# angela000/DQNFlappyBird

Hardware: AMD Instinct MI355X
Metric: env steps/sec (whole node) + DQN grad-steps/sec, 80x80x4 batch=32 (higher is better)
Workload: dtype f32

## Files before the change

dqnflappybird_amd/csrc/fb_common.h:

```cpp
#pragma once
#include <hip/hip_runtime.h>
#include <stdarg.h>
#include <stdint.h>
#include <stdio.h>
#include <string.h>
#include "../../include/fbdqn.h"

extern thread_local char fb_err_buf[512];
int fb_set_error(int code, const char *fmt, ...);

#define FB_CHECK_HIP(expr)                                                                     \
    do {                                                                                       \
        hipError_t e_ = (expr);                                                                \
        if (e_ != hipSuccess)                                                                  \
            return fb_set_error(FB_ERR_HIP, "%s failed: %s (%s:%d)", #expr, hipGetErrorString(e_), \
                                __FILE__, __LINE__);                                           \
    } while (0)

#define FB_REQUIRE(cond, ...)                                          \
    do {                                                               \
        if (!(cond)) return fb_set_error(FB_ERR_INVALID, __VA_ARGS__); \
    } while (0)

#define FB_LAUNCH_CHECK() FB_CHECK_HIP(hipGetLastError())
// ... 4 lines not shown
    return algo == FB_ALGO_C51 || algo == FB_ALGO_C51_DOUBLE || algo == FB_ALGO_C51_PER || algo == FB_ALGO_C51_DOUBLE_PER;
}
static inline bool is_double_c51(int algo) { return algo == FB_ALGO_C51_DOUBLE || algo == FB_ALGO_C51_DOUBLE_PER; }
static inline bool is_qr_algo(int algo) {
    return algo == FB_ALGO_QR || algo == FB_ALGO_QR_DOUBLE || algo == FB_ALGO_QR_PER || algo == FB_ALGO_QR_DOUBLE_PER;
}
static inline bool is_double_qr(int algo) { return algo == FB_ALGO_QR_DOUBLE || algo == FB_ALGO_QR_DOUBLE_PER; }
static inline bool is_per_algo(int algo) {
    return algo == FB_ALGO_PER || algo == FB_ALGO_C51_PER || algo == FB_ALGO_C51_DOUBLE_PER || algo == FB_ALGO_QR_PER ||
           algo == FB_ALGO_QR_DOUBLE_PER;
}

__device__ __forceinline__ unsigned long long fb_flag_load(const unsigned long long *flag) { return __hip_atomic_load(flag, __ATOMIC_RELAXED, __HIP_MEMORY_SCOPE_AGENT); }
__device__ __forceinline__ void fb_flag_store(unsigned long long *flag, unsigned long long v) { __hip_atomic_store(flag, v, __ATOMIC_RELAXED, __HIP_MEMORY_SCOPE_AGENT); }
__device__ __forceinline__ void fb_flag_acquire() { __atomic_thread_fence(__ATOMIC_ACQUIRE); }
struct FbGate { const unsigned long long *flag; unsigned long long val; unsigned *timeouts; };
__device__ __forceinline__ void fb_flag_wait(const unsigned long long *flag, unsigned long long v, unsigned *timeouts);
__device__ __forceinline__ bool fb_gate_workgroup(const FbGate &g) {
    if (!g.flag || blockIdx.x != gridDim.x - 1) return false;
    if (threadIdx.x == 0) fb_flag_wait(g.flag, g.val, g.timeouts);
    return true;
}
__device__ __forceinline__ void fb_flag_wait(const unsigned long long *flag, unsigned long long v, unsigned *timeouts) {
    if (fb_flag_load(flag) >= v) return;
    const long long t0 = wall_clock64();
    while (fb_flag_load(flag) < v) {
        __builtin_amdgcn_s_sleep(8);
        if (wall_clock64() - t0 > 100000000LL) { atomicAdd(timeouts, 1u); break; }
    }
}

#define FB_STREAM_GAP 0u
#define FB_STREAM_EPS 1u
#define FB_STREAM_SAMPLE 2u
#define FB_STREAM_PER 3u
#define FB_STREAM_INIT 4u
#define FB_STREAM_EVAL 5u
#define FB_STREAM_NOISE 6u
#define FB_STREAM_ENV_NOISE 7u

struct fb_u4 { uint32_t x, y, z, w; };

__host__ __device__ static inline fb_u4 fb_philox(uint32_t k0, uint32_t k1, uint32_t c0, uint32_t c1,
                                                  uint32_t c2, uint32_t c3) {
#pragma unroll
    for (int r = 0; r < 10; r++) {
        uint64_t p0 = (uint64_t)0xD2511F53u * c0, p1 = (uint64_t)0xCD9E8D57u * c2;
        uint32_t n0 = (uint32_t)(p1 >> 32) ^ c1 ^ k0, n1 = (uint32_t)p1;
        uint32_t n2 = (uint32_t)(p0 >> 32) ^ c3 ^ k1, n3 = (uint32_t)p0;
        c0 = n0; c1 = n1; c2 = n2; c3 = n3;
        k0 += 0x9E3779B9u; k1 += 0xBB67AE85u;
    }
    return fb_u4{c0, c1, c2, c3};
}

struct FbMT { uint32_t mt[624]; uint32_t idx; };

struct FbSplitFlags;
struct FbSampleCtx { FbMT *mt; int *error; long long n; FbSplitFlags *gate; unsigned long long gate_val; long long newest_from; int wait_last_round; };
struct FbSampleRider { FbSampleCtx ctx; int k; long long setsize; long long *out; };
struct NetOff { int bf1, wv, bv, wq, bq, n; };
struct HeadCore {
    const float *hf; int stot, nks; float *q; int FC, A, dueling; NetOff off;
    uint8_t *actions; float epsilon; uint32_t seed_lo, seed_hi, step_lo, step_hi;
};
struct FbHeadRider { HeadCore c; const float *params; int on; unsigned long long *on_arrival; unsigned long long arrival_val; };
struct FbEvalRider {
    const int32_t *env_of;
    int32_t *ep_k, *ep_len;
    int32_t *score, *length; uint8_t *trunc;
    int episodes;
    unsigned *live;
    unsigned long long *done_step;
    unsigned long long step;
};
struct FbGatherCtx {
    long long cap; int n_envs, t_f, kind;
    const unsigned long long *bits; const uint8_t *act; const float *rew; const uint8_t *term; int *error;
    int nstep; double gamma;
};
struct FbRingSrc { FbGatherCtx c; long long steps; const long long *idx; uint8_t *a; float *r; uint8_t *t; };
int fb_replay_ring_src(fb_replay_t h, int batch, const int64_t *idx, uint8_t *a, float *r, uint8_t *t, FbRingSrc *out);
int fb_qnet_train_step_ring(fb_qnet_t h, int algo, int batch, const FbRingSrc *ring, const float *isw, double gamma, float *loss,
                            float *abs_err, float *flat_grad, void *stream, const FbSampleRider *rider = nullptr, const struct FbSplitCtx *split = nullptr);
struct FbSplitFlags {
    unsigned long long c_entry, p0[7];
    unsigned long long trunk_done, p2[7];
    unsigned long long fc1_done, p3[7];
    unsigned long long env_done, p4[7];
    unsigned long long last_round, p8[7];
    unsigned clean_count;
    unsigned timeouts[7];
};
struct FbSplitCtx {
    hipStream_t tstream;
    FbSplitFlags *f;
    unsigned long long seq;
    const void *probed_stream; int probed_ok;
};
int fb_split_probe(FbSplitCtx *ctx, void *stream);
int fb_streams_concurrent(hipStream_t side, hipStream_t caller);
hipStream_t fb_side_stream_beside(hipStream_t caller, int priority, hipStream_t current, int *ok);
FbSplitCtx *fb_qnet_split_ctx(fb_qnet_t h);
int fb_replay_sample_gated(fb_replay_t h, int batch, int64_t *idx, const FbSplitCtx *ctx, void *stream, int wait_last_round = 0);
int fb_split_wait(const FbSplitCtx *ctx, const unsigned long long *flag, unsigned long long v, void *stream);
int fb_split_set(const FbSplitCtx *ctx, unsigned long long *flag, unsigned long long v, void *stream);
int fb_qnet_refresh_planes(fb_qnet_t h, void *stream);
int fb_qnet_profile_ring(fb_qnet_t h, int kernel, int reps, int algo, int batch, const FbRingSrc *ring, float *loss, void *stream);
struct FbPushRider { unsigned long long *bits; uint8_t *act; float *rew; uint8_t *term; long long *steps_dev; long long steps_new; };
int fb_env_step_rider(fb_env_t h, const uint8_t *actions, uint8_t *frames, uint64_t *frame_bits, float *reward, uint8_t *terminal,
                      int32_t *score, const FbSampleRider *rider, const FbPushRider *push, const FbHeadRider *head, void *stream);
int fb_qnet_num_actions(fb_qnet_t h);
int fb_qnet_is_c51(fb_qnet_t h);
int fb_qnet_is_qr(fb_qnet_t h);
int fb_qnet_is_dist(fb_qnet_t h);
int fb_qnet_c51_eval_head(fb_qnet_t h, const FbHeadRider *hd, int n, const int32_t *key_of, void *stream);
int fb_qnet_eval_trunk(fb_qnet_t h, const uint8_t *nib_states, int n, FbHeadRider *head, void *stream);
int fb_qnet_max_rows(fb_qnet_t h);
hipStream_t fb_qnet_side_stream(fb_qnet_t h);
void *fb_qnet_get_grad_event(fb_qnet_t h);
void *fb_qnet_take_grad_event_recorded(fb_qnet_t h);
int fb_qnet_check_step(fb_qnet_t h, int n_envs, int train_batch);
int fb_qnet_acting_noise(fb_qnet_t h);
int fb_qnet_check_env_noise(fb_qnet_t h, int n, const char *who);
int fb_qnet_act_nib_env_noise_keep(fb_qnet_t h, const uint8_t *nib_states, int n, float epsilon, uint64_t seed, uint64_t step,
                                   uint8_t *actions, float *q, void *stream);
int fb_env_num_envs(fb_env_t h);
int fb_replay_num_envs(fb_replay_t h);
int fb_replay_is_prioritized(fb_replay_t h);
int fb_replay_check_gamma(fb_replay_t h, double gamma, const char *who);
int fb_replay_check_complete(fb_replay_t h, int pushes_ahead, const char *who);
double fb_replay_bootstrap_gamma(fb_replay_t h, double gamma);
int fb_replay_update_priorities_keep(fb_replay_t h, int batch, const int64_t *idx, const float *abs_err, void *stream);
int fb_replay_update_priorities_ahead(fb_replay_t h, int batch, const int64_t *idx, const float *abs_err, void *stream);
int fb_replay_per_store_ahead(fb_replay_t h, void *stream);
int fb_replay_sample_ahead(fb_replay_t h, int batch, int64_t *idx, double *isw, float *isw32, void *stream);
int fb_env_can_carry_head(fb_env_t h);
int fb_qnet_act_nib_rider(fb_qnet_t h, const uint8_t *nib_states, int n, float epsilon, uint64_t seed, uint64_t step,
                          uint8_t *actions, FbHeadRider *head, void *stream, const FbSplitCtx *split = nullptr);
int fb_replay_begin_push_rider(fb_replay_t h, FbPushRider *push);
int fb_replay_finish_push(fb_replay_t h, void *stream);
int fb_replay_sample_f32(fb_replay_t h, int batch, const double *uniforms, int64_t *idx, double *isw, float *isw32, void *stream);
int fb_replay_sample_rider(fb_replay_t h, int batch, int64_t *idx, FbSampleRider *rider, int pushes_ahead = 1);
void fb_mt_init_genrand_host(FbMT *s, uint32_t seed);
void fb_mt_init_by_array_host(FbMT *s, const uint32_t *key, int n);
```

dqnflappybird_amd/csrc/fb_common.hip:

```cpp
#include <execinfo.h>
#include <fcntl.h>
#include <signal.h>
#include <stdlib.h>
#include <unistd.h>
#include "fb_common.h"

thread_local char fb_err_buf[512] = "";

int fb_set_error(int code, const char *fmt, ...) {
    va_list ap;
    va_start(ap, fmt);
    vsnprintf(fb_err_buf, sizeof(fb_err_buf), fmt, ap);
    va_end(ap);
    return code;
}

extern "C" const char *fb_last_error(void) { return fb_err_buf; }

static struct sigaction fb_prev_abrt;
static bool fb_abrt_installed = false;
static int fb_abrt_log_fd = -1;
static void fb_abort_backtrace(int sig, siginfo_t *info, void *ctx) {
    static const char msg[] = "\n[libfbdqn] SIGABRT: native stack of the aborting thread\n";
    void *frames[64];
// ... 180 lines not shown
}

hipStream_t fb_side_stream_beside(hipStream_t C, int priority, hipStream_t current, int *ok) {
    bool good = current && fb_streams_concurrent(current, C);
    for (int attempt = 0; !good && attempt < 6; attempt++) {
        hipStream_t ts = nullptr;
        if (hipStreamCreateWithPriority(&ts, hipStreamNonBlocking, priority) != hipSuccess) break;
        if (current) { (void)hipStreamSynchronize(current); (void)hipStreamDestroy(current); }
        current = ts;
        good = fb_streams_concurrent(current, C);
    }
    (void)hipGetLastError();
    if (ok) *ok = good ? 1 : 0;
    return current;
}

static int fb_vec_split_flag = 1;
extern "C" int fb_vec_step_set_schedule(int split) { fb_vec_split_flag = split ? 1 : 0; return FB_OK; }

extern "C" int fb_vec_step(fb_env_t env, fb_replay_t replay, fb_qnet_t net, const fb_step_buffers *b, int n_envs, int algo,
                           int batch, float epsilon, uint64_t seed, uint64_t step, int train, double gamma, void *stream) {
    FB_REQUIRE(env && replay && net && b, "fb_vec_step: NULL handle");
    FB_REQUIRE(b->nib && b->actions && b->frame_bits && b->reward && b->terminal && b->score, "fb_vec_step: NULL env buffer");
    const bool per = is_per_algo(algo);
    if (per && train) FB_REQUIRE(b->isw && b->isw32 && b->abs_err, "fb_vec_step: the prioritized step needs the isw / isw32 / abs_err buffers");
    FB_REQUIRE((algo >= 0 && algo <= 3) || is_c51_algo(algo) || is_qr_algo(algo), "fb_vec_step: unknown algo %d (0..3, FB_ALGO_C51 .. FB_ALGO_QR_DOUBLE_PER)", algo);
    if (is_c51_algo(algo) || fb_qnet_is_c51(net)) {
        FB_REQUIRE(is_c51_algo(algo) == (fb_qnet_is_c51(net) != 0),
                   "%s: a C51 net takes a C51 algo (FB_ALGO_C51, _DOUBLE, _PER, _DOUBLE_PER), and those algos take a C51 net only (algo %d)", "fb_vec_step", algo);
        if (!is_per_algo(algo))
            FB_REQUIRE(!fb_replay_is_prioritized(replay), "%s: C51 trains from a uniform memory only (prioritized replay with C51 is not supported)", "fb_vec_step");
    }
    {
        const int rq = qr_check(replay, net, algo, "fb_vec_step");
        if (rq != FB_OK) return rq;
    }
    FB_REQUIRE(per == (fb_replay_is_prioritized(replay) != 0), "fb_vec_step: algo %d and the memory's kind (uniform / prioritized) do not match", algo);
    FB_REQUIRE(n_envs == fb_env_num_envs(env) && n_envs == fb_replay_num_envs(replay), "fb_vec_step: n_envs %d does not match the env (%d) / replay (%d) handles",
               n_envs, fb_env_num_envs(env), fb_replay_num_envs(replay));
    if (train) FB_REQUIRE(b->idx && b->s && b->s2 && b->a && b->r && b->t && b->loss, "fb_vec_step: NULL training buffer");
    {
        const int rc0 = fb_qnet_check_step(net, n_envs, train ? batch : -1);
        if (rc0 != FB_OK) return rc0;
        const int rc1 = fb_replay_check_gamma(replay, gamma, "fb_vec_step");
        if (rc1 != FB_OK) return rc1;
        const int rc2 = train ? fb_replay_check_complete(replay, 1, "fb_vec_step") : FB_OK;
        if (rc2 != FB_OK) return rc2;
    }
    gamma = fb_replay_bootstrap_gamma(replay, gamma);
    const bool noisy = fb_qnet_is_noisy(net) != 0;
    const bool env_noise = noisy && fb_qnet_acting_noise(net) == FB_ACT_NOISE_PER_ENV;
    if (env_noise) {
        const int rc0 = fb_qnet_check_env_noise(net, n_envs, "fb_vec_step");
        if (rc0 != FB_OK) return rc0;
    }
    if (noisy && !env_noise) {
        const int rc0 = fb_qnet_reset_noise(net, 0, seed, step, FB_NOISE_SAMPLE, stream);
        if (rc0 != FB_OK) return rc0;
    }
    auto target_noise = [&]() { return noisy ? fb_qnet_reset_noise(net, 1, seed, step, FB_NOISE_SAMPLE, stream) : FB_OK; };
    if (fb_vec_split_flag && train && !per && n_envs >= 256 && batch < 256 && fb_env_can_carry_head(env) && fb_qnet_num_actions(net) == 2 &&
        !fb_qnet_is_dist(net)) {
        hipStream_t A = fb_stream(stream);
        hipStreamCaptureStatus cap = hipStreamCaptureStatusNone;
        (void)hipStreamIsCapturing(A, &cap);
        FbSampleRider probe;
        FbSplitCtx *sc = cap == hipStreamCaptureStatusNone && fb_replay_sample_rider(replay, batch, b->idx, &probe) ? fb_qnet_split_ctx(net) : nullptr;
        if (sc && !fb_split_probe(sc, stream)) sc = nullptr;
        if (sc) {
            hipStream_t C = A, S = sc->tstream;
            FbSplitFlags *F = sc->f;
            sc->seq += 1;
            const int trunk_wgs = (n_envs + 4) / 5, wait_last_round = n_envs >= 4096 && trunk_wgs % 256 != 0;
            if (!fb_replay_sample_gated(replay, batch, b->idx, sc, C, wait_last_round)) { sc->seq -= 1; return fb_set_error(FB_ERR_HIP, "fb_vec_step: the gated draw could not be launched"); }
            int rc = fb_split_wait(sc, &F->c_entry, sc->seq, S);
            FbHeadRider hrider;
            if (rc == FB_OK) rc = fb_qnet_act_nib_rider(net, b->nib, n_envs, epsilon, seed, step, b->actions, &hrider, S, sc);
            if (rc != FB_OK) { (void)hipStreamSynchronize(S); return rc; }
            hrider.on_arrival = &F->fc1_done; hrider.arrival_val = sc->seq;
            FbPushRider prider;
            fb_replay_begin_push_rider(replay, &prider);
            FbRingSrc ring;
            rc = fb_replay_ring_src(replay, batch, b->idx, b->a, b->r, b->t, &ring);
            if (rc == FB_OK) rc = fb_qnet_train_step_ring(net, algo, batch, &ring, nullptr, gamma, b->loss, nullptr, b->flat_grad, C, nullptr, sc);
            const int rc2 = fb_env_step_rider(env, b->actions, nullptr, b->frame_bits, b->reward, b->terminal, b->score, nullptr, &prider, &hrider, S);
            const int rc3 = fb_split_set(sc, &F->env_done, sc->seq, S);
            return rc != FB_OK ? rc : rc2 != FB_OK ? rc2 : rc3;
        }
    }
    int sampled = 0;
    if (per && fb_replay_per_store_ahead(replay, stream) && train)
        sampled = fb_replay_sample_ahead(replay, batch, b->idx, b->isw, b->isw32, stream);
    FbHeadRider hrider;
    const int have_h = fb_env_can_carry_head(env) && fb_qnet_num_actions(net) == 2 && !fb_qnet_is_dist(net);
    int rc = have_h ? fb_qnet_act_nib_rider(net, b->nib, n_envs, epsilon, seed, step, b->actions, &hrider, stream)
             : env_noise ? fb_qnet_act_nib_env_noise_keep(net, b->nib, n_envs, epsilon, seed, step, b->actions, nullptr, stream)
                         : fb_qnet_act_nib(net, b->nib, n_envs, epsilon, seed, step, b->actions, nullptr, stream);
    if (rc != FB_OK) return rc;
    FbSampleRider srider;
    FbPushRider prider;
    const int have_s = train ? fb_replay_sample_rider(replay, batch, b->idx, &srider) : 0;
    const int have_p = fb_replay_begin_push_rider(replay, &prider);
    rc = fb_env_step_rider(env, b->actions, nullptr, b->frame_bits, b->reward, b->terminal, b->score, have_s ? &srider : nullptr,
                           have_p ? &prider : nullptr, have_h ? &hrider : nullptr, stream);
    if (rc != FB_OK) return rc;
    if (!have_p) {
        if (train && !have_s && !per) rc = fb_replay_push_sample(replay, nullptr, b->frame_bits, b->actions, b->reward, b->terminal, batch, b->idx, stream);
        else rc = fb_replay_push(replay, nullptr, b->frame_bits, b->actions, b->reward, b->terminal, stream);
    } else {
        rc = fb_replay_finish_push(replay, stream);
        if (rc == FB_OK && train && !have_s && !per) rc = fb_replay_sample(replay, batch, nullptr, b->idx, nullptr, stream);
    }
    if (rc == FB_OK && env_noise) rc = fb_qnet_reset_noise(net, 0, seed, step, FB_NOISE_SAMPLE, stream);
    if (rc != FB_OK || !train) return rc;
    if (per) {
        if (!sampled) rc = fb_replay_sample_f32(replay, batch, nullptr, b->idx, b->isw, b->isw32, stream);
        if (rc != FB_OK) return rc;
        rc = target_noise();
        if (rc != FB_OK) return rc;
        if (n_envs >= 256) {
            FbRingSrc ring;
            rc = fb_replay_ring_src(replay, batch, b->idx, b->a, b->r, b->t, &ring);
            if (rc == FB_OK) rc = fb_qnet_train_step_ring(net, algo, batch, &ring, b->isw32, gamma, b->loss, b->abs_err, b->flat_grad, stream);
        } else {
            rc = fb_replay_gather(replay, batch, b->idx, b->s, b->s2, b->a, b->r, b->t, stream);
            if (rc == FB_OK) rc = fb_qnet_train_step(net, algo, batch, b->s, b->a, b->r, b->s2, b->t, b->isw32, gamma, b->loss, b->abs_err, nullptr, b->flat_grad, stream);
        }
        if (rc != FB_OK) return rc;
        if (fb_replay_update_priorities_ahead(replay, batch, b->idx, b->abs_err, stream)) return FB_OK;
        return fb_replay_update_priorities_keep(replay, batch, b->idx, b->abs_err, stream);
    }
    rc = target_noise();
    if (rc != FB_OK) return rc;
    if (n_envs >= 256) {
        FbRingSrc ring;
        rc = fb_replay_ring_src(replay, batch, b->idx, b->a, b->r, b->t, &ring);
        if (rc != FB_OK) return rc;
        return fb_qnet_train_step_ring(net, algo, batch, &ring, nullptr, gamma, b->loss, nullptr, b->flat_grad, stream);
    }
    rc = fb_replay_gather(replay, batch, b->idx, b->s, b->s2, b->a, b->r, b->t, stream);
    if (rc != FB_OK) return rc;
    return fb_qnet_train_step(net, algo, batch, b->s, b->a, b->r, b->s2, b->t, nullptr, gamma, b->loss, nullptr, nullptr, b->flat_grad,
                              stream);
}

extern "C" int fb_train_from_replay(fb_replay_t replay, fb_qnet_t net, int algo, int batch, const int64_t *idx, const float *isw, uint8_t *a,
                                    float *r, uint8_t *t, double gamma, float *loss, float *abs_err, float *flat_grad, void *stream) {
    FB_REQUIRE(replay && net && idx && a && r && t && loss, "fb_train_from_replay: NULL argument");
    FB_REQUIRE((algo >= 0 && algo <= 3) || is_c51_algo(algo) || is_qr_algo(algo), "fb_train_from_replay: unknown algo %d (0..3, FB_ALGO_C51 .. FB_ALGO_QR_DOUBLE_PER)", algo);
    if (is_c51_algo(algo) || fb_qnet_is_c51(net)) {
        FB_REQUIRE(is_c51_algo(algo) == (fb_qnet_is_c51(net) != 0),
                   "%s: a C51 net takes a C51 algo (FB_ALGO_C51, _DOUBLE, _PER, _DOUBLE_PER), and those algos take a C51 net only (algo %d)", "fb_train_from_replay", algo);
        if (!is_per_algo(algo))
            FB_REQUIRE(!fb_replay_is_prioritized(replay), "%s: C51 trains from a uniform memory only (prioritized replay with C51 is not supported)", "fb_train_from_replay");
    }
    {
        const int rq = qr_check(replay, net, algo, "fb_train_from_replay");
        if (rq != FB_OK) return rq;
    }
    FB_REQUIRE(!is_per_algo(algo) || isw, "fb_train_from_replay: the prioritized step needs the importance weights");
    if (is_c51_algo(algo) && is_per_algo(algo))
        FB_REQUIRE(fb_replay_is_prioritized(replay), "fb_train_from_replay: algo %d (C51 with prioritized replay) trains from a prioritized memory only", algo);
    FB_REQUIRE(batch >= 1 && batch <= 256, "fb_train_from_replay: batch must be in 1..256");
    int rc = fb_replay_check_gamma(replay, gamma, "fb_train_from_replay");
    if (rc != FB_OK) return rc;
    rc = fb_replay_check_complete(replay, 0, "fb_train_from_replay");
    if (rc != FB_OK) return rc;
    gamma = fb_replay_bootstrap_gamma(replay, gamma);
    FbRingSrc ring;
    rc = fb_replay_ring_src(replay, batch, idx, a, r, t, &ring);
    if (rc != FB_OK) return rc;
    if (batch >= 256) {
        rc = fb_qnet_refresh_planes(net, stream);
        if (rc != FB_OK) return rc;
    }
    return fb_qnet_train_step_ring(net, algo, batch, &ring, isw, gamma, loss, abs_err, flat_grad, stream);
}

extern "C" int fb_profile_ring_kernel(fb_replay_t replay, fb_qnet_t net, int kernel, int reps, int algo, int batch, const int64_t *idx,
                                      uint8_t *a, float *r, uint8_t *t, float *loss, void *stream) {
    FB_REQUIRE(replay && net && idx && a && r && t && loss && reps >= 1, "fb_profile_ring_kernel: bad argument");
    FbRingSrc ring;
    int rc = fb_replay_ring_src(replay, batch, idx, a, r, t, &ring);
    if (rc != FB_OK) return rc;
    return fb_qnet_profile_ring(net, kernel, reps, algo, batch, &ring, loss, stream);
}
```

dqnflappybird_amd/csrc/fb_qnet.hip:

```cpp
#include <math.h>
#include <stdlib.h>
#include "fb_common.h"

#ifndef FK_ABL
#define FK_ABL 0
#endif
#ifndef BW_ABL
#define BW_ABL 0
#endif

namespace {

typedef float f32x16 __attribute__((ext_vector_type(16)));

constexpr int OFF_W1 = 0, OFF_B1 = 8192, OFF_W2 = 8224, OFF_B2 = 40992, OFF_W3 = 41056, OFF_B3 = 77920,
              OFF_WF1 = 77984;
constexpr int CONV_PARAMS = OFF_WF1;
#include "fb_head.h"
#include "fb_sampler.h"
#include "fb_gather.h"
constexpr int MAXTB = 256;


struct Slice { const float *params; const uint8_t *states; int s_off, count; const uint16_t *w1s; int fshift; };
// ... 814 lines not shown
                    if constexpr (NS == 3) {
                        const _Float16 hh = (_Float16)bv, ll = (_Float16)((bv - (float)hh) * F16_LO_SCALE);
                        d[0] = __builtin_bit_cast(uint16_t, hh); d[IN_P * 8] = __builtin_bit_cast(uint16_t, ll);
                        bad |= bv >= FB_F16_RANGE;
                    } else d[0] = (uint16_t)f32_to_bf16_rn(bv);
                }
            }
        }
    }
    __syncthreads();
    if (W16 && wave >= 8) { if constexpr (NS == 3) note_overflow(bad, a.ovf); return; }
    if (RING && C23T_EXIT == 2) { if (smem[tid].x == 0x12345u) a.h2[0] = 1.f; return; }
    const int oy = j / 5, ox = j - oy * 5;
    const bool rowok = j < 25;
    f32x16 acc = {0}, acl = {0};
    auto finish = [&](const float *__restrict__ bias, float *__restrict__ out, bool planes) {
#pragma unroll
        for (int r = 0; r < 16; r++) red[((kq * 2 + ct) * 16 + r) * 64 + lane] = NS == 3 ? fmaf(acl[r], F16_LO_UNSCALE, acc[r]) : acc[r];
        __syncthreads();
        const int ctp = wave & 1, q = wave >> 1;
        float v[4];
#pragma unroll
        for (int e = 0; e < 4; e++) {
            v[e] = red[((0 * 2 + ctp) * 16 + 4 * q + e) * 64 + lane];
#pragma unroll
            for (int k = 1; k < 4; k++) v[e] += red[((k * 2 + ctp) * 16 + 4 * q + e) * 64 + lane];
        }
        const int ch = ctp * 32 + 8 * q + 4 * hl;
        const float4 bv = *reinterpret_cast<const float4 *>(bias + ch);
        v[0] = fmaxf(v[0] + bv.x, 0.f); v[1] = fmaxf(v[1] + bv.y, 0.f); v[2] = fmaxf(v[2] + bv.z, 0.f); v[3] = fmaxf(v[3] + bv.w, 0.f);
        if (rowok) *reinterpret_cast<float4 *>(out + (row * 25 + j) * 64 + ch) = make_float4(v[0], v[1], v[2], v[3]);
        if ((planes || a.a3s) && rowok) {
            uint32_t h0, l0, h1, l1, m_;
            if constexpr (NS == 3) { split2x2(v[0], v[1], h0, l0); split2x2(v[2], v[3], h1, l1); bad |= out_of_f16_range(v[0], v[1], v[2], v[3]); }
            else { split3x2(v[0], v[1], h0, m_, l0); split3x2(v[2], v[3], h1, m_, l1); }
            if (planes) {
                uint2 *d = reinterpret_cast<uint2 *>(smem + C2O + j * 8 + ((ctp * 4 + q) ^ ((j >> 1) & 7))) + hl;
                d[0] = make_uint2(h0, h1);
                if (NS == 3) d[2 * C2_P] = make_uint2(l0, l1);
            } else {
                uint16_t *d = a.a3s + (row * 25 + j) * 64 + ch;
                *reinterpret_cast<uint2 *>(d) = make_uint2(h0, h1);
                if (NS == 3) *reinterpret_cast<uint2 *>(d + a.pl3) = make_uint2(l0, l1);
            }
        }
#pragma unroll
        for (int r = 0; r < 16; r++) { acc[r] = 0.f; acl[r] = 0.f; }
    };
#pragma unroll
    for (int c = 0; c < 17; c++) {
        int aidx[2];
        if (c < 8) {
            const int tap = 2 * c + (kq >> 1), iy = 2 * oy + (tap >> 2) - 1, ix = 2 * ox + (tap & 3) - 1, pix = iy * 10 + ix;
            const bool ok = rowok && iy >= 0 && iy < 10 && ix >= 0 && ix < 10;
#pragma unroll
            for (int p = 0; p < NPL; p++) aidx[p] = ok ? p * IN_P + pix * 4 + ((((kq & 1) * 2 + hl) + (pix >> 2)) & 3) : ZOFF;
        } else {
            const int tap = c - 8, ky = tap / 3, iy = oy + ky - 1, ix = ox + (tap - 3 * ky) - 1, pix = iy * 5 + ix;
            const bool ok = rowok && iy >= 0 && iy < 5 && ix >= 0 && ix < 5;
#pragma unroll
            for (int p = 0; p < NPL; p++) aidx[p] = ok ? C2O + p * C2_P + pix * 8 + ((2 * kq + hl) ^ ((pix >> 1) & 7)) : ZOFF;
        }
        uint4 A[NPL];
#pragma unroll
        for (int p = 0; p < NPL; p++) A[p] = smem[aidx[p]];
        const WF W = w0;
        w0 = w1; w1 = w2;
        if (c + 3 < 17) w2 = loadW(c + 3);
        if constexpr (NS == 3) {
            acl = mfma_h(W.v[0], A[1], acl);
            acl = mfma_h(W.v[1], A[0], acl);
            acc = mfma_h(W.v[0], A[0], acc);
        } else acc = mfma_b(W.v[0], A[0], acc);
        if (c == 7) { finish(s.params + OFF_B2, a.h2, true); __syncthreads(); }
    }
    finish(s.params + OFF_B3, a.h3, false);
    if constexpr (NS == 3) note_overflow(bad, a.ovf);
}

constexpr int FC1_SP_KS = 4;
struct Fc1Args { const uint16_t *ain; size_t aplane; const uint16_t *zeros; const uint4 *w; float *hfp; int stot, M, N;
                 const unsigned *pver; unsigned *wver;
                 const uint4 *w2; int m_split;
                 const float *hp_src; float *hp_dst; int hp_n;
                 unsigned long long *set_flag; unsigned long long set_val; };

#ifndef FC1_ABL
#define FC1_ABL 0
#endif
template <int NS>
__global__ __launch_bounds__(256) void fc1_sp_kernel(Fc1Args a) {
    constexpr int NPL = NS == 3 ? 2 : 1, P0 = NS == 3 ? 0 : 2;
    constexpr int ASZ = NPL * 512, BSZ = 4 * NPL * 64, SLOT = ASZ + BSZ;
    __shared__ uint4 smem[3 * SLOT];
    const int lane = threadIdx.x & 63, wave = threadIdx.x >> 6, hl = lane >> 5, j = lane & 31;
    if (a.wver && blockIdx.x == 0 && threadIdx.x == 0) *a.wver = *a.pver;
    if (a.hp_dst) { const int i = blockIdx.x * 256 + threadIdx.x; if (i < a.hp_n) a.hp_dst[i] = a.hp_src[i]; }
    if (a.set_flag && blockIdx.x == 0 && threadIdx.x == 0) fb_flag_store(a.set_flag, a.set_val);
    const int xcd = blockIdx.x & 7, w = blockIdx.x >> 3, nth = a.N >> 7;
    const int ks = xcd & 3, m0 = (w / nth) * 128, n0 = ((xcd >> 2) * nth + w % nth) * 64;
    const int cbase = ks * 12 + (ks < 2 ? ks : 2), count = ks < 2 ? 13 : 12;
    struct St { uint4 a0, a1, a2, a3, b0, b1; };
    const int r0 = min(m0 + (int)(threadIdx.x >> 2), a.M - 1), r1 = min(m0 + 64 + (int)(threadIdx.x >> 2), a.M - 1);
    const uint16_t *pa0 = a.ain + (size_t)r0 * 1600 + (size_t)cbase * 32 + (threadIdx.x & 3) * 8;
    const uint16_t *pa1 = a.ain + (size_t)r1 * 1600 + (size_t)cbase * 32 + (threadIdx.x & 3) * 8;
    auto ldA = [&](int c, int p, int i) { return *reinterpret_cast<const uint4 *>((i ? pa1 : pa0) + p * a.aplane + c * 32); };
    const uint4 *wsel = a.w2 && m0 >= a.m_split ? a.w2 : a.w;
    auto pbq = [&](int q) {
        const int e = wave + 4 * q, k8 = e / NPL, pl = e - k8 * NPL;
        return wsel + ((size_t)(cbase * 4 + k8) * 3 + P0 + pl) * a.N + n0 + lane;
    };
    const uint4 *pb0 = pbq(0), *pb1 = pbq(NPL == 2 ? 1 : 0);
    const size_t bstep = (size_t)12 * a.N;
    auto ldB = [&](int c, int q) {
        (void)c;
        const uint4 *&pb = q == 0 ? pb0 : pb1;
        const uint4 v = *pb;
        pb += bstep;
        return v;
    };
    auto load = [&](int c) {
        St r;
        r.a0 = ldA(c, 0, 0); r.a1 = ldA(c, 0, 1); r.b0 = ldB(c, 0);
        if (NPL == 2) { r.a2 = ldA(c, 1, 0); r.a3 = ldA(c, 1, 1); r.b1 = ldB(c, 1); }
        else { r.a2 = r.a0; r.a3 = r.a0; r.b1 = r.b0; }
        return r;
    };
    auto stA_ = [&](int slot, int p, int i, const uint4 v) {
        const int q = threadIdx.x + 256 * i, row = q >> 2;
        smem[slot * SLOT + p * 512 + row * 4 + ((q + (row >> 2)) & 3)] = v;
    };
    auto store = [&](int slot, const St r) {
        stA_(slot, 0, 0, r.a0); stA_(slot, 0, 1, r.a1);
        uint4 *d = smem + slot * SLOT + ASZ + wave * 64 + lane;
        d[0] = r.b0;
        if (NPL == 2) { stA_(slot, 1, 0, r.a2); stA_(slot, 1, 1, r.a3); d[256] = r.b1; }
    };
    struct Fr { uint4 A[NPL]; uint4 W[2][NPL]; };
    const int row = wave * 32 + j;
    auto readF = [&](int slot, int s) {
        Fr f;
#pragma unroll
        for (int p = 0; p < NPL; p++) {
            f.A[p] = smem[slot * SLOT + p * 512 + row * 4 + ((2 * s + hl + (row >> 2)) & 3)];
#pragma unroll
            for (int ct = 0; ct < 2; ct++) f.W[ct][p] = smem[slot * SLOT + ASZ + ((2 * s + hl) * NPL + p) * 64 + ct * 32 + j];
        }
        return f;
    };
    f32x16 acc[2] = {{0}, {0}}, acl[2] = {{0}, {0}};
    auto compute = [&](const Fr f) {
        if (FC1_ABL == 2) { acc[0][0] += __uint_as_float(f.A[0].x ^ f.W[0][0].y ^ f.W[1][NPL - 1].z ^ f.A[NPL - 1].w); return; }
#pragma unroll
        for (int ct = 0; ct < 2; ct++) {
            if constexpr (NS == 3) {
                acl[ct] = mfma_h(f.A[1], f.W[ct][0], acl[ct]);
                acl[ct] = mfma_h(f.A[0], f.W[ct][1], acl[ct]);
                acc[ct] = mfma_h(f.A[0], f.W[ct][0], acc[ct]);
            } else acc[ct] = mfma_b(f.A[0], f.W[ct][0], acc[ct]);
        }
    };
    St stA = load(0), stB = load(1);
    store(0, stA); stA = load(2);
    __syncthreads();
    store(1, stB); stB = load(3);
    Fr cur = readF(0, 0);
    __syncthreads();
#define FB_STEP(cc, ST)                                                                                    \
    {                                                                                                          \
        const Fr f1 = FC1_ABL == 3 ? cur : readF((cc) % 3, 1);                                                 \
        __builtin_amdgcn_sched_barrier(0);                                                                     \
        compute(cur);                                                                                          \
        __builtin_amdgcn_sched_barrier(0);                                                                     \
        const Fr nx = FC1_ABL == 3 ? cur : readF(((cc) + 1) % 3, 0);                                           \
        if ((cc) + 2 < 13) { if (FC1_ABL != 3) store(((cc) + 2) % 3, ST); if ((cc) + 4 < 13 && FC1_ABL != 1) ST = load((cc) + 4); }              \
        __builtin_amdgcn_sched_barrier(0);                                                                     \
        compute(f1);                                                                                           \
        __builtin_amdgcn_sched_barrier(0);                                                                     \
        __syncthreads();                                                                                       \
        cur = nx;                                                                                              \
    }
// ... 126 lines not shown
#pragma unroll
                for (int a = 0; a < AT; a++) dadv[tid][a] = a == a_b ? g : 0.f;
            }
        }
    }
    __syncthreads();
    if (lead && tid == 0) {
        float s = 0.f;
        for (int b = 0; b < B; b++) s += lterm[b];
        *L.loss = L.algo == FB_ALGO_DQN ? s : s / (float)B;
        if (L.tick && L.adam->ticks == L.adam->applies) {
            AdamDev &ad = *L.adam;
            ad.alpha = ad.lr * sqrtf(1.f - ad.b2pow) / (1.f - ad.b1pow);
            ad.b1pow *= ad.b1; ad.b2pow *= ad.b2;
            ad.ticks += 1;
        }
    }
    if (lead && tid >= 64 && tid < 64 + A) { const int a = tid - 64; float s = 0.f; for (int b = 0; b < B; b++) s += dadv[b][a]; L.grad[L.off.bq + a] = s; }
    if (lead && tid == 128 && L.dueling) { float s = 0.f; for (int b = 0; b < B; b++) s += dv[b]; L.grad[L.off.bv] = s; }
    for (int b0 = bg; b0 < B; b0 += 128) {
        if (b0 != bg) {
#pragma unroll
            for (int u = 0; u < 8; u++) {
                const int b = b0 + 16 * u;
                hv[u] = fc1_out(L.hf, L.stot, L.FC, b < B ? b : bg, jj, bias, L.nks);
            }
#pragma unroll
            for (int u = 0; u < 8; u++) keep(hv[u]);
        }
#pragma unroll
        for (int u = 0; u < 8; u++) {
            const int b = b0 + 16 * u;
            if (b < B) {
                const float h = hv[u];
                float d = dv[b] * wvj;
#pragma unroll
                for (int a = 0; a < AT; a++) if (a < A) { d = fmaf(dadv[b][a], wrow[a], d); gw[a] = fmaf(h, dadv[b][a], gw[a]); }
                gv = fmaf(h, dv[b], gv);
                const float dh = h > 0.f ? d : 0.f;
                L.dhf[(size_t)b * L.FC + jj] = dh;
                dmax = fmaxf(dmax, fabsf(dh));
                gb += dh;
            }
        }
    }
#pragma unroll
    for (int a = 0; a < AT; a++) part[bg][jl][a] = gw[a];
    part[bg][jl][MAXA] = gv; part[bg][jl][MAXA + 1] = gb;
    wg_max_write(dmax, wmax, tid >> 6, tid & 63);
    __syncthreads();
    if (tid == 0) L.gmax[blockIdx.x] = wg_max_read<4>(wmax);
    if (bg == 0) {
        auto total = [&](int c) {
            float v = part[0][jl][c];
#pragma unroll
            for (int g = 1; g < 16; g++) v += part[g][jl][c];
            return v;
        };
#pragma unroll
        for (int a = 0; a < AT; a++)
            if (a < A) L.grad[L.off.wq + jj * A + a] = total(a);
        if (L.dueling) L.grad[L.off.wv + jj] = total(MAXA);
        L.grad[L.off.bf1 + jj] = total(MAXA + 1);
    }
}

__global__ __launch_bounds__(256) void loss_head_kernel(LossArgs L) {
    __shared__ float dadv[MAXTB][MAXA];
    __shared__ float dv[MAXTB];
    __shared__ float lterm[MAXTB];
    __shared__ float part[16][16][MAXA + 2];
    __shared__ float wmax[4];
    if (L.A == 2) loss_head_body<2>(L, dadv, dv, lterm, part, wmax);
    else loss_head_body<MAXA>(L, dadv, dv, lterm, part, wmax);
}

__global__ void adam_tick_kernel(AdamDev *ad) {
    if (ad->ticks != ad->applies) return;
    ad->alpha = ad->lr * sqrtf(1.f - ad->b2pow) / (1.f - ad->b1pow);
    ad->b1pow *= ad->b1; ad->b2pow *= ad->b2;
    ad->ticks += 1;
}
__global__ void bump_pver_kernel(AdamDev *ad, int which) { ad->pver[which] += 1; }
__global__ void mark_split_kernel(AdamDev *ad, int which) { ad->wver[which] = ad->pver[which]; ad->wverc[which] = ad->pver[which]; }

struct C51Sup { int N; float vmin, vmax, dz; };
__device__ __forceinline__ float rdlane(float v, int l) { return __int_as_float(__builtin_amdgcn_readlane(__float_as_int(v), l)); }
__device__ __forceinline__ float wave_sum(float v) {
#pragma unroll
    for (int o = 32; o > 0; o >>= 1) v += __shfl_xor(v, o);
    return v;
}
template <int AT>
__device__ __forceinline__ void c51_logits(const float *__restrict__ hf, int stot, int nks, int FC, const float *__restrict__ P, const NetOff &off,
                                           int A, int N, int row, int lane, float (&lg)[AT]) {
    const int AN = A * N, il = lane < N ? lane : N - 1;
#pragma unroll
    for (int a = 0; a < AT; a++) lg[a] = 0.f;
    for (int j0 = 0; j0 < FC; j0 += 64) {
        const float x = fc1_out(hf, stot, FC, row, j0 + lane, P[off.bf1 + j0 + lane], nks);
        const float *__restrict__ w = P + off.wq + (size_t)j0 * AN + il;
#pragma unroll 8
        for (int k = 0; k < 64; k++) {
            const float xs = rdlane(x, k);
#pragma unroll
            for (int a = 0; a < AT; a++) lg[a] = fmaf(xs, w[(size_t)k * AN + (a < A ? a : 0) * N], lg[a]);
        }
    }
#pragma unroll
    for (int a = 0; a < AT; a++) lg[a] += P[off.bq + (a < A ? a : 0) * N + il];
}
__device__ __forceinline__ float c51_softmax(float lg, bool on, float &lse) {
    const float m = wave_max(on ? lg : -INFINITY);
    const float e = on ? expf(lg - m) : 0.f;
    const float s = wave_sum(e);
    lse = m + logf(s);
    return e / s;
}
template <int AT>
__device__ __forceinline__ void c51_q(const float (&lg)[AT], bool on, float z, float (&qv)[AT]) {
#pragma unroll
    for (int a = 0; a < AT; a++) {
        float lse;
        qv[a] = wave_sum(c51_softmax(lg[a], on, lse) * z);
    }
}

struct C51Core {
    const float *hf; int stot, nks; float *q, *probs; int FC, A; NetOff off; C51Sup sup;
    uint8_t *actions; float epsilon; uint32_t seed_lo, seed_hi, step_lo, step_hi;
    const int32_t *key_of; uint32_t stream;
};
template <int AT, bool QR = false>
__device__ __forceinline__ void c51_head_one(const C51Core &C, const float *__restrict__ P, int smp, int lane) {
    const int A = AT == MAXA ? C.A : AT, N = C.sup.N;
    const bool on = lane < N;
    const int key = C.key_of ? C.key_of[smp] : smp;
    float lg[AT], qv[AT];
    c51_logits<AT>(C.hf, C.stot, C.nks, C.FC, P, C.off, A, N, smp, lane, lg);
    const float z = C.sup.vmin + (float)(on ? lane : 0) * C.sup.dz;
    if constexpr (QR) {
        float *row = C.probs ? C.probs + (size_t)smp * A * N + lane : nullptr;
#pragma unroll
        for (int a = 0; a < AT; a++) {
            if (row && on && a < A) row[a * N] = lg[a];
            qv[a] = wave_sum(on ? lg[a] : 0.f) * (1.f / (float)N);
        }
    } else if (C.probs) {
        float *row = C.probs + (size_t)smp * A * N + lane;
#pragma unroll
        for (int a = 0; a < AT; a++) {
            float lse;
            const float p = c51_softmax(lg[a], on, lse);
            if (on && a < A) row[a * N] = p;
            qv[a] = wave_sum(p * z);
        }
    } else c51_q<AT>(lg, on, z, qv);
    if (lane == 0) {
#pragma unroll
        for (int a = 0; a < AT; a++) if (a < A) C.q[(size_t)smp * A + a] = qv[a];
        if (C.actions) {
            int best = 0;
#pragma unroll
            for (int a = 1; a < AT; a++) if (a < A && qv[a] > qv[best]) best = a;
            const fb_u4 o = fb_philox(C.seed_lo, C.seed_hi, (uint32_t)key, C.step_lo, C.stream, C.step_hi);
            const float u = (float)(o.x >> 8) * (1.0f / 16777216.0f);
// ... 1114 lines not shown
        float g4[4];
#pragma unroll
        for (int q = 0; q < 4; q++) g4[q] = gmax[lane + 64 * q < nm ? lane + 64 * q : 0];
#pragma unroll
        for (int q = 0; q < 4; q++) gm = fmaxf(gm, g4[q]);
    }
    if (tile < n_dx) {
        const int mt = tile / 50, it = tile - mt * 50, m = mt * 32 + r;
        const int per = KX ? KX : FC / 128, k0 = wave * per;
        const float4 *pa = reinterpret_cast<const float4 *>(dhf + (size_t)(m < B ? m : 0) * FC + 8 * hl) + k0 * 4;
        const float4 *pb = reinterpret_cast<const float4 *>(params + OFF_WF1 + (size_t)(it * 32 + r) * FC + 8 * hl) + k0 * 4;
        auto ld = [&](int ks) { return FragF{pa[ks * 4], pa[ks * 4 + 1], pb[ks * 4], pb[ks * 4 + 1]}; };
        if constexpr (KX > 0) {
            FragF f[KX];
#pragma unroll
            for (int q = 0; q < KX; q++) f[q] = ld(q);
            const Pow2 G = pow2_scale(wave_max(gm));
#pragma unroll
            for (int q = 0; q < KX; q++) mma_frag<NS, true>(f[q], acc, acl, G.s, bad);
            if constexpr (NS == 3) {
#pragma unroll
                for (int q = 0; q < 16; q++) acc[q] = fmaf(acl[q], F16_LO_UNSCALE, acc[q]) * G.inv;
            }
        } else {
            const Pow2 G = pow2_scale(wave_max(gm));
            for (int q = 0; q < per; q++) mma_frag<NS, true>(ld(q), acc, acl, G.s, bad);
            if constexpr (NS == 3) {
#pragma unroll
                for (int q = 0; q < 16; q++) acc[q] = fmaf(acl[q], F16_LO_UNSCALE, acc[q]) * G.inv;
            }
        }
        reduce_rows<8>(acc, red, wave, lane, mt * 32, B, [&](float v, int, int mr) {
            const size_t o = (size_t)mr * 1600 + it * 32 + r;
            dh3[o] = h3[o] > 0.f ? v : 0.f;
        });
        return;
    }
    const int t = tile - n_dx, nt_n = FC / 32;
    const int it = t / nt_n, nt = t - it * nt_n;
    const float *pa = h3 + it * 32 + r, *pb = dhf + nt * 32 + r;
    const int per = KW ? KW : ((B + 15) / 16 + 7) / 8, k0 = wave * per;
    auto ld = [&](int ks) {
        const int b0 = 16 * (k0 + ks) + 8 * hl;
        float a[8], bb[8];
#pragma unroll
        for (int j = 0; j < 8; j++) {
            const bool ok = b0 + j < B;
            const size_t bc = ok ? b0 + j : 0;
            const float x = pa[bc * 1600], y = pb[bc * FC];
            a[j] = ok ? x : 0.f; bb[j] = ok ? y : 0.f;
        }
        return FragF{make_float4(a[0], a[1], a[2], a[3]), make_float4(a[4], a[5], a[6], a[7]), make_float4(bb[0], bb[1], bb[2], bb[3]),
                     make_float4(bb[4], bb[5], bb[6], bb[7])};
    };
    const Pow2 G = pow2_scale(wave_max(gm));
    if constexpr (KW > 0) {
        FragF f[KW];
#pragma unroll
        for (int q = 0; q < KW; q++) f[q] = ld(q);
#pragma unroll
        for (int q = 0; q < KW; q++) mma_frag<NS, false>(f[q], acc, acl, G.s, bad);
    } else {
        for (int q = 0; q < per; q++) mma_frag<NS, false>(ld(q), acc, acl, G.s, bad);
    }
    if constexpr (NS == 3) {
#pragma unroll
        for (int q = 0; q < 16; q++) acc[q] = fmaf(acl[q], F16_LO_UNSCALE, acc[q]) * G.inv;
        note_overflow(bad, ovf);
    }
    reduce_rows<8>(acc, red, wave, lane, 0, 32, [&](float v, int, int row32) {
        grad[OFF_WF1 + (size_t)(it * 32 + row32) * FC + nt * 32 + r] = v;
    });
}

__device__ __forceinline__ void adam4(float4 &P, float4 &Mv, float4 &V, const float4 Gv, float alpha, float omb1, float omb2, float eps) {
#define FB_ADAM1(c)                                  \
    Mv.c += (Gv.c - Mv.c) * omb1;                    \
    V.c += (Gv.c * Gv.c - V.c) * omb2;               \
    P.c -= (Mv.c * alpha) / (sqrtf(V.c) + eps);
    FB_ADAM1(x) FB_ADAM1(y) FB_ADAM1(z) FB_ADAM1(w)
#undef FB_ADAM1
}

struct AdamSpan { float *p, *m, *v; const float *g; const AdamDev *ad; int q0, q1; };
__device__ __forceinline__ void adam_span_body(int blk, int nblk, const AdamSpan a) {
    const float alpha = a.ad->alpha, omb1 = 1.f - a.ad->b1, omb2 = 1.f - a.ad->b2, eps = a.ad->eps;
    for (int q = a.q0 + blk * (int)blockDim.x + (int)threadIdx.x; q < a.q1; q += nblk * (int)blockDim.x) {
        float4 P = reinterpret_cast<float4 *>(a.p)[q], Mv = reinterpret_cast<float4 *>(a.m)[q], V = reinterpret_cast<float4 *>(a.v)[q];
        adam4(P, Mv, V, reinterpret_cast<const float4 *>(a.g)[q], alpha, omb1, omb2, eps);
        reinterpret_cast<float4 *>(a.p)[q] = P; reinterpret_cast<float4 *>(a.m)[q] = Mv; reinterpret_cast<float4 *>(a.v)[q] = V;
    }
}

constexpr int DW1_IMG_W = 104, DW1_IMG_H = 84, DW1_IMG = DW1_IMG_H * DW1_IMG_W * 4;
constexpr int DW1_STEPS = 30;

template <int NSP> struct Dw1Lds { static constexpr int U4 = DW1_IMG / 16 + (DW1_STEPS / NSP) * 2 * 64 + 64 + 4; };

struct Dw1Ring { const unsigned long long *bits, *fo; };
template <int NSP, bool RING = false>
__device__ __forceinline__ void conv1_dw2_body(int blk, const uint8_t *__restrict__ states, const float *__restrict__ dp1,
                                               const uint8_t *__restrict__ amax, float *__restrict__ slabs, size_t slab_stride, uint4 *pool,
                                               Dw1Ring ring = Dw1Ring{nullptr, nullptr}) {
    constexpr int SW = DW1_STEPS / NSP, PU = (SW + 7) / 8;
    uint4 *img4 = pool, *bfr = pool + DW1_IMG / 16;
    float (*bsum)[32] = reinterpret_cast<float (*)[32]>(bfr + SW * 2 * 64);
    float *sx = reinterpret_cast<float *>(bfr + SW * 2 * 64 + 64);
    const int b = blk / NSP, part = blk - b * NSP, s0 = part * SW;
    const int tid = threadIdx.x, lane = tid & 63, wave = tid >> 6, hl = lane >> 5, c = lane & 31;
    uint8_t *img = reinterpret_cast<uint8_t *>(img4);
    float dv[PU][4];
    int am[PU][4];
#pragma unroll
    for (int u = 0; u < PU; u++) {
        const int ls = wave + 8 * u, g = 2 * (s0 + ls) + hl, oy = g / 3, ox0 = (g - 3 * oy) * 8;
#pragma unroll
        for (int q = 0; q < 4; q++) {
            const int px = (ox0 >> 1) + q;
            const bool ok = ls < SW && px < 10;
            const uint32_t po = ((uint32_t)b * 100u + (uint32_t)(ok ? (oy >> 1) * 10 + px : 0)) * 32u + (uint32_t)c;
            dv[u][q] = dp1[po]; am[u][q] = amax[po];
        }
    }
    {
        float m = 0.f;
#pragma unroll
        for (int u = 0; u < PU; u++)
#pragma unroll
            for (int q = 0; q < 4; q++) m = fmaxf(m, wave + 8 * u < SW ? fabsf(dv[u][q]) : 0.f);
        wg_max_write(m, sx, wave, lane);
    }
    uint4 pxa, pxb, pxc, pxd;
    if constexpr (!RING) {
        const uint4 *sp = reinterpret_cast<const uint4 *>(states + (size_t)b * 25600);
        pxa = sp[tid]; pxb = sp[tid + 512]; pxc = sp[tid + 1024]; pxd = sp[tid + 1536 < 1600 ? tid + 1536 : 0];
    } else {
        const unsigned long long f0 = ring.fo[b * 4], f1 = ring.fo[b * 4 + 1], f2 = ring.fo[b * 4 + 2], f3 = ring.fo[b * 4 + 3];
        auto chunk = [&](int i) {
            const int pp = (i < 1600 ? i : 0) * 4, w = pp >> 6, sh = pp & 63;
            const uint32_t n0 = (uint32_t)(ring.bits[f0 + w] >> sh) & 0xFu, n1 = (uint32_t)(ring.bits[f1 + w] >> sh) & 0xFu,
                           n2 = (uint32_t)(ring.bits[f2 + w] >> sh) & 0xFu, n3 = (uint32_t)(ring.bits[f3 + w] >> sh) & 0xFu;
            return make_uint4(expand4(n0, n1, n2, n3, 0), expand4(n0, n1, n2, n3, 1), expand4(n0, n1, n2, n3, 2), expand4(n0, n1, n2, n3, 3));
        };
        pxa = chunk(tid); pxb = chunk(tid + 512); pxc = chunk(tid + 1024); pxd = chunk(tid + 1536);
    }
    for (int i = tid; i < DW1_IMG / 16; i += 512) img4[i] = make_uint4(0u, 0u, 0u, 0u);
    __syncthreads();
    {
        auto put = [&](int i, const uint4 v) {
            const int row = i / 20, col4 = i - row * 20;
            if (i < 1600) *reinterpret_cast<uint4 *>(img + ((row + 2) * DW1_IMG_W + 4 + 4 * col4) * 4) = v;
        };
        put(tid, pxa); put(tid + 512, pxb); put(tid + 1024, pxc); put(tid + 1536, pxd);
    }
    const Pow2 S1 = pow2_scale(wg_max_read<8>(sx));
    float bs = 0.f;
#pragma unroll
    for (int u = 0; u < PU; u++) {
        const int ls = wave + 8 * u, g = 2 * (s0 + ls) + hl, oy = g / 3, ox0 = (g - 3 * oy) * 8;
        float v[8];
#pragma unroll
        for (int q = 0; q < 4; q++) {
            const bool ok = ls < SW && (ox0 >> 1) + q < 10;
            const int pos = (oy & 1) * 2;
            v[2 * q] = ok && am[u][q] == pos ? dv[u][q] : 0.f;
            v[2 * q + 1] = ok && am[u][q] == pos + 1 ? dv[u][q] : 0.f;
        }
        uint4 fh, fl;
        split2x2(v[0] * S1.s, v[1] * S1.s, fh.x, fl.x); split2x2(v[2] * S1.s, v[3] * S1.s, fh.y, fl.y);
        split2x2(v[4] * S1.s, v[5] * S1.s, fh.z, fl.z); split2x2(v[6] * S1.s, v[7] * S1.s, fh.w, fl.w);
        if (ls < SW) { bfr[(ls * 2 + 0) * 64 + lane] = fh; bfr[(ls * 2 + 1) * 64 + lane] = fl; }
#pragma unroll
        for (int q = 0; q < 8; q++) bs += v[q];
    }
    bs += __shfl_xor(bs, 32);
    if (hl == 0) bsum[wave][c] = bs;
    __syncthreads();
    const int ky = wave, kx = c >> 2, ci = c & 3;
    const uint8_t *tapk = img + (ky * DW1_IMG_W + kx + 2) * 4 + ci;
    struct Ops { uint32_t x[8]; uint4 bh, bl; };
    auto fetch = [&](int ls) {
        const int g = 2 * (s0 + ls) + hl, oy = g / 3, ox0 = (g - 3 * oy) * 8;
        const uint8_t *tap = tapk + ((4 * oy) * DW1_IMG_W + 4 * ox0) * 4;
        Ops o;
#pragma unroll
        for (int jq = 0; jq < 8; jq++) o.x[jq] = tap[16 * jq];
        o.bh = bfr[(ls * 2 + 0) * 64 + lane]; o.bl = bfr[(ls * 2 + 1) * 64 + lane];
        return o;
    };
    f32x16 acc = {0}, acl = {0};
    Ops cur = fetch(0);
#pragma unroll
    for (int ls = 0; ls < SW; ls++) {
        Ops nxt = cur;
        if (ls + 1 < SW) nxt = fetch(ls + 1);
        uint4 A;
        {
            const f32x2 p0 = {(float)cur.x[0], (float)cur.x[1]}, p1 = {(float)cur.x[2], (float)cur.x[3]};
            const f32x2 p2 = {(float)cur.x[4], (float)cur.x[5]}, p3 = {(float)cur.x[6], (float)cur.x[7]};
            A.x = __builtin_bit_cast(uint32_t, __builtin_convertvector(p0, f16x2)); A.y = __builtin_bit_cast(uint32_t, __builtin_convertvector(p1, f16x2));
            A.z = __builtin_bit_cast(uint32_t, __builtin_convertvector(p2, f16x2)); A.w = __builtin_bit_cast(uint32_t, __builtin_convertvector(p3, f16x2));
        }
        acc = mfma_h(A, cur.bh, acc);
        acl = mfma_h(A, cur.bl, acl);
        cur = nxt;
    }
    float *o = slabs + (size_t)blk * slab_stride;
#pragma unroll
    for (int r = 0; r < 16; r++) o[OFF_W1 + (ky * 32 + drow(r, lane)) * 32 + c] = fmaf(acl[r], F16_LO_UNSCALE, acc[r]) * S1.inv;
    if (wave == 0 && hl == 0) {
        float sum = bsum[0][c];
#pragma unroll
        for (int w = 1; w < 8; w++) sum += bsum[w][c];
        o[OFF_B1 + c] = sum;
    }
}

template <int NS>
__global__ __launch_bounds__(512) void conv_bx_kernel(BxArgs bx, int B, int nz, float *__restrict__ slabs, size_t slab_stride, int n_adam,
                                                      AdamSpan span, FbSampleRider rider, int rb) {
    __shared__ uint4 pool[BxLds<NS>::U4];
    static_assert(BxLds<NS>::U4 * 16 >= FB_SAMPLE_LDS_WORDS * 4 && BxLds<NS>::U4 >= 2048, "the riders borrow the pool");
    const int rid = rider.k ? 1 : 0, bid = (int)blockIdx.x - rid;
    if (bid < 0) {
        uint32_t *sw = reinterpret_cast<uint32_t *>(pool);
        if (threadIdx.x < 64) sample_cpython_body(rider.ctx, rider.k, rider.setsize, rider.out, sw, reinterpret_cast<int *>(sw + 624));
        return;
    }
    if (bid < B) { conv32_bx_body<NS>(bx, bid, pool); return; }
    const int t = bid - B;
    if (t < 38 * nz) {
        float *red = reinterpret_cast<float *>(pool);
        conv_dw_body<3>(t % 38, t / 38, nz, red, B, bx.h2, bx.dh3, slabs, slab_stride, rb);
        return;
    }
    adam_span_body(t - 38 * nz, n_adam, span);
}

template <int NSP, bool RING>
__global__ __launch_bounds__(512) void conv_dw21_kernel(int nz, int B, const float *__restrict__ p1, const float *__restrict__ dh2,
                                                        const uint8_t *__restrict__ states, const float *__restrict__ dp1,
                                                        const uint8_t *__restrict__ amax, float *__restrict__ slabs, size_t slab_stride,
                                                        float *__restrict__ slabs1, size_t stride1, int rb, Dw1Ring ring, FbGate gate) {
    if (fb_gate_workgroup(gate)) return;
    const int n2 = 34 * nz;
    __shared__ uint4 pool[Dw1Lds<NSP>::U4];
    static_assert(Dw1Lds<NSP>::U4 >= 2048, "the conv2 tiles borrow the pool");
    if ((int)blockIdx.x < n2) {
        float *red = reinterpret_cast<float *>(pool);
        conv_dw_body<2>(blockIdx.x % 34, blockIdx.x / 34, nz, red, B, p1, dh2, slabs, slab_stride, rb);
        return;
    }
    if ((int)blockIdx.x < n2 + NSP * B) conv1_dw2_body<NSP, RING>((int)blockIdx.x - n2, states, dp1, amax, slabs1, stride1, pool, ring);
}

constexpr int BW1_ROWS = 44, BW1_IMG_U4 = BW1_ROWS * DW1_IMG_W * 4 / 16;
constexpr int BW_NW2 = 2, BW_NW3 = 2, BW_WGS = 2 + BW_NW2 + BW_NW3;
constexpr int BW_AUX_U4 = 1200, BW_DP1_U4 = 800;
template <int NS> struct BwLds { static constexpr int CH = BxLds<NS>::U4, U4 = CH + BW_AUX_U4 + BW_DP1_U4; };
static_assert(BW1_IMG_U4 <= BW_AUX_U4, "C1's image lives in the aux area");

#ifndef DWT_ABL
#define DWT_ABL 0
#endif
template <int LAYER>
__device__ __forceinline__ void dw_sample_tiles(const float *xs, const float *dys, float *__restrict__ o, bool rb, int sub, int nsub) {
    using G = DwGeom<LAYER>;
    constexpr int NT = DWT_ABL == 3 ? 8 : G::CELLS * G::CIT * 2;
    const int lane = threadIdx.x & 63, wave = threadIdx.x >> 6, hl = lane >> 5, i = lane & 31;
    for (int tile = wave + 8 * sub; tile < NT; tile += 8 * nsub) {
        const int cot = tile & 1, cit = G::CIT == 2 ? (tile >> 1) & 1 : 0, cell = tile / (2 * G::CIT), ky = cell / G::K, kx = cell - ky * G::K;
        float a[13], bb[13];
#pragma unroll
        for (int t = 0; t < 13; t++) {
            const int m = 2 * t + hl;
            const int oy = hl ? (2 * t + 1) / 5 : (2 * t) / 5, ox = hl ? (2 * t + 1) % 5 : (2 * t) % 5;
            const bool ok = t < 12 || hl == 0;
            const int iy = oy * G::S + ky - G::P, ix = ox * G::S + kx - G::P;
            const bool in = ok && iy >= 0 && iy < G::IH && ix >= 0 && ix < G::IW;
            const float xv = xs[(in ? iy * G::IW + ix : 0) * G::CI + cit * 32 + i], dv = dys[(ok ? m : 0) * 64 + cot * 32 + i];
            a[t] = in ? xv : 0.f; bb[t] = ok ? dv : 0.f;
        }
        f32x16 acc = {0};
        if (DWT_ABL == 1) { float sm = 0.f;
#pragma unroll
            for (int t = 0; t < 13; t++) sm += a[t] * bb[t];
#pragma unroll
            for (int r = 0; r < 16; r++) acc[r] = sm; }
        else {
#pragma unroll
        for (int t = 0; t < 13; t++) acc = mfma(rbf(a[t], rb), rbf(bb[t], rb), acc);
        }
        if (DWT_ABL == 2) { if (acc[0] == 12345.f) o[0] = acc[3]; continue; }
#pragma unroll
        for (int r = 0; r < 16; r++) o[G::WOFF + (size_t)(cell * G::CI + cit * 32 + drow(r, lane)) * G::CO + cot * 32 + i] = acc[r];
    }
}
__device__ __forceinline__ void dw_sample_bias(const float *dys, float *__restrict__ ob) {
    if (threadIdx.x < 64) {
        float sum = dys[threadIdx.x];
#pragma unroll
        for (int m = 1; m < 25; m++) sum += dys[m * 64 + threadIdx.x];
        ob[threadIdx.x] = sum;
    }
}

struct Bw1Pre { int am[2][4]; uint4 pxa, pxb; };
template <bool RING>
__device__ __forceinline__ Bw1Pre bw1_request(int b, int part, const uint8_t *__restrict__ states, const uint8_t *__restrict__ amax, Dw1Ring ring) {
    const int tid = threadIdx.x, lane = tid & 63, wave = tid >> 6, hl = lane >> 5, c = lane & 31, s0 = part * 15;
    Bw1Pre r;
#pragma unroll
    for (int u = 0; u < 2; u++) {
        const int ls = wave + 8 * u, g = 2 * (s0 + ls) + hl, oy = g / 3, ox0 = (g - 3 * oy) * 8;
#pragma unroll
        for (int q = 0; q < 4; q++) {
            const int px = (ox0 >> 1) + q;
            const bool ok = ls < 15 && px < 10;
            r.am[u][q] = amax[((uint32_t)b * 100u + (uint32_t)(ok ? (oy >> 1) * 10 + px : 0)) * 32u + (uint32_t)c];
        }
    }
    const int i0 = part ? 760 : 0, ia = i0 + tid, ib = i0 + (tid < 328 ? 512 + tid : 0);
    if constexpr (!RING) {
        const uint4 *sp = reinterpret_cast<const uint4 *>(states + (size_t)b * 25600);
        r.pxa = sp[ia]; r.pxb = sp[ib];
    } else {
        const unsigned long long f0 = ring.fo[b * 4], f1 = ring.fo[b * 4 + 1], f2 = ring.fo[b * 4 + 2], f3 = ring.fo[b * 4 + 3];
// ... 27 lines not shown
    float m = 0.f;
#pragma unroll
    for (int u = 0; u < PU; u++) {
        const int ls = wave + 8 * u, g = 2 * (s0 + ls) + hl, oy = g / 3, ox0 = (g - 3 * oy) * 8;
#pragma unroll
        for (int q = 0; q < 4; q++) {
            const int px = (ox0 >> 1) + q;
            const bool ok = ls < SW && px < 10;
            dv[u][q] = dp1s[(ok ? (oy >> 1) * 10 + px : 0) * 32 + c];
            m = fmaxf(m, ls < SW ? fabsf(dv[u][q]) : 0.f);
        }
    }
    wg_max_write(m, sx, wave, lane);
    __syncthreads();
    const Pow2 S1 = pow2_scale(wg_max_read<8>(sx));
    float bs = 0.f;
#pragma unroll
    for (int u = 0; u < PU; u++) {
        const int ls = wave + 8 * u, g = 2 * (s0 + ls) + hl, oy = g / 3, ox0 = (g - 3 * oy) * 8;
        float v[8];
#pragma unroll
        for (int q = 0; q < 4; q++) {
            const bool ok = ls < SW && (ox0 >> 1) + q < 10;
            const int pos = (oy & 1) * 2;
            v[2 * q] = ok && pre.am[u][q] == pos ? dv[u][q] : 0.f;
            v[2 * q + 1] = ok && pre.am[u][q] == pos + 1 ? dv[u][q] : 0.f;
        }
        uint4 fh, fl;
        split2x2(v[0] * S1.s, v[1] * S1.s, fh.x, fl.x); split2x2(v[2] * S1.s, v[3] * S1.s, fh.y, fl.y);
        split2x2(v[4] * S1.s, v[5] * S1.s, fh.z, fl.z); split2x2(v[6] * S1.s, v[7] * S1.s, fh.w, fl.w);
        if (ls < SW) { bfr[(ls * 2 + 0) * 64 + lane] = fh; bfr[(ls * 2 + 1) * 64 + lane] = fl; }
#pragma unroll
        for (int q = 0; q < 8; q++) bs += v[q];
    }
    bs += __shfl_xor(bs, 32);
    if (hl == 0) bsum[wave][c] = bs;
    __syncthreads();
    const int ky = wave, kx = c >> 2, ci = c & 3;
    const uint8_t *tapk = img + ((ky - 40 * part) * DW1_IMG_W + kx + 2) * 4 + ci;
    struct Ops { uint32_t x[8]; uint4 bh, bl; };
    auto fetch = [&](int ls) {
        const int g = 2 * (s0 + ls) + hl, oy = g / 3, ox0 = (g - 3 * oy) * 8;
        const uint8_t *tap = tapk + ((4 * oy) * DW1_IMG_W + 4 * ox0) * 4;
        Ops o;
#pragma unroll
        for (int jq = 0; jq < 8; jq++) o.x[jq] = tap[16 * jq];
        o.bh = bfr[(ls * 2 + 0) * 64 + lane]; o.bl = bfr[(ls * 2 + 1) * 64 + lane];
        return o;
    };
    f32x16 acc = {0}, acl = {0};
    Ops cur = fetch(0);
#pragma unroll
    for (int ls = 0; ls < SW; ls++) {
        Ops nxt = cur;
        if (ls + 1 < SW) nxt = fetch(ls + 1);
        uint4 A;
        {
            const f32x2 p0 = {(float)cur.x[0], (float)cur.x[1]}, p1 = {(float)cur.x[2], (float)cur.x[3]};
            const f32x2 p2 = {(float)cur.x[4], (float)cur.x[5]}, p3 = {(float)cur.x[6], (float)cur.x[7]};
            A.x = __builtin_bit_cast(uint32_t, __builtin_convertvector(p0, f16x2)); A.y = __builtin_bit_cast(uint32_t, __builtin_convertvector(p1, f16x2));
            A.z = __builtin_bit_cast(uint32_t, __builtin_convertvector(p2, f16x2)); A.w = __builtin_bit_cast(uint32_t, __builtin_convertvector(p3, f16x2));
        }
        acc = mfma_h(A, cur.bh, acc);
        acl = mfma_h(A, cur.bl, acl);
        cur = nxt;
    }
    float *o = slabs + (size_t)blk * slab_stride;
#pragma unroll
    for (int r = 0; r < 16; r++) o[OFF_W1 + (ky * 32 + drow(r, lane)) * 32 + c] = fmaf(acl[r], F16_LO_UNSCALE, acc[r]) * S1.inv;
    if (wave == 0 && hl == 0) {
        float sum = bsum[0][c];
#pragma unroll
        for (int w = 1; w < 8; w++) sum += bsum[w][c];
        o[OFF_B1 + c] = sum;
    }
}

#ifndef CBW_ABL
#define CBW_ABL 0
#endif
template <int NS, bool RING>
__global__ __launch_bounds__(512) void conv_bw_kernel(BxArgs bx, int B, float *__restrict__ slabs, size_t slab_stride, float *__restrict__ slabs1,
                                                      size_t stride1, const uint8_t *__restrict__ states, const uint8_t *__restrict__ amax, Dw1Ring ring,
                                                      int n_adam, AdamSpan span, FbSampleRider rider, int rb, FbGate gate) {
    __shared__ uint4 pool[BwLds<NS>::U4];
    if (fb_gate_workgroup(gate)) return;
    static_assert(BwLds<NS>::U4 * 16 >= FB_SAMPLE_LDS_WORDS * 4, "the sampler rider borrows the pool");
    uint4 *aux = pool + BwLds<NS>::CH;
    float *dp1s = reinterpret_cast<float *>(aux + BW_AUX_U4);
    const int rid = rider.k ? 1 : 0, bid = (int)blockIdx.x - rid, tid = threadIdx.x;
    if (bid < 0) {
        uint32_t *sw = reinterpret_cast<uint32_t *>(pool);
        if (tid < 64) sample_cpython_body(rider.ctx, rider.k, rider.setsize, rider.out, sw, reinterpret_cast<int *>(sw + 624));
        return;
    }
    if (bid < 2 * B) {
        if (CBW_ABL == 5 || CBW_ABL == 6 || CBW_ABL == 7 || CBW_ABL == 8 || CBW_ABL == 11) return;
        const int b = bid >> 1, part = bid & 1;
        const Bw1Pre pre = bw1_request<RING>(b, part, states, amax, ring);
        for (int i = tid; i < BW1_IMG_U4; i += 512) aux[i] = make_uint4(0u, 0u, 0u, 0u);
        conv32_bx_body<NS, 1>(bx, b, pool, dp1s);
        bw1_put(pre, part, aux);
        __syncthreads();
        if (CBW_ABL == 1 || CBW_ABL == 10) { if (dp1s[tid] == 12345.f) slabs1[0] = 1.f; return; }
        bw1_main(bid, part, pre, dp1s, aux, pool + (BwLds<NS>::CH - 2048 - 4), slabs1, stride1);
        return;
    }
    if (bid < (2 + BW_NW2) * B) {
        if (CBW_ABL == 6 || CBW_ABL == 7 || CBW_ABL == 9 || CBW_ABL == 10) return;
        const int b = (bid - 2 * B) / BW_NW2, sub = (bid - 2 * B) - b * BW_NW2;
        float *p1s = reinterpret_cast<float *>(aux), *dys = p1s + 3200;
        const float4 *src = reinterpret_cast<const float4 *>(bx.p1 + (size_t)b * 3200);
        const float4 xa = src[tid], xb = src[tid < 288 ? 512 + tid : 0];
        reinterpret_cast<float4 *>(p1s)[tid] = xa;
        if (tid < 288) reinterpret_cast<float4 *>(p1s)[512 + tid] = xb;
        conv32_bx_body<NS, 2>(bx, b, pool, dys);
        __syncthreads();
        float *o = slabs + (size_t)b * slab_stride;
        if (CBW_ABL == 2 || CBW_ABL == 11) { if (dys[tid] == 12345.f) o[0] = 1.f; return; }
        dw_sample_tiles<2>(p1s, dys, o, rb, sub, BW_NW2);
        if (sub == BW_NW2 - 1) dw_sample_bias(dys, o + OFF_B2);
        return;
    }
    if (bid < BW_WGS * B) {
        if (CBW_ABL == 3 || CBW_ABL == 6 || CBW_ABL == 8 || CBW_ABL == 9 || CBW_ABL == 10 || CBW_ABL == 11) return;
        const int b = (bid - (2 + BW_NW2) * B) / BW_NW3, sub = (bid - (2 + BW_NW2) * B) - b * BW_NW3;
        float *dys = reinterpret_cast<float *>(aux), *xs = dys + 1600;
        const int q = tid < 400 ? tid : 0;
        const float4 d = reinterpret_cast<const float4 *>(bx.dh3 + (size_t)b * 1600)[q], x = reinterpret_cast<const float4 *>(bx.h2 + (size_t)b * 1600)[q];
        if (tid < 400) { reinterpret_cast<float4 *>(dys)[tid] = d; reinterpret_cast<float4 *>(xs)[tid] = x; }
        __syncthreads();
        float *o = slabs + (size_t)b * slab_stride;
        dw_sample_tiles<3>(xs, dys, o, rb, sub, BW_NW3);
        if (sub == BW_NW3 - 1) dw_sample_bias(dys, o + OFF_B3);
        return;
    }
    if (CBW_ABL == 4) return;
    adam_span_body(bid - BW_WGS * B, n_adam, span);
}

template <int NS> struct DwgLds {
    static constexpr int NPL = NS == 3 ? 2 : 1, PLH = 25 * 32 * 16;
    static constexpr int U4 = 2 * NPL * PLH / 8 + 64 + 128 + 2048 + 4;
};

template <int NS, int LAYER>
__device__ __forceinline__ void conv_dwg_body(int blk, const float *__restrict__ x, const float *__restrict__ dy, float *__restrict__ slabs,
                                              size_t slab_stride, uint4 *pool, unsigned *ovf) {
    constexpr int NPL = DwgLds<NS>::NPL, PLH = DwgLds<NS>::PLH, ZERO = 2 * NPL * PLH;
    uint16_t *X = reinterpret_cast<uint16_t *>(pool), *DY = X + NPL * PLH;
    float *part = reinterpret_cast<float *>(pool + 2 * NPL * PLH / 8 + 64);
    float *red = part + 512;
    float *sx = red + 8192;
    const int tid = threadIdx.x, lane = tid & 63, wave = tid >> 6, hl = lane >> 5, r = lane & 31;
    const int cot = blk & 1, mid = LAYER == 3 ? (blk >> 1) & 1 : (blk >> 1) & 3, g = LAYER == 3 ? blk >> 2 : blk >> 3;
    const int py = mid >> 1, px = mid & 1;
    float xa[13], xb[13], ya[13], yb[13];
#pragma unroll
    for (int q = 0; q < 13; q++) {
        const int w = wave + 8 * q, wc = w < 100 ? w : 0, pos = wc % 25, bp = wc / 25 + 4 * hl;
        const size_t s0 = (size_t)g * 16 + 2 * bp;
        size_t xo;
        if (LAYER == 3) xo = (s0 * 25 + pos) * 64 + mid * 32 + r;
        else { const int qy = pos / 5, qx = pos - qy * 5; xo = (s0 * 100 + (py + 2 * qy) * 10 + px + 2 * qx) * 32 + r; }
        const size_t yo = (s0 * 25 + pos) * 64 + cot * 32 + r;
        xa[q] = x[xo]; xb[q] = x[xo + (LAYER == 3 ? 1600 : 3200)];
        ya[q] = dy[yo]; yb[q] = dy[yo + 1600];
    }
    if (tid < 64) pool[2 * NPL * PLH / 8 + tid] = make_uint4(0u, 0u, 0u, 0u);
// ... 82 lines not shown
        fold();
        if (half) {
#pragma unroll
            for (int q = 0; q < 16; q++) red[(t4 * 16 + q) * 64 + lane] = acc[q];
        }
        __syncthreads();
        if (!half) {
#pragma unroll
            for (int q = 0; q < 16; q++)
                o[OFF_W2 + (size_t)(((ky * 4 + kx) * 32 + drow(q, lane)) * 64) + cot * 32 + r] = acc[q] + red[(t4 * 16 + q) * 64 + lane];
        }
    }
}

template <int NS>
__global__ __launch_bounds__(512) void conv_dwg_kernel(int n3, const float *__restrict__ h2, const float *__restrict__ dh3, const float *__restrict__ p1,
                                                       const float *__restrict__ dh2, float *__restrict__ slabs, size_t slab_stride, unsigned *__restrict__ ovf) {
    __shared__ uint4 pool[DwgLds<NS>::U4];
    if ((int)blockIdx.x < n3) conv_dwg_body<NS, 3>(blockIdx.x, h2, dh3, slabs, slab_stride, pool, ovf);
    else conv_dwg_body<NS, 2>(blockIdx.x - n3, p1, dh2, slabs, slab_stride, pool, ovf);
}

constexpr int CONV1_PARAMS = OFF_W2;
__global__ void slab_fold_kernel(const float *__restrict__ sub, int nsub, int fold, float *__restrict__ slabs, size_t slab_stride) {
    const int idx = blockIdx.x * blockDim.x + threadIdx.x, s = blockIdx.y;
    if (idx >= CONV1_PARAMS) return;
    float v = 0.f;
    for (int q0 = 0; q0 < fold; q0 += 4) {
        float x[4];
#pragma unroll
        for (int q = 0; q < 4; q++) {
            const int z = s * fold + q0 + q;
            const bool ok = q0 + q < fold && z < nsub;
            x[q] = sub[(size_t)(ok ? z : 0) * CONV1_PARAMS + idx];
            x[q] = ok ? x[q] : 0.f;
        }
#pragma unroll
        for (int q = 0; q < 4; q++) v += x[q];
    }
    slabs[s * slab_stride + idx] = v;
}

constexpr int SLAB_CHUNK = 16;
__device__ __forceinline__ float4 slab_chunk4(const float *__restrict__ slabs, size_t slab_stride, long long q4, int z, int c) {
    float4 g = make_float4(0.f, 0.f, 0.f, 0.f), t[SLAB_CHUNK];
    const int s0 = c * SLAB_CHUNK;
#pragma unroll
    for (int q = 0; q < SLAB_CHUNK; q++) t[q] = *reinterpret_cast<const float4 *>(slabs + (size_t)(s0 + q < z ? s0 + q : 0) * slab_stride + q4 * 4);
#pragma unroll
    for (int q = 0; q < SLAB_CHUNK; q++) {
        const bool ok = s0 + q < z;
        g.x += ok ? t[q].x : 0.f; g.y += ok ? t[q].y : 0.f; g.z += ok ? t[q].z : 0.f; g.w += ok ? t[q].w : 0.f;
    }
    return g;
}
__device__ __forceinline__ float4 add4(float4 a, float4 b) { return make_float4(a.x + b.x, a.y + b.y, a.z + b.z, a.w + b.w); }
__device__ __forceinline__ float4 slab_combine4(float4 c0, float4 c1, float4 c2, float4 c3) { return add4(add4(add4(c0, c1), c2), c3); }
__device__ __forceinline__ float4 slab_sum4(const float *__restrict__ slabs, size_t slab_stride, long long q4, int z) {
    const float4 zero = make_float4(0.f, 0.f, 0.f, 0.f);
    const float4 c0 = slab_chunk4(slabs, slab_stride, q4, z, 0);
    const float4 c1 = z > SLAB_CHUNK ? slab_chunk4(slabs, slab_stride, q4, z, 1) : zero;
    const float4 c2 = z > 2 * SLAB_CHUNK ? slab_chunk4(slabs, slab_stride, q4, z, 2) : zero;
    const float4 c3 = z > 3 * SLAB_CHUNK ? slab_chunk4(slabs, slab_stride, q4, z, 3) : zero;
    return slab_combine4(c0, c1, c2, c3);
}

__global__ __launch_bounds__(256) void slab_reduce_kernel(const float *__restrict__ slabs, size_t slab_stride, int z1, int z2, int z3,
                                   float *__restrict__ grad) {
    const int q4 = blockIdx.x * blockDim.x + threadIdx.x, idx = q4 * 4;
    if (idx >= CONV_PARAMS) return;
    const int z = idx < OFF_W2 ? z1 : (idx < OFF_W3 ? z2 : z3);
    reinterpret_cast<float4 *>(grad)[q4] = slab_sum4(slabs, slab_stride, q4, z);
}
static_assert(OFF_W2 % 4 == 0 && OFF_W3 % 4 == 0 && CONV_PARAMS % 4 == 0, "slab regions are float4 aligned");

constexpr int ADAMF_T2 = 64, ADAMF_T3 = 72;
struct AdamFused {
    float *p, *m, *v; const float *g; long long n; AdamDev *ad;
    const float *slabs; size_t slab_stride; int z1, z2, z3;
    uint16_t *w1s; uint4 *wsp; int FC;
    int tail0;
    int n_rest;
    int lanes;
    FbSplitFlags *split; unsigned long long split_val;
};
__device__ __forceinline__ float4 shfl4(float4 v, int src) { return make_float4(__shfl(v.x, src), __shfl(v.y, src), __shfl(v.z, src), __shfl(v.w, src)); }
__global__ __launch_bounds__(256) void adam_fused_kernel(AdamFused a) {
    __shared__ float tile[8][68];
    const int bid = blockIdx.x, tid = threadIdx.x, lane = tid & 63;
    const float alpha = a.ad->alpha, omb1 = 1.f - a.ad->b1, omb2 = 1.f - a.ad->b2, eps = a.ad->eps;
    const float4 zero = make_float4(0.f, 0.f, 0.f, 0.f);
    if (bid < ADAMF_T2 + ADAMF_T3) {
        const bool l3 = bid >= ADAMF_T2;
        const int k0 = 8 * (l3 ? bid - ADAMF_T2 : bid), woff = l3 ? OFF_W3 : OFF_W2, CI = l3 ? 64 : 32, z = l3 ? a.z3 : a.z2;
        const int f = tid >> 1, c = tid & 1, kr = f >> 4, c4 = f & 15;
        const long long q = (woff + (k0 + kr) * 64 + 4 * c4) >> 2;
        float4 P = reinterpret_cast<float4 *>(a.p)[q], Mv = reinterpret_cast<float4 *>(a.m)[q], V = reinterpret_cast<float4 *>(a.v)[q];
        float4 Gv;
        if (z > 0) {
            const float4 ca = slab_chunk4(a.slabs, a.slab_stride, q, z, c);
            const float4 cb = z > 2 * SLAB_CHUNK ? slab_chunk4(a.slabs, a.slab_stride, q, z, c + 2) : zero;
            const float4 oa = shfl4(ca, lane ^ 1), ob = shfl4(cb, lane ^ 1);
            Gv = c == 0 ? slab_combine4(ca, oa, cb, ob) : slab_combine4(oa, ca, ob, cb);
        } else Gv = reinterpret_cast<const float4 *>(a.g)[q];
        adam4(P, Mv, V, Gv, alpha, omb1, omb2, eps);
        if (c == 0) {
            reinterpret_cast<float4 *>(a.p)[q] = P; reinterpret_cast<float4 *>(a.m)[q] = Mv; reinterpret_cast<float4 *>(a.v)[q] = V;
            *reinterpret_cast<float4 *>(&tile[kr][4 * c4]) = P;
        }
        __syncthreads();
        if (tid < 64) {
            const int col = tid;
            uint4 *o = a.wsp + (l3 ? WSP_W3 : WSP_W2) + (size_t)(k0 / 8) * 3 * 64 + col;
            wsplit_store(o, 64, tile[0][col], tile[1][col], tile[2][col], tile[3][col], tile[4][col], tile[5][col], tile[6][col], tile[7][col]);
        } else if (tid < 128) {
            const int r = (tid - 64) >> 3, co8 = tid & 7, tap = k0 / CI, ci = k0 - tap * CI + r;
            uint4 *o = a.wsp + (l3 ? wsp_w3t(a.FC) : wsp_w2t(a.FC)) + (size_t)(tap * 8 + co8) * 3 * CI + ci;
            const float *t = &tile[r][8 * co8];
            wsplit_store(o, CI, t[0], t[1], t[2], t[3], t[4], t[5], t[6], t[7]);
        }
        return;
    }
    const int n0 = OFF_W2 / 4, n1 = (OFF_W3 - OFF_B2) / 4, n2 = (OFF_WF1 - OFF_B3) / 4;
    const long long n4 = a.n >> 2, nq = n0 + n1 + n2 + (n4 - a.tail0);
    const int L = a.lanes, per = 256 / L, c = tid & (L - 1);
    for (long long base = (long long)(bid - ADAMF_T2 - ADAMF_T3) * per; base < nq; base += (long long)a.n_rest * per) {
        const long long qq = base + tid / L;
        const bool live = qq < nq;
        const long long qc = live ? qq : 0;
        long long q; int z;
        if (qc < n0) { q = qc; z = a.z1; }
        else if (qc < n0 + n1) { q = OFF_B2 / 4 + (qc - n0); z = a.z2; }
        else if (qc < n0 + n1 + n2) { q = OFF_B3 / 4 + (qc - n0 - n1); z = a.z3; }
        else { q = a.tail0 + (qc - n0 - n1 - n2); z = 0; }
        float4 P = reinterpret_cast<float4 *>(a.p)[q], Mv = reinterpret_cast<float4 *>(a.m)[q], V = reinterpret_cast<float4 *>(a.v)[q];
        float4 Gv;
        if (L == 4) {
            const float4 mine = z > c * SLAB_CHUNK ? slab_chunk4(a.slabs, a.slab_stride, q, z, c) : zero;
            const int l0 = lane & ~3;
            const float4 c0 = shfl4(mine, l0), c1 = shfl4(mine, l0 + 1), c2 = shfl4(mine, l0 + 2), c3 = shfl4(mine, l0 + 3);
            Gv = z > 0 ? slab_combine4(c0, c1, c2, c3) : reinterpret_cast<const float4 *>(a.g)[q];
        } else Gv = z > 0 ? slab_sum4(a.slabs, a.slab_stride, q, z) : reinterpret_cast<const float4 *>(a.g)[q];
        adam4(P, Mv, V, Gv, alpha, omb1, omb2, eps);
        if (live && c == 0) {
            reinterpret_cast<float4 *>(a.p)[q] = P; reinterpret_cast<float4 *>(a.m)[q] = Mv; reinterpret_cast<float4 *>(a.v)[q] = V;
            if (q * 4 < OFF_B1) {
                const int idx = (int)q * 4;
                split_w1(P.x, idx, a.w1s); split_w1(P.y, idx + 1, a.w1s); split_w1(P.z, idx + 2, a.w1s); split_w1(P.w, idx + 3, a.w1s);
            }
        }
    }
    if (bid == ADAMF_T2 + ADAMF_T3 && tid == 0) { a.ad->applies = a.ad->ticks; a.ad->pver[0] += 1; a.ad->wverc[0] = a.ad->pver[0]; }
    if (bid == ADAMF_T2 + ADAMF_T3 && tid < (int)(a.n & 3)) {
        const long long q = (n4 << 2) + tid;
        float mm = a.m[q], vv = a.v[q];
        mm += (a.g[q] - mm) * omb1; vv += (a.g[q] * a.g[q] - vv) * omb2;
        a.p[q] -= (mm * alpha) / (sqrtf(vv) + eps);
        a.m[q] = mm; a.v[q] = vv;
    }
    if (a.split && bid == ADAMF_T2 + ADAMF_T3 && tid == 0) fb_flag_wait(&a.split->env_done, a.split_val, &a.split->timeouts[4]);
}

__global__ void init_params_kernel(float *__restrict__ p, long long n, NetOff off, int FC, int A, int dueling,
                                   uint32_t seed_lo, uint32_t seed_hi) {
    const long long i = (long long)blockIdx.x * blockDim.x + threadIdx.x;
    if (i >= n) return;
    bool bias = (i >= OFF_B1 && i < OFF_W2) || (i >= OFF_B2 && i < OFF_W3) || (i >= OFF_B3 && i < OFF_WF1) ||
                (i >= off.bf1 && i < off.bf1 + FC) || (i >= off.bq && i < off.bq + A) || (dueling && i == off.bv);
    if (bias) { p[i] = 0.01f; return; }
    for (uint32_t ctr = 0;; ctr++) {
        const fb_u4 r = fb_philox(seed_lo, seed_hi, (uint32_t)i, ctr, FB_STREAM_INIT, 0u);
        const float u1 = ((r.x >> 8) + 1) * (1.0f / 16777216.0f), u2 = (r.y >> 8) * (1.0f / 16777216.0f);
        const float z = sqrtf(-2.f * logf(u1)) * cosf(6.28318530717958647692f * u2);
        if (fabsf(z) <= 2.f) { p[i] = 0.01f * z; return; }
    }
}

}

#ifndef FB_ADAM_GRID
#define FB_ADAM_GRID 1024
#endif
constexpr int ADAM_GRID = FB_ADAM_GRID;

struct fb_qnet {
    int arch, FC, A, max_batch;
    long long n;
    NetOff off;
    float *params[2], *adam_m, *adam_v, *grad, *slabs;
    float *slabs1;
    uint16_t *w1s[2];
    uint4 *wsp[2];
    uint16_t *zeros;
    uint16_t *a1s, *a3s;
    int nsplit;
    int nsplit_train;
    bool adam_ticked;
    AdamDev *adam;
    float *p1, *h2, *h3, *hf, *q;
    float *qpart;
    unsigned long long *ring_fo;
    hipEvent_t grad_ev;
    hipEvent_t grad_ev_recorded;
    uint8_t *amax;
    float *dhf, *dh3, *dh2, *dp1;
    float *gmax;
    int zmax;
    float *hf_act, *hp_act;
    FbSplitCtx *split;
    C51Sup sup;
    float kappa;
    float *c51_dl, *c51_xs, *c51_lt;
    NetOff hoff;
    float *heff[2];
    bool noisy;
    long long ntot;
    NoisyNet nnet;
    float *mst[2], *nz[2];
    int act_noise;
    float *nz_zero, *ht;
    uint4 *wsig;
    uint16_t *a3n;
    int *sig_seen;
    bool split_adam_pending;
};

static NetOff make_off(int FC, int A, int dueling) {
    NetOff o;
    o.bf1 = OFF_WF1 + 1600 * FC;
    int p = o.bf1 + FC;
    if (dueling) { o.wv = p; o.bv = p + FC; p = o.bv + 1; } else { o.wv = 0; o.bv = 0; }
    o.wq = p; o.bq = p + FC * A; o.n = o.bq + A;
    return o;
}

static NetOff make_off_c51d(int FC, int A, int N) {
    NetOff o;
    o.bf1 = OFF_WF1 + 1600 * FC;
    o.wv = o.bf1 + FC; o.bv = o.wv + FC * N;
    o.wq = o.bv + N; o.bq = o.wq + FC * A * N; o.n = o.bq + A * N;
    return o;
}
static bool is_c51d(const fb_qnet *h) { return h->arch == FB_ARCH_C51_DUELING || h->arch == FB_ARCH_QR_DUELING; }
static bool is_qr(const fb_qnet *h) { return h->arch == FB_ARCH_QR || h->arch == FB_ARCH_QR_DUELING; }
static const float *head_base(const fb_qnet *h, const float *params) {
    if (!is_c51d(h)) return params;
    return h->heff[params == h->params[1] ? 1 : 0] - h->off.bf1;
}
static void c51d_fold(fb_qnet *h, int which, hipStream_t st) {
    if (!is_c51d(h)) return;
    const C51dFoldArgs F{h->params[which], h->heff[which], h->off, h->FC, h->A, h->sup.N};
    const int tot = h->FC + (h->FC + 1) * h->A * h->sup.N;
    hipLaunchKernelGGL(c51d_fold_kernel, dim3((tot + 255) / 256), dim3(256), 0, st, F);
}

static float *master(const fb_qnet *h, int which) { return h->noisy ? h->mst[which] : h->params[which]; }
static void noisy_materialise(fb_qnet *h, int which, int q0, bool bump, hipStream_t st) {
    if (!h->noisy) return;
    const NoisyMat a{h->mst[which], h->params[which], h->nz[which], h->nnet, q0, which, bump ? h->adam : nullptr};
    hipLaunchKernelGGL(noisy_mat_kernel, dim3((unsigned)((h->n - q0 + 255) / 256)), dim3(256), 0, st, a);
}
static void env_noise_invalidate(fb_qnet *h, int which, hipStream_t st) {
    if (h->noisy && which == 0) (void)hipMemsetD32Async((hipDeviceptr_t)h->sig_seen, -1, 1, st);
}
static void noisy_sgrad(fb_qnet *h, float *g, hipStream_t st) {
    if (!h->noisy) return;
    hipLaunchKernelGGL(noisy_sgrad_kernel, dim3((unsigned)((h->n - OFF_WF1 + 255) / 256)), dim3(256), 0, st, g, (const float *)h->nz[0], h->nnet);
}

static int qnet_create(int arch, int fc_width, int n_actions, const C51Sup &sup, int max_batch, fb_qnet_t *out, float sigma0 = -1.f);

extern "C" int fb_qnet_create(int arch, int fc_width, int n_actions, int max_batch, fb_qnet_t *out) {
    FB_REQUIRE(out, "fb_qnet_create: out is NULL");
    FB_REQUIRE(arch != FB_ARCH_C51, "fb_qnet_create: a C51 net is made by fb_qnet_create_c51 (it needs the support)");
    FB_REQUIRE(arch != FB_ARCH_C51_DUELING, "fb_qnet_create: a dueling C51 net is made by fb_qnet_create_c51_dueling (it needs the support)");
    FB_REQUIRE(arch != FB_ARCH_QR && arch != FB_ARCH_QR_DUELING, "fb_qnet_create: a QR net is made by fb_qnet_create_qr (it needs N and kappa)");
    FB_REQUIRE(arch == FB_ARCH_PLAIN || arch == FB_ARCH_DUELING, "fb_qnet_create: arch must be 0 or 1");
    FB_REQUIRE(fc_width >= 128 && fc_width <= 4096 && fc_width % 128 == 0, "fb_qnet_create: fc_width must be a multiple of 128");
    FB_REQUIRE(n_actions >= 1 && n_actions <= MAXA, "fb_qnet_create: n_actions must be in 1..%d", MAXA);
    FB_REQUIRE(max_batch >= 1 && max_batch <= (1 << 20), "fb_qnet_create: max_batch out of range");
    return qnet_create(arch, fc_width, n_actions, C51Sup{0, 0.f, 0.f, 0.f}, max_batch, out);
}

static int c51_create(const char *fn, int arch, int fc_width, int n_actions, int n_atoms, float v_min, float v_max, int max_batch, fb_qnet_t *out,
                      float sigma0 = -1.f) {
    FB_REQUIRE(out, "%s: out is NULL", fn);
    FB_REQUIRE(fc_width >= 128 && fc_width <= 4096 && fc_width % 128 == 0, "%s: fc_width must be a multiple of 128", fn);
    FB_REQUIRE(n_actions >= 1 && n_actions <= MAXA, "%s: n_actions must be in 1..%d", fn, MAXA);
    FB_REQUIRE(n_atoms >= 2 && n_atoms <= FB_C51_MAX_ATOMS, "%s: n_atoms=%d outside 2..%d", fn, n_atoms, FB_C51_MAX_ATOMS);
    FB_REQUIRE(n_actions * n_atoms <= 128, "%s: n_actions * n_atoms = %d exceeds 128", fn, n_actions * n_atoms);
    FB_REQUIRE(isfinite(v_min) && isfinite(v_max) && v_min < v_max, "%s: the support needs finite v_min < v_max (got %g, %g)",
               fn, (double)v_min, (double)v_max);
    FB_REQUIRE(max_batch >= 1 && max_batch <= (1 << 20), "%s: max_batch out of range", fn);
    const float dz = (v_max - v_min) / (float)(n_atoms - 1);
    FB_REQUIRE(isfinite(dz) && dz > 0.f, "%s: the atom spacing (v_max - v_min) / (n_atoms - 1) is not a positive finite float", fn);
    return qnet_create(arch, fc_width, n_actions, C51Sup{n_atoms, v_min, v_max, dz}, max_batch, out, sigma0);
}

extern "C" int fb_qnet_create_c51(int fc_width, int n_actions, int n_atoms, float v_min, float v_max, int max_batch, fb_qnet_t *out) {
    return c51_create("fb_qnet_create_c51", FB_ARCH_C51, fc_width, n_actions, n_atoms, v_min, v_max, max_batch, out);
}

extern "C" int fb_qnet_create_c51_dueling(int fc_width, int n_actions, int n_atoms, float v_min, float v_max, int max_batch, fb_qnet_t *out) {
    return c51_create("fb_qnet_create_c51_dueling", FB_ARCH_C51_DUELING, fc_width, n_actions, n_atoms, v_min, v_max, max_batch, out);
}

extern "C" int fb_qnet_create_c51_noisy(int arch, int fc_width, int n_actions, int n_atoms, float v_min, float v_max, float sigma0, int max_batch,
// ... 81 lines not shown
    alloc((void **)&h->gmax, (size_t)(fc_width / 16) * 4);
    alloc((void **)&h->hf_act, S * fc_width * 4 * FC1_SP_KS); alloc((void **)&h->hp_act, sizeof(float) * (size_t)(h->n - h->off.bf1));
    if (sup.N) { alloc((void **)&h->c51_dl, Bm * 64 * 4); alloc((void **)&h->c51_xs, Bm * fc_width * 4); alloc((void **)&h->c51_lt, Bm * 4); }
    if (is_c51d(h)) for (int w = 0; w < 2; w++) alloc((void **)&h->heff[w], sizeof(float) * (size_t)(h->hoff.n - h->off.bf1));
    if (e != hipSuccess) {
        fb_set_error(e == hipErrorOutOfMemory ? FB_ERR_NOMEM : FB_ERR_HIP, "fb_qnet_create: %s", hipGetErrorString(e));
        fb_qnet_destroy(h);
        return e == hipErrorOutOfMemory ? FB_ERR_NOMEM : FB_ERR_HIP;
    }
    *out = h;
    {
        AdamDev a; memset(&a, 0, sizeof(a));
        a.pver[0] = a.pver[1] = 1;
        if (hipMemcpy(h->adam, &a, sizeof(a), hipMemcpyHostToDevice) != hipSuccess) { fb_qnet_destroy(h); *out = nullptr; return fb_set_error(FB_ERR_HIP, "fb_qnet_create: hipMemcpy failed"); }
    }
    return fb_qnet_set_hparams(h, 1e-6f, 0.9f, 0.999f, 1e-8f);
}

extern "C" int fb_qnet_destroy(fb_qnet_t h) {
    if (!h) return FB_OK;
    void *ptrs[] = {h->zeros, h->wsp[0], h->wsp[1], h->a1s, h->a3s, h->w1s[0], h->w1s[1], h->params[0], h->params[1], h->adam_m, h->adam_v, h->grad, h->slabs, h->slabs1, h->adam, h->p1, h->amax, h->h2,
                    h->h3, h->hf, h->q, h->qpart, h->dhf, h->dh3, h->dh2, h->dp1, h->ring_fo, h->gmax, h->hf_act, h->hp_act,
                    h->c51_dl, h->c51_xs, h->c51_lt, h->heff[0], h->heff[1], h->mst[0], h->mst[1], h->nz[0], h->nz[1],
                    h->nz_zero, h->wsig, h->a3n, h->ht, h->sig_seen};
    if (h->split) {
        FbSplitCtx *c = h->split;
        if (c->tstream) { (void)hipStreamSynchronize(c->tstream); (void)hipStreamDestroy(c->tstream); }
        if (c->f) (void)hipFree(c->f);
        delete c;
    }
    for (void *p : ptrs) if (p) (void)hipFree(p);
    delete h;
    return FB_OK;
}

__global__ void flag_wait_kernel(const unsigned long long *flag, unsigned long long v, unsigned *timeouts) { if (threadIdx.x == 0) fb_flag_wait(flag, v, timeouts); }
__global__ void flag_set_kernel(unsigned long long *flag, unsigned long long v) { fb_flag_store(flag, v); }

FbSplitCtx *fb_qnet_split_ctx(fb_qnet_t h) {
    if (!h) return nullptr;
    if (h->split) return h->split->tstream ? h->split : nullptr;
    FbSplitCtx *c = new FbSplitCtx();
    memset(c, 0, sizeof(*c));
    h->split = c;
    int lo = 0, hi = 0;
    bool ok = hipMalloc((void **)&c->f, sizeof(FbSplitFlags)) == hipSuccess && hipMemset(c->f, 0, sizeof(FbSplitFlags)) == hipSuccess;
    hipStream_t ts = nullptr;
    ok = ok && hipDeviceGetStreamPriorityRange(&lo, &hi) == hipSuccess && hipStreamCreateWithPriority(&ts, hipStreamNonBlocking, lo) == hipSuccess;
    if (!ok) { (void)hipGetLastError(); return nullptr; }
    c->tstream = ts;
    return c;
}

int fb_split_probe(FbSplitCtx *c, void *stream) {
    if (!c || !c->tstream) return 0;
    if (c->probed_stream == stream && c->seq > 0) return c->probed_ok;
    int lo = 0, hi = 0, ok = 0;
    if (hipDeviceGetStreamPriorityRange(&lo, &hi) != hipSuccess) return 0;
    c->tstream = fb_side_stream_beside(reinterpret_cast<hipStream_t>(stream), lo, c->tstream, &ok);
    c->probed_stream = stream; c->probed_ok = ok;
    return ok;
}

int fb_split_wait(const FbSplitCtx *c, const unsigned long long *flag, unsigned long long v, void *stream) {
    hipLaunchKernelGGL(flag_wait_kernel, dim3(1), dim3(64), 0, fb_stream(stream), flag, v, &c->f->timeouts[1]);
    FB_LAUNCH_CHECK();
    return FB_OK;
}

int fb_split_set(const FbSplitCtx *, unsigned long long *flag, unsigned long long v, void *stream) {
    hipLaunchKernelGGL(flag_set_kernel, dim3(1), dim3(1), 0, fb_stream(stream), flag, v);
    FB_LAUNCH_CHECK();
    return FB_OK;
}

extern "C" int fb_qnet_split_stats(fb_qnet_t h, int64_t *steps_host, int64_t *clean_host) {
    FB_REQUIRE(h && steps_host && clean_host, "fb_qnet_split_stats: NULL argument");
    *steps_host = 0; *clean_host = 0;
    if (!h->split || !h->split->tstream) return FB_OK;
    FB_CHECK_HIP(hipDeviceSynchronize());
    unsigned v[8] = {0};
    FB_CHECK_HIP(hipMemcpy(v, &h->split->f->clean_count, sizeof(v), hipMemcpyDeviceToHost));
    FB_REQUIRE(!(v[1] | v[2] | v[3] | v[4] | v[5] | v[6]), "fb_qnet_split_stats: waits between the two chains of the split schedule gave up after 1 s (the draw %u, the side stream's entry %u, "
               "the fc1 backward launch's gate %u, the conv backward launch's gate %u, the Adam launch's last wait %u): the results of those steps are not to be trusted", v[1], v[2], v[3], v[4], v[5]);
    *steps_host = (int64_t)h->split->seq; *clean_host = (int64_t)v[0];
    return FB_OK;
}

extern "C" int fb_qnet_num_params(fb_qnet_t h, int64_t *n_host) {
    FB_REQUIRE(h && n_host, "fb_qnet_num_params: NULL argument");
    *n_host = h->ntot;
    return FB_OK;
}

extern "C" int fb_qnet_set_hparams(fb_qnet_t h, float lr, float beta1, float beta2, float eps) {
    FB_REQUIRE(h, "fb_qnet_set_hparams: NULL handle");
    FB_CHECK_HIP(hipDeviceSynchronize());
    AdamDev a;
    FB_CHECK_HIP(hipMemcpy(&a, h->adam, sizeof(a), hipMemcpyDeviceToHost));
    const bool fresh = a.b1 == 0.f && a.b2 == 0.f;
    a.lr = lr; a.b1 = beta1; a.b2 = beta2; a.eps = eps;
    if (fresh) { a.b1pow = beta1; a.b2pow = beta2; a.alpha = 0.f; }
    FB_CHECK_HIP(hipMemcpy(h->adam, &a, sizeof(a), hipMemcpyHostToDevice));
    return FB_OK;
}

extern "C" int fb_qnet_overflow_count(fb_qnet_t h, int reset, int64_t *count_host) {
    FB_REQUIRE(h && count_host, "fb_qnet_overflow_count: NULL argument");
    FB_CHECK_HIP(hipDeviceSynchronize());
    unsigned v = 0;
    FB_CHECK_HIP(hipMemcpy(&v, &h->adam->ovf, sizeof(v), hipMemcpyDeviceToHost));
    if (reset && v) { const unsigned z = 0; FB_CHECK_HIP(hipMemcpy(&h->adam->ovf, &z, sizeof(z), hipMemcpyHostToDevice)); }
    *count_host = (int64_t)v;
    return FB_OK;
}

extern "C" int fb_qnet_set_inference_dtype(fb_qnet_t h, int dtype) {
    FB_REQUIRE(h && (dtype == FB_DTYPE_F32 || dtype == FB_DTYPE_BF16), "fb_qnet_set_inference_dtype: dtype must be FB_DTYPE_F32 or FB_DTYPE_BF16");
    h->nsplit = dtype == FB_DTYPE_BF16 ? 1 : 3;
    return FB_OK;
}

extern "C" int fb_qnet_set_train_dtype(fb_qnet_t h, int dtype) {
    FB_REQUIRE(h && (dtype == FB_DTYPE_F32 || dtype == FB_DTYPE_BF16), "fb_qnet_set_train_dtype: dtype must be FB_DTYPE_F32 or FB_DTYPE_BF16");
    h->nsplit_train = dtype == FB_DTYPE_BF16 ? 1 : 3;
    return FB_OK;
}

static void resplit_now(fb_qnet *h, int which, hipStream_t st) {
    const int items = wsplit_items(h->FC);
    hipLaunchKernelGGL(wsplit_kernel, dim3((items + 255) / 256), dim3(256), 0, st, h->params[which], h->wsp[which], h->FC,
                       (const unsigned *)&h->adam->pver[which], (const unsigned *)&h->adam->wver[which]);
    hipLaunchKernelGGL(mark_split_kernel, dim3(1), dim3(1), 0, st, h->adam, which);
}

extern "C" int fb_qnet_init_params(fb_qnet_t h, int which, uint64_t seed, void *stream) {
    FB_REQUIRE(h && (which == 0 || which == 1), "fb_qnet_init_params: bad argument");
    hipLaunchKernelGGL(init_params_kernel, dim3((unsigned)((h->n + 255) / 256)), dim3(256), 0, fb_stream(stream),
                       master(h, which), h->n, h->off, h->FC, h->sup.N ? h->A * h->sup.N : h->A, h->arch == FB_ARCH_DUELING || is_c51d(h), (uint32_t)seed,
                       (uint32_t)(seed >> 32));
    if (is_c51d(h)) {
        const float b = 0.01f;
        uint32_t bits;
        memcpy(&bits, &b, 4);
        FB_CHECK_HIP(hipMemsetD32Async((hipDeviceptr_t)(master(h, which) + h->off.bv), (int)bits, (size_t)h->sup.N, fb_stream(stream)));
    }
    if (h->noisy)
        hipLaunchKernelGGL(noisy_sigma_init_kernel, dim3((unsigned)((h->n - OFF_WF1 + 255) / 256)), dim3(256), 0, fb_stream(stream), h->mst[which], h->nnet);
    noisy_materialise(h, which, 0, false, fb_stream(stream));
    env_noise_invalidate(h, which, fb_stream(stream));
    c51d_fold(h, which, fb_stream(stream));
    hipLaunchKernelGGL(w1_split_kernel, dim3(32), dim3(256), 0, fb_stream(stream), h->params[which], h->w1s[which], &h->adam->pver[which]);
    resplit_now(h, which, fb_stream(stream));
    FB_LAUNCH_CHECK();
    return FB_OK;
}

extern "C" int fb_qnet_load_params(fb_qnet_t h, int which, const float *flat, void *stream) {
    FB_REQUIRE(h && flat && (which == 0 || which == 1), "fb_qnet_load_params: bad argument");
    FB_CHECK_HIP(hipMemcpyAsync(master(h, which), flat, sizeof(float) * (size_t)h->ntot, hipMemcpyDeviceToDevice, fb_stream(stream)));
    noisy_materialise(h, which, 0, false, fb_stream(stream));
    env_noise_invalidate(h, which, fb_stream(stream));
    hipLaunchKernelGGL(w1_split_kernel, dim3(32), dim3(256), 0, fb_stream(stream), h->params[which], h->w1s[which], &h->adam->pver[which]);
    c51d_fold(h, which, fb_stream(stream));
    resplit_now(h, which, fb_stream(stream));
    FB_LAUNCH_CHECK();
    return FB_OK;
}

extern "C" int fb_qnet_store_params(fb_qnet_t h, int which, float *flat, void *stream) {
    FB_REQUIRE(h && flat && (which == 0 || which == 1), "fb_qnet_store_params: bad argument");
    FB_CHECK_HIP(hipMemcpyAsync(flat, master(h, which), sizeof(float) * (size_t)h->ntot, hipMemcpyDeviceToDevice, fb_stream(stream)));
    return FB_OK;
}

extern "C" int fb_qnet_get_adam_state(fb_qnet_t h, float *m, float *v, float *beta_pows_host) {
    FB_REQUIRE(h, "fb_qnet_get_adam_state: NULL handle");
    FB_CHECK_HIP(hipDeviceSynchronize());
    const size_t nb = sizeof(float) * (size_t)h->ntot;
    if (m) FB_CHECK_HIP(hipMemcpy(m, h->adam_m, nb, hipMemcpyDeviceToDevice));
    if (v) FB_CHECK_HIP(hipMemcpy(v, h->adam_v, nb, hipMemcpyDeviceToDevice));
    if (beta_pows_host) {
        AdamDev a;
        FB_CHECK_HIP(hipMemcpy(&a, h->adam, sizeof(a), hipMemcpyDeviceToHost));
        beta_pows_host[0] = a.b1pow; beta_pows_host[1] = a.b2pow;
    }
    return FB_OK;
}

extern "C" int fb_qnet_set_adam_state(fb_qnet_t h, const float *m, const float *v, const float *beta_pows_host) {
    FB_REQUIRE(h, "fb_qnet_set_adam_state: NULL handle");
    FB_CHECK_HIP(hipDeviceSynchronize());
    const size_t nb = sizeof(float) * (size_t)h->ntot;
    if (m) FB_CHECK_HIP(hipMemcpy(h->adam_m, m, nb, hipMemcpyDeviceToDevice));
    if (v) FB_CHECK_HIP(hipMemcpy(h->adam_v, v, nb, hipMemcpyDeviceToDevice));
    if (beta_pows_host) {
        AdamDev a;
        FB_CHECK_HIP(hipMemcpy(&a, h->adam, sizeof(a), hipMemcpyDeviceToHost));
        a.b1pow = beta_pows_host[0]; a.b2pow = beta_pows_host[1];
        FB_CHECK_HIP(hipMemcpy(h->adam, &a, sizeof(a), hipMemcpyHostToDevice));
    }
    return FB_OK;
}

enum KernelId {
    K_CONV1 = 0, K_CONV2, K_CONV3, K_FC1, K_HEAD, K_LOSS, K_FC1_BWD, K_CONV3_BWD, K_CONV2_BWD, K_CONV1_DW, K_SLAB, K_ADAM,
    K_COUNT
};

struct Plan {
    Slices sl; int ns;
    bool nib;
    uint8_t *actions; float epsilon; uint64_t seed, step;
    bool train;
    int algo, B; const uint8_t *s, *a, *t; const float *r, *isw; double gamma;
    float *loss, *abs_err, *y, *G; bool apply_adam, tick;
    FbHeadRider *head_rider;
    const FbSampleRider *sample_rider;
    const FbRingSrc *ring;
    const FbSplitCtx *split;
    bool any_rows;
    float *probs;
    bool no_head;
};

#include <type_traits>
template <int V> using IntTag = std::integral_constant<int, V>;
template <class F> static void with_nsp(int nsp, F f) { if (nsp == 3) f(IntTag<3>{}); else f(IntTag<1>{}); }
template <class F> static void with_bool(bool b, F f) { if (b) f(std::true_type{}); else f(std::false_type{}); }
template <class F> static void with_actions(int A, F f) { if (A == 2) f(IntTag<2>{}); else f(IntTag<MAXA>{}); }

template <class T> static void put_seed_words(T &c, uint64_t seed, uint64_t step) {
    c.seed_lo = (uint32_t)seed; c.seed_hi = (uint32_t)(seed >> 32);
    c.step_lo = (uint32_t)step; c.step_hi = (uint32_t)(step >> 32);
}

struct PlanCtx {
    int only; hipStream_t st;
    int maxc, total;
    bool big, trunk, fused, c51;
    int nsp, stot; size_t pl1, pl2;
};
static bool runs(const PlanCtx &c, int id) { return c.only < 0 || c.only == id; }

static PlanCtx plan_ctx(const fb_qnet *h, const Plan &p, int only, hipStream_t st) {
    PlanCtx c{only, st, 0, 0};
    for (int z = 0; z < p.ns; z++) { if (p.sl.s[z].count > c.maxc) c.maxc = p.sl.s[z].count; c.total += p.sl.s[z].count; }
    c.big = c.maxc >= 256 || p.any_rows;
    c.nsp = p.train ? h->nsplit_train : h->nsplit;
    c.stot = 3 * h->max_batch; c.pl1 = (size_t)c.stot * 3200; c.pl2 = (size_t)c.stot * 1600;
    c.trunk = p.ring != nullptr;
    c.fused = c.big && p.nib && !p.train && !c.trunk && p.ns == 1;
    c.c51 = h->sup.N > 0;
    return c;
}

static C23T trunk_args(fb_qnet *h, const Plan &p, const PlanCtx &c, SplitJob *job) {
    C23T c23t;
    memset(job, 0, sizeof(*job)); memset(&c23t, 0, sizeof(c23t));
    job->FC = h->FC;
    c23t.sl = p.sl; c23t.p1 = h->p1; c23t.h2 = h->h2; c23t.h3 = h->h3; c23t.ovf = &h->adam->ovf;
    for (int z = 0; z < p.ns; z++) {
        const int which = p.sl.s[z].params == h->params[1] ? 1 : 0;
        c23t.w[z] = h->wsp[which] + WSP_W2;
        if (c.only < 0) {
            job->params[which] = h->params[which]; job->wsp[which] = h->wsp[which];
            job->pver[which] = &h->adam->pver[which]; job->wverc[which] = &h->adam->wverc[which];
            c23t.pver[which] = &h->adam->pver[which]; c23t.wverc[which] = &h->adam->wverc[which];
        }
    }
    return c23t;
}

static void ring_trunk(fb_qnet *h, const Plan &p, const PlanCtx &c) {
    SplitJob job;
    C23T c23t = trunk_args(h, p, c, &job);
    if (c.big) { c23t.a3s = h->a3s; c23t.pl3 = c.pl2; }
    c23t.ring = *p.ring; c23t.p1o = h->p1; c23t.amax = h->amax; c23t.ring_fo = h->ring_fo;
    const bool w16 = c.maxc * p.ns <= 256;
    const bool nst = p.ring->c.nstep > 1;
    with_nsp(c.nsp, [&](auto ns) { with_bool(w16, [&](auto w) { with_bool(nst, [&](auto nv) {
        constexpr bool W16 = decltype(w)::value;
        hipLaunchKernelGGL((conv23_t_kernel<decltype(ns)::value, true, W16, decltype(nv)::value>), dim3(c.maxc, p.ns), dim3(W16 ? 1024 : 512), 0, c.st, c23t);
    }); }); });
}

static int large_pass(fb_qnet *h, const Plan &p, const PlanCtx &c, int *z) {
    const int z0 = *z;
    int z1 = z0 + 1;
    while (z1 < p.ns && p.sl.s[z1].params == p.sl.s[z0].params && p.sl.s[z1].count == p.sl.s[z0].count && p.sl.s[z1].s_off == p.sl.s[z1 - 1].s_off + p.sl.s[z1 - 1].count) z1++;
    const Slice s0 = p.sl.s[z0];
    const int which = s0.params == h->params[1] ? 1 : 0, row0 = s0.s_off, rows = s0.count * (z1 - z0);
    const unsigned *pver = c.only < 0 ? &h->adam->pver[which] : nullptr;
    unsigned *wver = c.only < 0 ? &h->adam->wver[which] : nullptr;
    Slice sl = s0;
    sl.count = rows;
    C1Side side;
    memset(&side, 0, sizeof(side));
    if (z1 - z0 > 1) { side.per = s0.count; side.st1 = p.sl.s[z0 + 1].states; side.st2 = z1 - z0 > 2 ? p.sl.s[z0 + 2].states : p.sl.s[z0 + 1].states; }
    if (p.train) { side.p1 = h->p1; side.amax = h->amax; }
    const int t1p = (rows * 100 + 7) / 8, gsp = min(256, (t1p + C1_WAVES - 1) / C1_WAVES);
    if (!c.trunk && !c.fused && runs(c, K_CONV1))
        hipLaunchKernelGGL(conv1_sp_kernel, dim3(gsp), dim3(64 * C1_WAVES), 0, c.st, sl, (const uint8_t *)h->zeros, h->a1s, c.pl1, c.nsp, h->wsp[which], h->FC, pver, (const unsigned *)wver, side, &h->adam->ovf);
    C23Args c23{h->a1s + (size_t)row0 * 3200, c.pl1, h->wsp[which] + WSP_W2, s0.params + OFF_B2, s0.params + OFF_B3, h->a3s + (size_t)row0 * 1600, c.pl2, rows, pver, wver, c.only < 0 ? &h->adam->wverc[which] : nullptr,
                p.train ? h->h2 + (size_t)row0 * 1600 : nullptr, p.train ? h->h3 + (size_t)row0 * 1600 : nullptr,
                s0.states, s0.w1s, s0.params + OFF_B1, s0.params, h->wsp[which], h->FC, &h->adam->ovf};
    Fc1Args af{h->a3s + (size_t)row0 * 1600, c.pl2, h->zeros, h->wsp[which] + WSP_WF1, (c.fused ? h->hf_act : h->hf) + (size_t)row0 * h->FC, c.stot, rows, h->FC,
               c.fused ? pver : nullptr, c.fused ? wver : nullptr, nullptr, 0,
               c.fused ? head_base(h, s0.params) + h->off.bf1 : nullptr, c.fused ? h->hp_act : nullptr, c.fused ? (int)(h->hoff.n - h->off.bf1) : 0,
               c.fused && p.split && c.only < 0 ? &p.split->f->trunk_done : nullptr, p.split ? p.split->seq : 0};
    if (c.trunk && z1 < p.ns && rows % 128 == 0) {
        int z2 = z1 + 1;
        while (z2 < p.ns && p.sl.s[z2].params == p.sl.s[z1].params && p.sl.s[z2].s_off == p.sl.s[z2 - 1].s_off + p.sl.s[z2 - 1].count) z2++;
        const Slice sn = p.sl.s[z1];
        if (z2 == p.ns && sn.s_off == row0 + rows && sn.params != s0.params) {
            int rows2 = 0;
            for (int z = z1; z < z2; z++) rows2 += p.sl.s[z].count;
            af.w2 = h->wsp[sn.params == h->params[1] ? 1 : 0] + WSP_WF1; af.m_split = rows; af.M = rows + rows2;
            z1 = z2;
        }
    }
    *z = z1;
    const dim3 gc((rows + 4) / 5), gf(((af.M + 127) / 128) * (h->FC / 64) * FC1_SP_KS);
    if (c.fused && p.split && c.only < 0 && gc.x > 256 && gc.x % 256 != 0) { c23.round_flag = &p.split->f->last_round; c23.round_val = p.split->seq; c23.round_blk = (int)(gc.x / 256) * 256; }
    with_nsp(c.nsp, [&](auto ns) {
        if (!c.trunk && runs(c, K_CONV2))
            with_bool(c.fused, [&](auto fu) { hipLaunchKernelGGL((conv23_sp_kernel<decltype(ns)::value, 5, decltype(fu)::value>), gc, dim3(512), 0, c.st, c23); });
        if (runs(c, K_FC1)) hipLaunchKernelGGL(fc1_sp_kernel<decltype(ns)::value>, gf, dim3(256), 0, c.st, af);
    });
    if (c.fused && (c.only < 0 || c.only == K_FC1) && (long long)af.hp_n > (long long)gf.x * 256) {
        const size_t done = (size_t)gf.x * 256;
        FB_CHECK_HIP(hipMemcpyAsync(h->hp_act + done, af.hp_src + done, sizeof(float) * ((size_t)af.hp_n - done), hipMemcpyDeviceToDevice, c.st));
    }
    return FB_OK;
}

static void small_forward(fb_qnet *h, const Plan &p, const PlanCtx &c) {
    if (!c.trunk) {
        SplitJob job;
        const C23T c23t = trunk_args(h, p, c, &job);
        const int t1 = (c.maxc * 100 + 7) / 8;
        if (runs(c, K_CONV1))
            with_bool(p.nib, [&](auto nib) { hipLaunchKernelGGL(conv1_pool_kernel<decltype(nib)::value>, dim3((t1 + 3) / 4, 1, p.ns), dim3(256), 0, c.st, p.sl, h->p1, h->amax, job); });
        if (runs(c, K_CONV2))
            with_nsp(c.nsp, [&](auto ns) { hipLaunchKernelGGL((conv23_t_kernel<decltype(ns)::value, false>), dim3(c.maxc, p.ns), dim3(512), 0, c.st, c23t); });
    }
    if (runs(c, K_FC1)) {
        FkArgs fa;
        fa.sl = p.sl; fa.h3 = h->h3; fa.hf = h->hf; fa.qpart = p.train && !c.c51 ? h->qpart : nullptr; fa.FC = h->FC; fa.A = h->A;
        fa.dueling = h->arch == FB_ARCH_DUELING; fa.stot = c.stot; fa.off = h->off;
        hipLaunchKernelGGL(fc1_fk_kernel, dim3((c.maxc + 15) / 16, h->FC / 16, p.ns), dim3(512), 0, c.st, fa);
    }
}

static void launch_dist_head(const fb_qnet *h, const C51HeadArgs &H, int rows, hipStream_t st) {
    with_actions(h->A, [&](auto a) {
        if (is_qr(h)) hipLaunchKernelGGL(qr_head_kernel<decltype(a)::value>, dim3((rows + 3) / 4), dim3(256), 0, st, H);
        else hipLaunchKernelGGL(c51_head_kernel<decltype(a)::value>, dim3((rows + 3) / 4), dim3(256), 0, st, H);
    });
}

static void head_stage(fb_qnet *h, const Plan &p, const PlanCtx &c) {
    if (c.c51 && !p.train && !p.no_head && runs(c, K_HEAD)) {
        C51HeadArgs H;
        H.sl = p.sl; H.nslices = p.ns; H.params = nullptr;
        for (int z = 0; z < p.ns; z++) H.sl.s[z].params = head_base(h, p.sl.s[z].params);
        C51Core &C = H.c;
        C.hf = c.fused ? h->hf_act : h->hf; C.stot = c.stot; C.nks = c.big ? FC1_SP_KS : 1; C.q = h->q; C.probs = p.probs; C.FC = h->FC; C.A = h->A;
        C.off = h->hoff; C.sup = h->sup; C.actions = p.actions; C.epsilon = p.epsilon;
        put_seed_words(C, p.seed, p.step); C.key_of = nullptr; C.stream = FB_STREAM_EPS;
        if (p.head_rider) {
            memset(p.head_rider, 0, sizeof(*p.head_rider));
            p.head_rider->c.hf = C.hf; p.head_rider->c.stot = c.stot; p.head_rider->c.nks = C.nks;
            p.head_rider->params = c.fused ? h->hp_act - h->off.bf1 : H.sl.s[0].params;
        } else launch_dist_head(h, H, c.total, c.st);
    }
    if (!c.c51 && !(!c.big && p.train) && runs(c, K_HEAD)) {
        HeadArgs H;
        H.sl = p.sl; H.nslices = p.ns;
        HeadCore &C = H.c;
        C.hf = c.fused ? h->hf_act : h->hf; C.stot = c.stot; C.nks = c.big ? FC1_SP_KS : 1; C.q = h->q; C.FC = h->FC; C.A = h->A;
        C.dueling = h->arch == FB_ARCH_DUELING; C.off = h->off; C.actions = p.actions; C.epsilon = p.epsilon;
        put_seed_words(C, p.seed, p.step);
        if (p.head_rider) { p.head_rider->c = C; p.head_rider->params = c.fused ? h->hp_act - h->off.bf1 : p.sl.s[0].params; p.head_rider->on = 1; p.head_rider->on_arrival = nullptr; p.head_rider->arrival_val = 0; }
        else hipLaunchKernelGGL(head_kernel, dim3((c.total + 3) / 4), dim3(256), 0, c.st, H);
    }
}

static void loss_stage(fb_qnet *h, const Plan &p, const PlanCtx &c) {
    const int B = p.B, FC = h->FC;
    if (!c.c51) {
        LossArgs L;
        L.algo = p.algo; L.B = B; L.FC = FC; L.A = h->A; L.dueling = h->arch == FB_ARCH_DUELING; L.off = h->off;
        L.params = h->params[0]; L.q = h->q; L.hf = h->hf; L.stot = c.stot; L.nks = FC1_SP_KS; L.act = p.a; L.rew = p.r; L.term = p.t; L.isw = p.isw;
        L.gamma = p.gamma; L.grad = p.G; L.dhf = h->dhf; L.loss = p.loss; L.abs_err = p.abs_err; L.y_out = p.y; L.gmax = h->gmax;
        L.adam = h->adam; L.tick = p.tick;
        hipLaunchKernelGGL(loss_head_kernel, dim3(FC / 16), dim3(256), 0, c.st, L);
        return;
    }
    const bool pw = is_per_algo(p.algo);
    auto shared = [&](auto &L) {
        L.B = B; L.FC = FC; L.A = h->A; L.nks = c.big ? FC1_SP_KS : 1; L.stot = c.stot; L.off = h->hoff;
        L.p_on = head_base(h, h->params[0]); L.p_next = head_base(h, p.sl.s[1].params);
        L.p_tgt = head_base(h, p.ns > 2 ? p.sl.s[2].params : p.sl.s[1].params);
        L.hf = h->hf; L.act = p.a; L.rew = p.r; L.term = p.t; L.gamma = p.gamma;
        L.dl = h->c51_dl; L.xs = h->c51_xs; L.lterm = h->c51_lt; L.dhf = h->dhf;
        L.isw = pw ? p.isw : nullptr; L.abs_err = pw ? p.abs_err : nullptr;
    };
    with_actions(h->A, [&](auto a) { with_bool(pw, [&](auto w) {
        if (is_qr(h)) {
            QRLossArgs L;
            shared(L);
            L.algo = is_double_qr(p.algo) ? FB_ALGO_QR_DOUBLE : FB_ALGO_QR; L.N = h->sup.N; L.kappa = h->kappa;
            hipLaunchKernelGGL((qr_loss_kernel<decltype(a)::value, decltype(w)::value>), dim3((B + 3) / 4), dim3(256), 0, c.st, L);
        } else {
            C51LossArgs L;
            shared(L);
            L.algo = is_double_c51(p.algo) ? FB_ALGO_C51_DOUBLE : FB_ALGO_C51; L.sup = h->sup;
            hipLaunchKernelGGL((c51_loss_kernel<decltype(a)::value, decltype(w)::value>), dim3((B + 3) / 4), dim3(256), 0, c.st, L);
        }
    }); });
    const C51GradArgs gA{B, FC, h->A, h->sup.N, h->off, h->c51_dl, h->c51_xs, h->c51_lt, h->dhf, p.a, p.G, p.loss, h->gmax, h->adam, p.tick};
    if (is_c51d(h)) hipLaunchKernelGGL(c51d_grad_kernel, dim3(FC / 16), dim3(256), 0, c.st, gA);
    else hipLaunchKernelGGL(c51_grad_kernel, dim3(FC / 16), dim3(256), 0, c.st, gA);
}

static void fc1_backward(fb_qnet *h, const Plan &p, const PlanCtx &c) {
    const int B = p.B, FC = h->FC;
    if (!c.big && !c.c51) {
        const int ndx1 = ((B + 31) / 32) * 50;
        Bw1Args L;
        L.algo = p.algo; L.B = B; L.FC = FC; L.A = h->A; L.dueling = h->arch == FB_ARCH_DUELING; L.stot = c.stot; L.n_dx = ndx1; L.off = h->off;
        L.params = h->params[0]; L.pnext = p.sl.s[1].params; L.ptarget = p.ns > 2 ? p.sl.s[2].params : p.sl.s[1].params;
        L.hf = h->hf; L.qpart = h->qpart; L.h3 = h->h3; L.act = p.a; L.rew = p.r; L.term = p.t; L.isw = p.isw; L.gamma = p.gamma;
        L.grad = p.G; L.dh3 = h->dh3; L.loss = p.loss; L.abs_err = p.abs_err; L.y_out = p.y;
        L.adam = h->adam; L.tick = p.tick; L.rb = h->nsplit_train == 1;
        L.gate = p.split && c.only < 0 ? FbGate{&p.split->f->trunk_done, p.split->seq, &p.split->f->timeouts[2]} : FbGate{nullptr, 0, nullptr};
        hipLaunchKernelGGL(fc1_bwd2_kernel, dim3(ndx1 + (FC / 32) * 7 + (L.gate.flag ? 1 : 0)), dim3(512), 0, c.st, L);
        return;
    }
    const int ndx = ((B + 31) / 32) * 50, ntile = ndx + 50 * (FC / 32);
    const bool std_shape = FC == 512 && B == 256;
    with_nsp(h->nsplit_train, [&](auto ns) { with_bool(std_shape, [&](auto s) {
        hipLaunchKernelGGL((fc1_bwd_big_kernel<decltype(ns)::value, decltype(s)::value ? 4 : 0, decltype(s)::value ? 2 : 0>), dim3(ntile), dim3(512), 0, c.st,
                           ndx, h->params[0], h->h3, h->dhf, h->dh3, p.G, B, FC, (const float *)h->gmax, &h->adam->ovf);
    }); });
}

struct SlabCounts { int z1, z3; };
static SlabCounts conv_backward(fb_qnet *h, const Plan &p, const PlanCtx &c, int span0, int span1) {
    const int B = p.B, FC = h->FC, rbt = h->nsplit_train == 1;
    int z3 = min((B * 25 + 255) / 256, h->zmax);
    const size_t ss = CONV_PARAMS;
    const AdamSpan span{master(h, 0), h->adam_m, h->adam_v, p.G, h->adam, span0, span1};
    const FbGate gate_fc1 = p.split && c.only < 0 ? FbGate{&p.split->f->fc1_done, p.split->seq, &p.split->f->timeouts[3]} : FbGate{nullptr, 0, nullptr};
    const FbSampleRider srider = p.sample_rider ? *p.sample_rider : FbSampleRider{};
    const bool fold1 = 2 * B > h->zmax;
    const int fold = (2 * B + h->zmax - 1) / h->zmax;
    const int z1 = fold1 ? (2 * B + fold - 1) / fold : 2 * B;
    const int n_adam5 = (span1 - span0 + 511) / 512;
    const BxArgs bx{h->dh3, h->h2, h->p1, h->dh2, h->dp1, h->wsp[0] + wsp_w3t(FC), h->wsp[0] + wsp_w2t(FC)};
    const Dw1Ring dr{p.ring ? p.ring->c.bits : nullptr, h->ring_fo};
    float *s1 = fold1 ? h->slabs1 : h->slabs;
    const size_t st1 = fold1 ? (size_t)CONV1_PARAMS : ss;
    const bool dwg = c.big && B % 16 == 0;
    const int zt3 = dwg ? 0 : z3, zt2 = zt3;
    const bool bw = !c.big && B <= h->zmax;
    if (bw) {
        z3 = B;
        const dim3 g(BW_WGS * B + n_adam5 + (srider.k ? 1 : 0) + (gate_fc1.flag ? 1 : 0));
        if (runs(c, K_CONV3_BWD)) with_nsp(h->nsplit_train, [&](auto ns) { with_bool(p.ring != nullptr, [&](auto r) {
            hipLaunchKernelGGL((conv_bw_kernel<decltype(ns)::value, decltype(r)::value>), g, dim3(512), 0, c.st,
                               bx, B, h->slabs, ss, s1, st1, p.s, (const uint8_t *)h->amax, dr, n_adam5, span, srider, rbt, gate_fc1);
        }); });
    } else {
        const dim3 g3(B + 38 * zt3 + n_adam5 + (srider.k ? 1 : 0)), g2(34 * zt2 + 2 * B + (gate_fc1.flag ? 1 : 0));
        if (runs(c, K_CONV3_BWD)) with_nsp(h->nsplit_train, [&](auto ns) {
            hipLaunchKernelGGL(conv_bx_kernel<decltype(ns)::value>, g3, dim3(512), 0, c.st, bx, B, zt3, h->slabs, ss, n_adam5, span, srider, rbt);
        });
        if (dwg) {
            z3 = B / 16;
            const int n3 = z3 * 4, n2 = z3 * 8;
            if (runs(c, K_CONV2_BWD)) with_nsp(h->nsplit_train, [&](auto ns) {
                hipLaunchKernelGGL(conv_dwg_kernel<decltype(ns)::value>, dim3(n3 + n2), dim3(512), 0, c.st, n3, h->h2, h->dh3, h->p1, h->dh2, h->slabs, ss, &h->adam->ovf);
            });
        }
        if (runs(c, K_CONV2_BWD)) with_bool(p.ring != nullptr, [&](auto r) {
            hipLaunchKernelGGL((conv_dw21_kernel<2, decltype(r)::value>), g2, dim3(512), 0, c.st,
                               zt2, B, h->p1, h->dh2, p.s, h->dp1, h->amax, h->slabs, ss, s1, st1, rbt, dr, gate_fc1);
        });
    }
    if (fold1 && runs(c, K_CONV2_BWD)) hipLaunchKernelGGL(slab_fold_kernel, dim3((CONV1_PARAMS + 255) / 256, z1), dim3(256), 0, c.st, h->slabs1, 2 * B, fold, h->slabs, ss);
    return SlabCounts{z1, z3};
}

static void reduce_or_adam(fb_qnet *h, const Plan &p, const PlanCtx &c, SlabCounts z, int span1) {
    if (p.split && c.only < 0) h->split_adam_pending = !p.apply_adam;
    if (!p.apply_adam && runs(c, K_SLAB)) hipLaunchKernelGGL(slab_reduce_kernel, dim3((CONV_PARAMS / 4 + 255) / 256), dim3(256), 0, c.st, h->slabs, (size_t)CONV_PARAMS, z.z1, z.z3, z.z3, p.G);
    if (c.only < 0) noisy_sgrad(h, p.G, c.st);
    if (p.apply_adam && runs(c, K_ADAM)) {
        AdamFused af;
        af.p = master(h, 0); af.m = h->adam_m; af.v = h->adam_v; af.g = p.G; af.n = h->ntot; af.ad = h->adam;
        af.slabs = h->slabs; af.slab_stride = CONV_PARAMS; af.z1 = z.z1; af.z2 = af.z3 = z.z3;
        af.w1s = h->w1s[0]; af.wsp = h->wsp[0]; af.FC = h->FC; af.tail0 = span1;
        const long long nrest4 = OFF_W2 / 4 + (OFF_W3 - OFF_B2) / 4 + (OFF_WF1 - OFF_B3) / 4 + (h->ntot / 4 - span1);
        af.lanes = 4;
        af.split = p.split && c.only < 0 ? p.split->f : nullptr; af.split_val = p.split ? p.split->seq : 0;
        af.n_rest = (int)((nrest4 * af.lanes + 255) / 256);
        hipLaunchKernelGGL(adam_fused_kernel, dim3(ADAMF_T2 + ADAMF_T3 + af.n_rest), dim3(256), 0, c.st, af);
        noisy_materialise(h, 0, 0, false, c.st);
        c51d_fold(h, 0, c.st);
    }
}

static int run_plan(fb_qnet *h, const Plan &p, int only, hipStream_t st) {
    const PlanCtx c = plan_ctx(h, p, only, st);
    if (c.trunk && runs(c, K_CONV2)) ring_trunk(h, p, c);
    if (c.big) {
        for (int z = 0; z < p.ns;) {
            const int rc = large_pass(h, p, c, &z);
            if (rc != FB_OK) return rc;
        }
    } else small_forward(h, p, c);
    head_stage(h, p, c);
    if (p.train) {
        if (p.tick) h->adam_ticked = !p.apply_adam;
        if ((c.c51 || c.big) && runs(c, K_LOSS)) loss_stage(h, p, c);
        if (runs(c, K_FC1_BWD)) fc1_backward(h, p, c);
        if (!p.apply_adam && only < 0) {
            h->grad_ev_recorded = nullptr;
            if (h->grad_ev) { FB_CHECK_HIP(hipEventRecord(h->grad_ev, st)); h->grad_ev_recorded = h->grad_ev; }
        }
        const int span0 = OFF_WF1 / 4, span1 = p.apply_adam ? (OFF_WF1 + 1600 * h->FC) / 4 : span0;
        reduce_or_adam(h, p, c, conv_backward(h, p, c, span0, span1), span1);
    }
    FB_LAUNCH_CHECK();
    return FB_OK;
}

static Plan forward_plan(fb_qnet *h, int which, const uint8_t *states, int n) {
    Plan p; memset(&p, 0, sizeof(p));
    p.sl.s[0] = Slice{h->params[which], states, 0, n, h->w1s[which], 0};
    p.ns = 1;
    return p;
}

static bool rows_ok(const fb_qnet *h, int n) { return n >= 1 && n <= 3 * h->max_batch; }
static int copy_q(fb_qnet *h, int n, float *q, hipStream_t st) {
    if (q) FB_CHECK_HIP(hipMemcpyAsync(q, h->q, sizeof(float) * (size_t)n * h->A, hipMemcpyDeviceToDevice, st));
    return FB_OK;
}

extern "C" int fb_qnet_forward(fb_qnet_t h, int which, const uint8_t *states, int batch, float *q, void *stream) {
    FB_REQUIRE(h && states && q && (which == 0 || which == 1), "fb_qnet_forward: bad argument");
    FB_REQUIRE(rows_ok(h, batch), "fb_qnet_forward: batch %d exceeds 3*max_batch", batch);
    int rc = run_plan(h, forward_plan(h, which, states, batch), -1, fb_stream(stream));
    if (rc != FB_OK) return rc;
    return copy_q(h, batch, q, fb_stream(stream));
}

static int act_states(fb_qnet *h, const uint8_t *states, bool nib, int n, float epsilon, uint64_t seed, uint64_t step, uint8_t *actions, float *q,
                      hipStream_t st) {
    Plan p = forward_plan(h, 0, states, n);
    p.nib = nib;
    p.actions = actions; p.epsilon = epsilon; p.seed = seed; p.step = step;
    int rc = run_plan(h, p, -1, st);
    if (rc != FB_OK) return rc;
    return copy_q(h, n, q, st);
}

extern "C" int fb_qnet_act(fb_qnet_t h, const uint8_t *states, int n, float epsilon, uint64_t seed, uint64_t step,
                           uint8_t *actions, float *q, void *stream) {
    FB_REQUIRE(h && states && actions, "fb_qnet_act: NULL argument");
    FB_REQUIRE(rows_ok(h, n), "fb_qnet_act: n %d exceeds 3*max_batch", n);
    return act_states(h, states, false, n, epsilon, seed, step, actions, q, fb_stream(stream));
}

extern "C" int fb_qnet_act_nib(fb_qnet_t h, const uint8_t *nib_states, int n, float epsilon, uint64_t seed, uint64_t step,
                               uint8_t *actions, float *q, void *stream) {
    FB_REQUIRE(h && nib_states && actions, "fb_qnet_act_nib: NULL argument");
    FB_REQUIRE(rows_ok(h, n), "fb_qnet_act_nib: n %d exceeds 3*max_batch", n);
    return act_states(h, nib_states, true, n, epsilon, seed, step, actions, q, fb_stream(stream));
}

int fb_qnet_num_actions(fb_qnet_t h) { return h ? h->A : 0; }
int fb_qnet_is_c51(fb_qnet_t h) { return h && h->sup.N > 0 && !is_qr(h); }
int fb_qnet_is_qr(fb_qnet_t h) { return h && is_qr(h); }
int fb_qnet_is_dist(fb_qnet_t h) { return h && h->sup.N > 0; }
extern "C" int fb_qnet_is_noisy(fb_qnet_t h) { return h && h->noisy ? 1 : 0; }

extern "C" int fb_qnet_reset_noise(fb_qnet_t h, int which, uint64_t seed, uint64_t step, int mode, void *stream) {
    FB_REQUIRE(h && (which == 0 || which == 1), "fb_qnet_reset_noise: bad argument");
    FB_REQUIRE(h->noisy, "fb_qnet_reset_noise: not a noisy net (fb_qnet_create_c51_noisy)");
    FB_REQUIRE(mode == FB_NOISE_SAMPLE || mode == FB_NOISE_MEAN, "fb_qnet_reset_noise: mode must be FB_NOISE_SAMPLE or FB_NOISE_MEAN (got %d)", mode);
    hipStream_t st = fb_stream(stream);
    hipLaunchKernelGGL(noise_draw_kernel, dim3((h->nnet.nz + 255) / 256), dim3(256), 0, st, h->nz[which], h->nnet.nz, (uint32_t)seed, (uint32_t)(seed >> 32),
                       (uint32_t)step, (uint32_t)(step >> 32) * 2u + (uint32_t)which, mode == FB_NOISE_MEAN ? 1 : 0);
    noisy_materialise(h, which, OFF_WF1, true, st);
    c51d_fold(h, which, st);
    FB_LAUNCH_CHECK();
    return FB_OK;
}

extern "C" int fb_qnet_get_noise(fb_qnet_t h, int which, float *out) {
    FB_REQUIRE(h && out && (which == 0 || which == 1), "fb_qnet_get_noise: bad argument");
    FB_REQUIRE(h->noisy, "fb_qnet_get_noise: not a noisy net (fb_qnet_create_c51_noisy)");
    FB_CHECK_HIP(hipDeviceSynchronize());
    FB_CHECK_HIP(hipMemcpy(out, h->nz[which], sizeof(float) * (size_t)h->nnet.nz, hipMemcpyDefault));
    return FB_OK;
}

extern "C" int fb_qnet_set_acting_noise(fb_qnet_t h, int mode) {
    FB_REQUIRE(h, "fb_qnet_set_acting_noise: NULL handle");
    FB_REQUIRE(h->noisy, "fb_qnet_set_acting_noise: not a noisy net (fb_qnet_create_c51_noisy)");
    FB_REQUIRE(mode == FB_ACT_NOISE_SHARED || mode == FB_ACT_NOISE_PER_ENV,
               "fb_qnet_set_acting_noise: mode must be FB_ACT_NOISE_SHARED or FB_ACT_NOISE_PER_ENV (got %d)", mode);
    h->act_noise = mode;
    return FB_OK;
}
int fb_qnet_acting_noise(fb_qnet_t h) { return h && h->noisy ? h->act_noise : FB_ACT_NOISE_SHARED; }

int fb_qnet_check_env_noise(fb_qnet_t h, int n, const char *who) {
    FB_REQUIRE(h, "%s: NULL handle", who);
    FB_REQUIRE(h->noisy, "%s: per-env acting noise needs a noisy net (fb_qnet_create_c51_noisy)", who);
    FB_REQUIRE(h->nsplit == 3, "%s: per-env acting noise takes FB_DTYPE_F32 inference only (the net is set to FB_DTYPE_BF16)", who);
    FB_REQUIRE(rows_ok(h, n), "%s: n %d exceeds 3*max_batch", who, n);
    FB_REQUIRE((unsigned long long)n * (unsigned long long)h->nnet.nz < (1ull << 32), "%s: n * nz = %d * %d must stay below 2^32 (the noise counter)",
               who, n, h->nnet.nz);
    return FB_OK;
}

static int act_env_noise(fb_qnet *h, const uint8_t *nib_states, int n, float epsilon, uint64_t seed, uint64_t step, uint8_t *actions, float *q,
                         bool restore, hipStream_t st) {
    FB_REQUIRE(h && nib_states && actions, "fb_qnet_act_nib_env_noise: NULL argument");
    int rc = fb_qnet_check_env_noise(h, n, "fb_qnet_act_nib_env_noise");
    if (rc != FB_OK) return rc;
    const NoisyMat mu{h->mst[0], h->params[0], h->nz_zero, h->nnet, OFF_WF1, 0, h->adam};
    hipLaunchKernelGGL(noisy_mat_kernel, dim3((unsigned)((h->n - OFF_WF1 + 255) / 256)), dim3(256), 0, st, mu);
    c51d_fold(h, 0, st);
    Plan p = forward_plan(h, 0, nib_states, n);
    p.nib = true; p.no_head = true;
    rc = run_plan(h, p, -1, st);
    if (rc != FB_OK) return rc;
    const bool sp = n >= 256;
    const int FC = h->FC, stot = 3 * h->max_batch;
    const size_t pl2 = (size_t)stot * 1600;
    const float *sig = h->mst[0] + h->n - OFF_WF1;
    hipLaunchKernelGGL(env_noise_sigsplit_kernel, dim3((unsigned)((200 * FC + 255) / 256)), dim3(256), 0, st, sig, h->wsig, FC, (const AdamDev *)h->adam,
                       (const int *)h->sig_seen);
    EnvScale es{sp ? h->a3s : nullptr, sp ? nullptr : h->h3, pl2, h->a3n, n, h->nnet.nz, 0, 0, 0, 0, h->adam, h->sig_seen, &h->adam->ovf};
    put_seed_words(es, seed, step);
    hipLaunchKernelGGL(env_noise_scale_kernel, dim3((unsigned)(((long long)n * 800 + 255) / 256)), dim3(256), 0, st, es);
    const Fc1Args af{h->a3n, pl2, h->zeros, h->wsig + WSP_WF1, h->ht, stot, n, FC, nullptr, nullptr, nullptr, 0, nullptr, nullptr, 0, nullptr, 0};
    hipLaunchKernelGGL(fc1_sp_kernel<3>, dim3(((n + 127) / 128) * (FC / 64) * FC1_SP_KS), dim3(256), 0, st, af);
    EnvNoiseHead H;
    H.hf = sp ? h->hf_act : h->hf; H.ht = h->ht; H.stot = stot; H.nks = sp ? FC1_SP_KS : 1;
    H.P = head_base(h, h->params[0]); H.hoff = h->hoff; H.sig = sig; H.off = h->off; H.N = h->nnet;
    H.n = n; H.FC = FC; H.A = h->A; H.sup = h->sup; H.q = h->q; H.actions = actions; H.epsilon = epsilon;
    put_seed_words(H, seed, step); H.key_of = nullptr; H.stream = FB_STREAM_EPS;
    with_actions(h->A, [&](auto a) { with_bool(is_c51d(h), [&](auto d) {
        hipLaunchKernelGGL((env_noise_head_kernel<decltype(a)::value, decltype(d)::value>), dim3((n + ENH_WAVES - 1) / ENH_WAVES), dim3(64 * ENH_WAVES), 0, st, H);
    }); });
    if (restore) {
        noisy_materialise(h, 0, OFF_WF1, true, st);
        c51d_fold(h, 0, st);
    }
    FB_LAUNCH_CHECK();
    return copy_q(h, n, q, st);
}

extern "C" int fb_qnet_act_nib_env_noise(fb_qnet_t h, const uint8_t *nib_states, int n, float epsilon, uint64_t seed, uint64_t step,
                                         uint8_t *actions, float *q, void *stream) {
    return act_env_noise(h, nib_states, n, epsilon, seed, step, actions, q, true, fb_stream(stream));
}
int fb_qnet_act_nib_env_noise_keep(fb_qnet_t h, const uint8_t *nib_states, int n, float epsilon, uint64_t seed, uint64_t step,
                                   uint8_t *actions, float *q, void *stream) {
    return act_env_noise(h, nib_states, n, epsilon, seed, step, actions, q, false, fb_stream(stream));
}

extern "C" int fb_qnet_get_support(fb_qnet_t h, int *n_atoms_host, float *v_min_host, float *v_max_host) {
    FB_REQUIRE(h && n_atoms_host && v_min_host && v_max_host, "fb_qnet_get_support: NULL argument");
    *n_atoms_host = is_qr(h) ? 0 : h->sup.N; *v_min_host = h->sup.vmin; *v_max_host = h->sup.vmax;
    return FB_OK;
}

extern "C" int fb_qnet_get_quantiles(fb_qnet_t h, int *n_quantiles_host, float *kappa_host) {
    FB_REQUIRE(h && n_quantiles_host && kappa_host, "fb_qnet_get_quantiles: NULL argument");
    *n_quantiles_host = is_qr(h) ? h->sup.N : 0; *kappa_host = is_qr(h) ? h->kappa : 0.f;
    return FB_OK;
}

extern "C" int fb_qnet_forward_quantiles(fb_qnet_t h, int which, const uint8_t *states, int batch, float *theta, void *stream) {
    FB_REQUIRE(h && states && theta && (which == 0 || which == 1), "fb_qnet_forward_quantiles: bad argument");
    FB_REQUIRE(is_qr(h), "fb_qnet_forward_quantiles: not a QR net (fb_qnet_create_qr)");
    FB_REQUIRE(rows_ok(h, batch), "fb_qnet_forward_quantiles: batch %d exceeds 3*max_batch", batch);
    Plan p = forward_plan(h, which, states, batch);
    p.probs = theta;
    return run_plan(h, p, -1, fb_stream(stream));
}

extern "C" int fb_qnet_forward_dist(fb_qnet_t h, int which, const uint8_t *states, int batch, float *probs, void *stream) {
    FB_REQUIRE(h && states && probs && (which == 0 || which == 1), "fb_qnet_forward_dist: bad argument");
    FB_REQUIRE(h->sup.N > 0 && !is_qr(h), "fb_qnet_forward_dist: not a C51 net (fb_qnet_create_c51; a QR net: fb_qnet_forward_quantiles)");
    FB_REQUIRE(rows_ok(h, batch), "fb_qnet_forward_dist: batch %d exceeds 3*max_batch", batch);
    Plan p = forward_plan(h, which, states, batch);
    p.probs = probs;
    return run_plan(h, p, -1, fb_stream(stream));
}

int fb_qnet_c51_eval_head(fb_qnet_t h, const FbHeadRider *hd, int n, const int32_t *key_of, void *stream) {
    FB_REQUIRE(h && hd && key_of && h->sup.N > 0, "fb_qnet_c51_eval_head: bad argument");
    C51HeadArgs H;
    memset(&H, 0, sizeof(H));
    H.sl.s[0] = Slice{hd->params, nullptr, 0, n, nullptr, 0}; H.nslices = 1; H.params = hd->params;
    C51Core &C = H.c;
    C.hf = hd->c.hf; C.stot = hd->c.stot; C.nks = hd->c.nks; C.q = hd->c.q; C.probs = nullptr; C.FC = h->FC; C.A = h->A;
    C.off = h->hoff; C.sup = h->sup; C.actions = hd->c.actions; C.epsilon = hd->c.epsilon;
    C.seed_lo = hd->c.seed_lo; C.seed_hi = hd->c.seed_hi; C.step_lo = hd->c.step_lo; C.step_hi = hd->c.step_hi;
    C.key_of = key_of; C.stream = FB_STREAM_EVAL;
    launch_dist_head(h, H, n, fb_stream(stream));
    FB_LAUNCH_CHECK();
    return FB_OK;
}
int fb_qnet_max_rows(fb_qnet_t h) { return h ? 3 * h->max_batch : 0; }
hipStream_t fb_qnet_side_stream(fb_qnet_t h) { return h && h->split ? h->split->tstream : nullptr; }

int fb_qnet_eval_trunk(fb_qnet_t h, const uint8_t *nib_states, int n, FbHeadRider *head, void *stream) {
    FB_REQUIRE(h && nib_states && head, "fb_qnet_eval_trunk: NULL argument");
    FB_REQUIRE(rows_ok(h, n), "fb_qnet_eval_trunk: n %d exceeds 3*max_batch", n);
    Plan p = forward_plan(h, 0, nib_states, n);
    p.nib = true; p.any_rows = true;
    p.head_rider = head;
    return run_plan(h, p, -1, fb_stream(stream));
}

extern "C" int fb_eval_q(fb_qnet_t h, const uint8_t *nib_states, int n, float *q, void *stream) {
    FB_REQUIRE(h && nib_states && q, "fb_eval_q: NULL argument");
    FB_REQUIRE(rows_ok(h, n), "fb_eval_q: n %d exceeds 3*max_batch", n);
    Plan p = forward_plan(h, 0, nib_states, n);
    p.nib = true; p.any_rows = true;
    int rc = run_plan(h, p, -1, fb_stream(stream));
    if (rc != FB_OK) return rc;
    return copy_q(h, n, q, fb_stream(stream));
}

int fb_qnet_check_step(fb_qnet_t h, int n_envs, int train_batch) {
    FB_REQUIRE(h, "fb_vec_step: NULL net");
    FB_REQUIRE(n_envs >= 1 && n_envs <= 3 * h->max_batch, "fb_vec_step: %d envs exceed 3*max_batch of the net", n_envs);
    FB_REQUIRE(train_batch < 0 || (train_batch >= 1 && train_batch <= h->max_batch && train_batch <= MAXTB),
               "fb_vec_step: batch %d exceeds min(max_batch, %d)", train_batch, MAXTB);
    return FB_OK;
}

int fb_qnet_act_nib_rider(fb_qnet_t h, const uint8_t *nib_states, int n, float epsilon, uint64_t seed, uint64_t step,
                          uint8_t *actions, FbHeadRider *head, void *stream, const FbSplitCtx *split) {
    FB_REQUIRE(h && nib_states && actions && head, "fb_qnet_act_nib_rider: NULL argument");
    FB_REQUIRE(h->sup.N == 0, "fb_qnet_act_nib_rider: a C51 or QR net's head does not ride in the env launch");
    FB_REQUIRE(rows_ok(h, n), "fb_qnet_act_nib: n %d exceeds 3*max_batch", n);
    Plan p = forward_plan(h, 0, nib_states, n);
    p.nib = true;
    p.actions = actions; p.epsilon = epsilon; p.seed = seed; p.step = step;
    p.head_rider = head;
    p.split = split;
    return run_plan(h, p, -1, fb_stream(stream));
}

extern "C" int fb_qnet_apply_adam(fb_qnet_t h, const float *flat_grad, void *stream) {
    FB_REQUIRE(h && flat_grad, "fb_qnet_apply_adam: NULL argument");
    hipStream_t st = fb_stream(stream);
    hipStreamCaptureStatus cap = hipStreamCaptureStatusNone;
    (void)hipStreamIsCapturing(st, &cap);
    if (!h->adam_ticked || cap != hipStreamCaptureStatusNone) hipLaunchKernelGGL(adam_tick_kernel, dim3(1), dim3(1), 0, st, h->adam);
    h->adam_ticked = false;
    AdamFused af;
    af.p = master(h, 0); af.m = h->adam_m; af.v = h->adam_v; af.g = flat_grad; af.n = h->ntot; af.ad = h->adam;
    af.slabs = nullptr; af.slab_stride = 0; af.z1 = af.z2 = af.z3 = 0;
    af.w1s = h->w1s[0]; af.wsp = h->wsp[0]; af.FC = h->FC; af.tail0 = OFF_WF1 / 4;
    af.n_rest = ADAM_GRID; af.lanes = 1;
    af.split = h->split_adam_pending && h->split && h->split->tstream ? h->split->f : nullptr; af.split_val = af.split ? h->split->seq : 0;
    h->split_adam_pending = false;
    hipLaunchKernelGGL(adam_fused_kernel, dim3(ADAMF_T2 + ADAMF_T3 + af.n_rest), dim3(256), 0, st, af);
    noisy_materialise(h, 0, 0, false, st);
    c51d_fold(h, 0, st);
    FB_LAUNCH_CHECK();
    return FB_OK;
}

extern "C" int fb_qnet_set_grad_event(fb_qnet_t h, void *event) {
    FB_REQUIRE(h, "fb_qnet_set_grad_event: NULL handle");
    h->grad_ev = (hipEvent_t)event;
    return FB_OK;
}

void *fb_qnet_get_grad_event(fb_qnet_t h) { return h ? (void *)h->grad_ev : nullptr; }
void *fb_qnet_take_grad_event_recorded(fb_qnet_t h) {
    if (!h) return nullptr;
    void *e = (void *)h->grad_ev_recorded;
    h->grad_ev_recorded = nullptr;
    return e;
}

extern "C" int64_t fb_qnet_grad_split(fb_qnet_t h) { return h ? (int64_t)CONV_PARAMS : 0; }

extern "C" int fb_qnet_sync_target(fb_qnet_t h, void *stream) {
    FB_REQUIRE(h, "fb_qnet_sync_target: NULL handle");
    FB_CHECK_HIP(hipMemcpyAsync(master(h, 1), master(h, 0), sizeof(float) * (size_t)h->ntot, hipMemcpyDeviceToDevice, fb_stream(stream)));
    FB_CHECK_HIP(hipMemcpyAsync(h->w1s[1], h->w1s[0], 3 * 8192 * 2, hipMemcpyDeviceToDevice, fb_stream(stream)));
    hipLaunchKernelGGL(bump_pver_kernel, dim3(1), dim3(1), 0, fb_stream(stream), h->adam, 1);
    noisy_materialise(h, 1, 0, false, fb_stream(stream));
    resplit_now(h, 1, fb_stream(stream));
    c51d_fold(h, 1, fb_stream(stream));
    FB_LAUNCH_CHECK();
    return FB_OK;
}

static int train_plan(fb_qnet *h, int algo, int B, const uint8_t *s, const uint8_t *a, const float *r, const uint8_t *s2,
                      const uint8_t *t, const float *isw, double gamma, float *loss, float *abs_err, float *q_target,
                      float *flat_grad, Plan *out, const FbRingSrc *ring = nullptr) {
    FB_REQUIRE(h && a && r && t && loss && (ring || (s && s2)), "fb_qnet_train_step: NULL argument");
    FB_REQUIRE(algo >= 0 && algo <= FB_ALGO_QR_DOUBLE_PER, "fb_qnet_train_step: unknown algo %d", algo);
    {
        const bool c51a = is_c51_algo(algo), qra = is_qr_algo(algo);
        FB_REQUIRE(c51a == (h->sup.N > 0 && !is_qr(h)), c51a ? "fb_qnet_train_step: algo %d (C51) needs a C51 net (fb_qnet_create_c51)"
                                                : "fb_qnet_train_step: a C51 net trains with FB_ALGO_C51, FB_ALGO_C51_PER, FB_ALGO_C51_DOUBLE_PER "
                                                  "or FB_ALGO_C51_DOUBLE only (got algo %d)", algo);
        FB_REQUIRE(qra == is_qr(h), qra ? "fb_qnet_train_step: algo %d (QR) needs a QR net (fb_qnet_create_qr)"
                                        : "fb_qnet_train_step: a QR net trains with FB_ALGO_QR, FB_ALGO_QR_DOUBLE, FB_ALGO_QR_PER or "
                                          "FB_ALGO_QR_DOUBLE_PER only (got algo %d)", algo);
    }
    FB_REQUIRE(B >= 1 && B <= h->max_batch && B <= MAXTB, "fb_qnet_train_step: batch %d exceeds min(max_batch, %d)", B, MAXTB);
    FB_REQUIRE(algo != FB_ALGO_PG || (B <= 128 && !ring && gamma >= (double)B), "fb_qnet_train_step: FB_ALGO_PG takes chunks of <= 128 gathered states and gamma = the whole batch's sample count (>= %d)", B);
    FB_REQUIRE(!is_per_algo(algo) || isw, "fb_qnet_train_step: PER needs isw (algo %d)", algo);
    Plan p; memset(&p, 0, sizeof(p));
    p.ns = 2;
    p.sl.s[0] = Slice{h->params[0], s, 0, B, h->w1s[0], 0};
    if (algo == FB_ALGO_DQN || algo == FB_ALGO_PG) p.sl.s[1] = Slice{h->params[0], s2, B, B, h->w1s[0], 1};
    else if (algo == FB_ALGO_DOUBLE || is_double_c51(algo) || is_double_qr(algo)) { p.sl.s[1] = Slice{h->params[0], s2, B, B, h->w1s[0], 1}; p.sl.s[2] = Slice{h->params[1], s2, 2 * B, B, h->w1s[1], 1}; p.ns = 3; }
    else p.sl.s[1] = Slice{h->params[1], s2, B, B, h->w1s[1], 1};
    p.sl.rb = h->nsplit_train == 1;
    p.train = true; p.algo = algo; p.B = B; p.s = s; p.a = a; p.r = r; p.t = t; p.isw = isw; p.gamma = gamma;
    p.loss = loss; p.abs_err = abs_err; p.y = q_target;
    p.G = flat_grad ? flat_grad : h->grad;
    p.apply_adam = flat_grad == nullptr; p.tick = true;
    p.ring = ring;
    if (ring && ring->c.nstep > 1)
        for (int z = 0; z < p.ns; z++) if (p.sl.s[z].fshift) p.sl.s[z].fshift = ring->c.nstep;
    *out = p;
    return FB_OK;
}

int fb_qnet_train_step_ring(fb_qnet_t h, int algo, int B, const FbRingSrc *ring, const float *isw, double gamma, float *loss, float *abs_err,
                            float *flat_grad, void *stream, const FbSampleRider *rider, const FbSplitCtx *split) {
    FB_REQUIRE(h && ring && ring->idx && ring->a && ring->r && ring->t, "fb_qnet_train_step_ring: NULL argument");
    Plan p;
    int rc = train_plan(h, algo, B, nullptr, ring->a, ring->r, nullptr, ring->t, isw, gamma, loss, abs_err, nullptr, flat_grad, &p, ring);
    if (rc != FB_OK) return rc;
    p.sample_rider = rider;
    p.split = split;
    return run_plan(h, p, -1, fb_stream(stream));
}

__global__ void wsplit_both_kernel(const float *__restrict__ p0, const float *__restrict__ p1, uint4 *__restrict__ w0, uint4 *__restrict__ w1, int FC,
                                   const AdamDev *__restrict__ ad) {
    const int n = blockIdx.y;
    if (ad->pver[n] == ad->wver[n]) return;
    wsplit_item(n ? p1 : p0, n ? w1 : w0, FC, blockIdx.x * blockDim.x + threadIdx.x);
}
__global__ void mark_split_both_kernel(AdamDev *ad) {
    const int n = threadIdx.x;
    if (n < 2) { ad->wver[n] = ad->pver[n]; ad->wverc[n] = ad->pver[n]; }
}

int fb_qnet_refresh_planes(fb_qnet_t h, void *stream) {
    FB_REQUIRE(h, "fb_qnet_refresh_planes: NULL handle");
    const int items = wsplit_items(h->FC);
    hipLaunchKernelGGL(wsplit_both_kernel, dim3((items + 255) / 256, 2), dim3(256), 0, fb_stream(stream), h->params[0], h->params[1], h->wsp[0], h->wsp[1],
                       h->FC, (const AdamDev *)h->adam);
    hipLaunchKernelGGL(mark_split_both_kernel, dim3(1), dim3(64), 0, fb_stream(stream), h->adam);
    FB_LAUNCH_CHECK();
    return FB_OK;
}

int fb_qnet_profile_ring(fb_qnet_t h, int kernel, int reps, int algo, int B, const FbRingSrc *ring, float *loss, void *stream) {
    FB_REQUIRE(h && ring && kernel >= 0 && kernel < K_COUNT && reps >= 1, "fb_qnet_profile_ring: bad argument");
    FB_REQUIRE(!is_per_algo(algo), "fb_qnet_profile_ring: uniform memories only");
    Plan p;
    int rc = train_plan(h, algo, B, nullptr, ring->a, ring->r, nullptr, ring->t, nullptr, 0.99, loss, nullptr, nullptr, nullptr, &p, ring);
    if (rc != FB_OK) return rc;
    p.tick = false;
    rc = fb_qnet_refresh_planes(h, stream);
    for (int i = 0; i < reps && rc == FB_OK; i++) rc = run_plan(h, p, kernel, fb_stream(stream));
    return rc;
}

extern "C" int fb_qnet_train_step(fb_qnet_t h, int algo, int B, const uint8_t *s, const uint8_t *a, const float *r,
                                  const uint8_t *s2, const uint8_t *t, const float *isw, double gamma, float *loss,
                                  float *abs_err, float *q_target, float *flat_grad, void *stream) {
    Plan p;
    int rc = train_plan(h, algo, B, s, a, r, s2, t, isw, gamma, loss, abs_err, q_target, flat_grad, &p);
    if (rc != FB_OK) return rc;
    return run_plan(h, p, -1, fb_stream(stream));
}

extern "C" int fb_qnet_profile_kernel(fb_qnet_t h, int kernel, int reps, int algo, int B, const uint8_t *s, const uint8_t *a,
                                      const float *r, const uint8_t *s2, const uint8_t *t, float *loss, void *stream) {
    FB_REQUIRE(kernel >= 0 && kernel < K_COUNT && reps >= 1, "fb_qnet_profile_kernel: bad kernel id / reps");
    Plan p;
    int rc = FB_OK;
    if (algo < 0) {
        FB_REQUIRE(h && s && B >= 1 && B <= 3 * h->max_batch && kernel <= K_HEAD, "fb_qnet_profile_kernel: bad forward request");
        p = forward_plan(h, 0, s, B);
        p.nib = algo == -2;
    } else rc = train_plan(h, algo, B, s, a, r, s2, t, nullptr, 0.99, loss, nullptr, nullptr, nullptr, &p);
    if (rc != FB_OK) return rc;
    p.tick = false;
    for (int n = 0; n < 2; n++) resplit_now(h, n, fb_stream(stream));
    for (int i = 0; i < reps; i++) { rc = run_plan(h, p, kernel, fb_stream(stream)); if (rc != FB_OK) return rc; }
    return FB_OK;
}

extern "C" const char *fb_qnet_kernel_name(int kernel) {
    static const char *names[K_COUNT] = {"conv1_pool_kernel", "conv23_t_kernel", "(conv3: in conv23_t)", "fc1_fk_kernel", "head_kernel",
                                         "(loss: in fc1_bwd2)", "fc1_bwd2_kernel", "conv_bw_kernel", "(conv2 / conv1 dW: in conv_bw)",
                                         "(conv1 dW: in conv_bw)", "slab_reduce_kernel", "adam_fused_kernel"};
    return kernel >= 0 && kernel < K_COUNT ? names[kernel] : "";
}
```

Baseline: 11.35 million.

## Emit fc1 weight planes from the Adam update and drop trunk_done gating

The Adam update for the fc1 weight span now writes the split f16/bf16 weight planes directly. Before, a separate weight-split pass had to re-read the master weights, and the planes are marked fresh through wver. The intent is to avoid that re-read and the refresh pass on the vectorised training path. The split schedule loses its trunk_done flag and the fc1 gate on the conv backward kernels, and the fc1 backward now waits on fc1_done instead. This is simpler synchronisation but changes the ordering guarantees between the two streams. A dtype-change recheck marks planes stale so they are rebuilt.

```diff
diff --git a/dqnflappybird_amd/csrc/fb_common.h b/dqnflappybird_amd/csrc/fb_common.h
--- a/dqnflappybird_amd/csrc/fb_common.h
+++ b/dqnflappybird_amd/csrc/fb_common.h
@@ -110,10 +110,10 @@
 struct FbRingSrc { FbGatherCtx c; long long steps; const long long *idx; uint8_t *a; float *r; uint8_t *t; };
 int fb_replay_ring_src(fb_replay_t h, int batch, const int64_t *idx, uint8_t *a, float *r, uint8_t *t, FbRingSrc *out);
 int fb_qnet_train_step_ring(fb_qnet_t h, int algo, int batch, const FbRingSrc *ring, const float *isw, double gamma, float *loss,
-                            float *abs_err, float *flat_grad, void *stream, const FbSampleRider *rider = nullptr, const struct FbSplitCtx *split = nullptr);
+                            float *abs_err, float *flat_grad, void *stream, const FbSampleRider *rider = nullptr, const struct FbSplitCtx *split = nullptr,
+                            bool planes = false);
 struct FbSplitFlags {
     unsigned long long c_entry, p0[7];
-    unsigned long long trunk_done, p2[7];
     unsigned long long fc1_done, p3[7];
     unsigned long long env_done, p4[7];
     unsigned long long last_round, p8[7];
diff --git a/dqnflappybird_amd/csrc/fb_common.hip b/dqnflappybird_amd/csrc/fb_common.hip
--- a/dqnflappybird_amd/csrc/fb_common.hip
+++ b/dqnflappybird_amd/csrc/fb_common.hip
@@ -286,7 +286,7 @@
             fb_replay_begin_push_rider(replay, &prider);
             FbRingSrc ring;
             rc = fb_replay_ring_src(replay, batch, b->idx, b->a, b->r, b->t, &ring);
-            if (rc == FB_OK) rc = fb_qnet_train_step_ring(net, algo, batch, &ring, nullptr, gamma, b->loss, nullptr, b->flat_grad, C, nullptr, sc);
+            if (rc == FB_OK) rc = fb_qnet_train_step_ring(net, algo, batch, &ring, nullptr, gamma, b->loss, nullptr, b->flat_grad, C, nullptr, sc, true);
             const int rc2 = fb_env_step_rider(env, b->actions, nullptr, b->frame_bits, b->reward, b->terminal, b->score, nullptr, &prider, &hrider, S);
             const int rc3 = fb_split_set(sc, &F->env_done, sc->seq, S);
             return rc != FB_OK ? rc : rc2 != FB_OK ? rc2 : rc3;
@@ -325,7 +325,7 @@
         if (n_envs >= 256) {
             FbRingSrc ring;
             rc = fb_replay_ring_src(replay, batch, b->idx, b->a, b->r, b->t, &ring);
-            if (rc == FB_OK) rc = fb_qnet_train_step_ring(net, algo, batch, &ring, b->isw32, gamma, b->loss, b->abs_err, b->flat_grad, stream);
+            if (rc == FB_OK) rc = fb_qnet_train_step_ring(net, algo, batch, &ring, b->isw32, gamma, b->loss, b->abs_err, b->flat_grad, stream, nullptr, nullptr, true);
         } else {
             rc = fb_replay_gather(replay, batch, b->idx, b->s, b->s2, b->a, b->r, b->t, stream);
             if (rc == FB_OK) rc = fb_qnet_train_step(net, algo, batch, b->s, b->a, b->r, b->s2, b->t, b->isw32, gamma, b->loss, b->abs_err, nullptr, b->flat_grad, stream);
@@ -340,7 +340,7 @@
         FbRingSrc ring;
         rc = fb_replay_ring_src(replay, batch, b->idx, b->a, b->r, b->t, &ring);
         if (rc != FB_OK) return rc;
-        return fb_qnet_train_step_ring(net, algo, batch, &ring, nullptr, gamma, b->loss, nullptr, b->flat_grad, stream);
+        return fb_qnet_train_step_ring(net, algo, batch, &ring, nullptr, gamma, b->loss, nullptr, b->flat_grad, stream, nullptr, nullptr, true);
     }
     rc = fb_replay_gather(replay, batch, b->idx, b->s, b->s2, b->a, b->r, b->t, stream);
     if (rc != FB_OK) return rc;
diff --git a/dqnflappybird_amd/csrc/fb_qnet.hip b/dqnflappybird_amd/csrc/fb_qnet.hip
--- a/dqnflappybird_amd/csrc/fb_qnet.hip
+++ b/dqnflappybird_amd/csrc/fb_qnet.hip
@@ -920,8 +920,7 @@
 struct Fc1Args { const uint16_t *ain; size_t aplane; const uint16_t *zeros; const uint4 *w; float *hfp; int stot, M, N;
                  const unsigned *pver; unsigned *wver;
                  const uint4 *w2; int m_split;
-                 const float *hp_src; float *hp_dst; int hp_n;
-                 unsigned long long *set_flag; unsigned long long set_val; };
+                 const float *hp_src; float *hp_dst; int hp_n; };
 
 #ifndef FC1_ABL
 #define FC1_ABL 0
@@ -934,7 +933,6 @@
     const int lane = threadIdx.x & 63, wave = threadIdx.x >> 6, hl = lane >> 5, j = lane & 31;
     if (a.wver && blockIdx.x == 0 && threadIdx.x == 0) *a.wver = *a.pver;
     if (a.hp_dst) { const int i = blockIdx.x * 256 + threadIdx.x; if (i < a.hp_n) a.hp_dst[i] = a.hp_src[i]; }
-    if (a.set_flag && blockIdx.x == 0 && threadIdx.x == 0) fb_flag_store(a.set_flag, a.set_val);
     const int xcd = blockIdx.x & 7, w = blockIdx.x >> 3, nth = a.N >> 7;
     const int ks = xcd & 3, m0 = (w / nth) * 128, n0 = ((xcd >> 2) * nth + w % nth) * 64;
     const int cbase = ks * 12 + (ks < 2 ? ks : 2), count = ks < 2 ? 13 : 12;
@@ -1227,6 +1225,7 @@
     ad->ticks += 1;
 }
 __global__ void bump_pver_kernel(AdamDev *ad, int which) { ad->pver[which] += 1; }
+__global__ void mark_stale_kernel(AdamDev *ad, int which) { ad->wver[which] = ad->pver[which] - 1; }
 __global__ void mark_split_kernel(AdamDev *ad, int which) { ad->wver[which] = ad->pver[which]; ad->wverc[which] = ad->pver[which]; }
 
 struct C51Sup { int N; float vmin, vmax, dz; };
@@ -2507,15 +2506,64 @@
 #undef FB_ADAM1
 }
 
-struct AdamSpan { float *p, *m, *v; const float *g; const AdamDev *ad; int q0, q1; };
+constexpr int PLANES_F16 = 1, PLANES_BF16 = 2;
+struct AdamSpan { float *p, *m, *v; const float *g; const AdamDev *ad; int q0, q1; uint4 *planes; int FC, pmask; };
+constexpr int SPAN_WG = 512;
+constexpr int SPAN_ACTIVE = 64;
+__host__ __device__ __forceinline__ int adam_span_wgs(const AdamSpan &a) {
+    return a.planes ? (200 * (a.FC / 4) + SPAN_ACTIVE - 1) / SPAN_ACTIVE : (a.q1 - a.q0 + SPAN_WG - 1) / SPAN_WG;
+}
+__device__ __forceinline__ void adam_span_planes(int blk, int nblk, const AdamSpan a, float alpha, float omb1, float omb2, float eps) {
+    const int ug = a.FC >> 2, n = 200 * ug;
+    if (threadIdx.x >= SPAN_ACTIVE) return;
+    for (int t = blk * SPAN_ACTIVE + (int)threadIdx.x; t < n; t += nblk * SPAN_ACTIVE) {
+        const int k8 = t / ug, u4 = t - k8 * ug;
+        const size_t q = (size_t)a.q0 + (size_t)(k8 * 8) * ug + u4;
+        float4 P[8], Mv[8], V[8], Gv[8];
+#pragma unroll
+        for (int e = 0; e < 8; e++) {
+            const size_t qe = q + (size_t)e * ug;
+            P[e] = reinterpret_cast<float4 *>(a.p)[qe]; Mv[e] = reinterpret_cast<float4 *>(a.m)[qe]; V[e] = reinterpret_cast<float4 *>(a.v)[qe];
+            Gv[e] = reinterpret_cast<const float4 *>(a.g)[qe];
+        }
+#pragma unroll
+        for (int e = 0; e < 8; e++) adam4(P[e], Mv[e], V[e], Gv[e], alpha, omb1, omb2, eps);
+#pragma unroll
+        for (int e = 0; e < 8; e++) {
+            const size_t qe = q + (size_t)e * ug;
+            reinterpret_cast<float4 *>(a.p)[qe] = P[e]; reinterpret_cast<float4 *>(a.m)[qe] = Mv[e]; reinterpret_cast<float4 *>(a.v)[qe] = V[e];
+        }
+        uint4 *o = a.planes + (size_t)k8 * 3 * a.FC + 4 * u4;
+        if (a.pmask & PLANES_F16) {
+            uint4 h0, h1, h2, h3, l0, l1, l2, l3;
+            split2x2(P[0].x, P[1].x, h0.x, l0.x); split2x2(P[2].x, P[3].x, h0.y, l0.y); split2x2(P[4].x, P[5].x, h0.z, l0.z); split2x2(P[6].x, P[7].x, h0.w, l0.w);
+            split2x2(P[0].y, P[1].y, h1.x, l1.x); split2x2(P[2].y, P[3].y, h1.y, l1.y); split2x2(P[4].y, P[5].y, h1.z, l1.z); split2x2(P[6].y, P[7].y, h1.w, l1.w);
+            split2x2(P[0].z, P[1].z, h2.x, l2.x); split2x2(P[2].z, P[3].z, h2.y, l2.y); split2x2(P[4].z, P[5].z, h2.z, l2.z); split2x2(P[6].z, P[7].z, h2.w, l2.w);
+            split2x2(P[0].w, P[1].w, h3.x, l3.x); split2x2(P[2].w, P[3].w, h3.y, l3.y); split2x2(P[4].w, P[5].w, h3.z, l3.z); split2x2(P[6].w, P[7].w, h3.w, l3.w);
+            o[0] = h0; o[1] = h1; o[2] = h2; o[3] = h3;
+            o[a.FC] = l0; o[a.FC + 1] = l1; o[a.FC + 2] = l2; o[a.FC + 3] = l3;
+        }
+        if (a.pmask & PLANES_BF16) {
+            uint4 b0, b1, b2, b3;
+            uint32_t m_, l_;
+            split3x2(P[0].x, P[1].x, b0.x, m_, l_); split3x2(P[2].x, P[3].x, b0.y, m_, l_); split3x2(P[4].x, P[5].x, b0.z, m_, l_); split3x2(P[6].x, P[7].x, b0.w, m_, l_);
+            split3x2(P[0].y, P[1].y, b1.x, m_, l_); split3x2(P[2].y, P[3].y, b1.y, m_, l_); split3x2(P[4].y, P[5].y, b1.z, m_, l_); split3x2(P[6].y, P[7].y, b1.w, m_, l_);
+            split3x2(P[0].z, P[1].z, b2.x, m_, l_); split3x2(P[2].z, P[3].z, b2.y, m_, l_); split3x2(P[4].z, P[5].z, b2.z, m_, l_); split3x2(P[6].z, P[7].z, b2.w, m_, l_);
+            split3x2(P[0].w, P[1].w, b3.x, m_, l_); split3x2(P[2].w, P[3].w, b3.y, m_, l_); split3x2(P[4].w, P[5].w, b3.z, m_, l_); split3x2(P[6].w, P[7].w, b3.w, m_, l_);
+            o[2 * a.FC] = b0; o[2 * a.FC + 1] = b1; o[2 * a.FC + 2] = b2; o[2 * a.FC + 3] = b3;
+        }
+    }
+}
 __device__ __forceinline__ void adam_span_body(int blk, int nblk, const AdamSpan a) {
     const float alpha = a.ad->alpha, omb1 = 1.f - a.ad->b1, omb2 = 1.f - a.ad->b2, eps = a.ad->eps;
+    if (a.planes) { adam_span_planes(blk, nblk, a, alpha, omb1, omb2, eps); return; }
     for (int q = a.q0 + blk * (int)blockDim.x + (int)threadIdx.x; q < a.q1; q += nblk * (int)blockDim.x) {
         float4 P = reinterpret_cast<float4 *>(a.p)[q], Mv = reinterpret_cast<float4 *>(a.m)[q], V = reinterpret_cast<float4 *>(a.v)[q];
         adam4(P, Mv, V, reinterpret_cast<const float4 *>(a.g)[q], alpha, omb1, omb2, eps);
         reinterpret_cast<float4 *>(a.p)[q] = P; reinterpret_cast<float4 *>(a.m)[q] = Mv; reinterpret_cast<float4 *>(a.v)[q] = V;
     }
 }
+__global__ __launch_bounds__(SPAN_ACTIVE) void adam_span_kernel(AdamSpan span) { adam_span_body(blockIdx.x, gridDim.x, span); }
 
 constexpr int DW1_IMG_W = 104, DW1_IMG_H = 84, DW1_IMG = DW1_IMG_H * DW1_IMG_W * 4;
 constexpr int DW1_STEPS = 30;
@@ -2666,8 +2714,7 @@
 __global__ __launch_bounds__(512) void conv_dw21_kernel(int nz, int B, const float *__restrict__ p1, const float *__restrict__ dh2,
                                                         const uint8_t *__restrict__ states, const float *__restrict__ dp1,
                                                         const uint8_t *__restrict__ amax, float *__restrict__ slabs, size_t slab_stride,
-                                                        float *__restrict__ slabs1, size_t stride1, int rb, Dw1Ring ring, FbGate gate) {
-    if (fb_gate_workgroup(gate)) return;
+                                                        float *__restrict__ slabs1, size_t stride1, int rb, Dw1Ring ring) {
     const int n2 = 34 * nz;
     __shared__ uint4 pool[Dw1Lds<NSP>::U4];
     static_assert(Dw1Lds<NSP>::U4 >= 2048, "the conv2 tiles borrow the pool");
@@ -2861,9 +2908,8 @@
 template <int NS, bool RING>
 __global__ __launch_bounds__(512) void conv_bw_kernel(BxArgs bx, int B, float *__restrict__ slabs, size_t slab_stride, float *__restrict__ slabs1,
                                                       size_t stride1, const uint8_t *__restrict__ states, const uint8_t *__restrict__ amax, Dw1Ring ring,
-                                                      int n_adam, AdamSpan span, FbSampleRider rider, int rb, FbGate gate) {
+                                                      int n_adam, AdamSpan span, FbSampleRider rider, int rb) {
     __shared__ uint4 pool[BwLds<NS>::U4];
-    if (fb_gate_workgroup(gate)) return;
     static_assert(BwLds<NS>::U4 * 16 >= FB_SAMPLE_LDS_WORDS * 4, "the sampler rider borrows the pool");
     uint4 *aux = pool + BwLds<NS>::CH;
     float *dp1s = reinterpret_cast<float *>(aux + BW_AUX_U4);
@@ -3112,6 +3158,7 @@
     int tail0;
     int n_rest;
     int lanes;
+    int planes;
     FbSplitFlags *split; unsigned long long split_val;
 };
 __device__ __forceinline__ float4 shfl4(float4 v, int src) { return make_float4(__shfl(v.x, src), __shfl(v.y, src), __shfl(v.z, src), __shfl(v.w, src)); }
@@ -3180,7 +3227,10 @@
             }
         }
     }
-    if (bid == ADAMF_T2 + ADAMF_T3 && tid == 0) { a.ad->applies = a.ad->ticks; a.ad->pver[0] += 1; a.ad->wverc[0] = a.ad->pver[0]; }
+    if (bid == ADAMF_T2 + ADAMF_T3 && tid == 0) {
+        a.ad->applies = a.ad->ticks; a.ad->pver[0] += 1; a.ad->wverc[0] = a.ad->pver[0];
+        if (a.planes) a.ad->wver[0] = a.ad->pver[0];
+    }
     if (bid == ADAMF_T2 + ADAMF_T3 && tid < (int)(a.n & 3)) {
         const long long q = (n4 << 2) + tid;
         float mm = a.m[q], vv = a.v[q];
@@ -3253,6 +3303,8 @@
     uint16_t *a3n;
     int *sig_seen;
     bool split_adam_pending;
+    bool planes_pending;
+    bool wf1_recheck;
 };
 
 static NetOff make_off(int FC, int A, int dueling) {
@@ -3500,7 +3552,7 @@
     unsigned v[8] = {0};
     FB_CHECK_HIP(hipMemcpy(v, &h->split->f->clean_count, sizeof(v), hipMemcpyDeviceToHost));
     FB_REQUIRE(!(v[1] | v[2] | v[3] | v[4] | v[5] | v[6]), "fb_qnet_split_stats: waits between the two chains of the split schedule gave up after 1 s (the draw %u, the side stream's entry %u, "
-               "the fc1 backward launch's gate %u, the conv backward launch's gate %u, the Adam launch's last wait %u): the results of those steps are not to be trusted", v[1], v[2], v[3], v[4], v[5]);
+               "the fc1 backward launch's gate %u, the Adam launch's last wait %u): the results of those steps are not to be trusted", v[1], v[2], v[3], v[5]);
     *steps_host = (int64_t)h->split->seq; *clean_host = (int64_t)v[0];
     return FB_OK;
 }
@@ -3535,13 +3587,17 @@
 
 extern "C" int fb_qnet_set_inference_dtype(fb_qnet_t h, int dtype) {
     FB_REQUIRE(h && (dtype == FB_DTYPE_F32 || dtype == FB_DTYPE_BF16), "fb_qnet_set_inference_dtype: dtype must be FB_DTYPE_F32 or FB_DTYPE_BF16");
-    h->nsplit = dtype == FB_DTYPE_BF16 ? 1 : 3;
+    const int nsplit = dtype == FB_DTYPE_BF16 ? 1 : 3;
+    if (nsplit != h->nsplit) h->wf1_recheck = true;
+    h->nsplit = nsplit;
     return FB_OK;
 }
 
 extern "C" int fb_qnet_set_train_dtype(fb_qnet_t h, int dtype) {
     FB_REQUIRE(h && (dtype == FB_DTYPE_F32 || dtype == FB_DTYPE_BF16), "fb_qnet_set_train_dtype: dtype must be FB_DTYPE_F32 or FB_DTYPE_BF16");
-    h->nsplit_train = dtype == FB_DTYPE_BF16 ? 1 : 3;
+    const int nsplit = dtype == FB_DTYPE_BF16 ? 1 : 3;
+    if (nsplit != h->nsplit_train) h->wf1_recheck = true;
+    h->nsplit_train = nsplit;
     return FB_OK;
 }
 
@@ -3637,6 +3693,7 @@
     const FbSampleRider *sample_rider;
     const FbRingSrc *ring;
     const FbSplitCtx *split;
+    bool planes;
     bool any_rows;
     float *probs;
     bool no_head;
@@ -3660,6 +3717,11 @@
     int nsp, stot; size_t pl1, pl2;
 };
 static bool runs(const PlanCtx &c, int id) { return c.only < 0 || c.only == id; }
+
+static bool emits_planes(const fb_qnet *h, const Plan &p) { return p.planes && !h->noisy; }
+static int planes_mask(const fb_qnet *h) {
+    return (h->nsplit == 3 || h->nsplit_train == 3 ? PLANES_F16 : 0) | (h->nsplit == 1 || h->nsplit_train == 1 ? PLANES_BF16 : 0);
+}
 
 static PlanCtx plan_ctx(const fb_qnet *h, const Plan &p, int only, hipStream_t st) {
     PlanCtx c{only, st, 0, 0};
@@ -3725,8 +3787,7 @@
                 s0.states, s0.w1s, s0.params + OFF_B1, s0.params, h->wsp[which], h->FC, &h->adam->ovf};
     Fc1Args af{h->a3s + (size_t)row0 * 1600, c.pl2, h->zeros, h->wsp[which] + WSP_WF1, (c.fused ? h->hf_act : h->hf) + (size_t)row0 * h->FC, c.stot, rows, h->FC,
                c.fused ? pver : nullptr, c.fused ? wver : nullptr, nullptr, 0,
-               c.fused ? head_base(h, s0.params) + h->off.bf1 : nullptr, c.fused ? h->hp_act : nullptr, c.fused ? (int)(h->hoff.n - h->off.bf1) : 0,
-               c.fused && p.split && c.only < 0 ? &p.split->f->trunk_done : nullptr, p.split ? p.split->seq : 0};
+               c.fused ? head_base(h, s0.params) + h->off.bf1 : nullptr, c.fused ? h->hp_act : nullptr, c.fused ? (int)(h->hoff.n - h->off.bf1) : 0};
     if (c.trunk && z1 < p.ns && rows % 128 == 0) {
         int z2 = z1 + 1;
         while (z2 < p.ns && p.sl.s[z2].params == p.sl.s[z1].params && p.sl.s[z2].s_off == p.sl.s[z2 - 1].s_off + p.sl.s[z2 - 1].count) z2++;
@@ -3853,7 +3914,7 @@
         L.hf = h->hf; L.qpart = h->qpart; L.h3 = h->h3; L.act = p.a; L.rew = p.r; L.term = p.t; L.isw = p.isw; L.gamma = p.gamma;
         L.grad = p.G; L.dh3 = h->dh3; L.loss = p.loss; L.abs_err = p.abs_err; L.y_out = p.y;
         L.adam = h->adam; L.tick = p.tick; L.rb = h->nsplit_train == 1;
-        L.gate = p.split && c.only < 0 ? FbGate{&p.split->f->trunk_done, p.split->seq, &p.split->f->timeouts[2]} : FbGate{nullptr, 0, nullptr};
+        L.gate = p.split && c.only < 0 ? FbGate{&p.split->f->fc1_done, p.split->seq, &p.split->f->timeouts[2]} : FbGate{nullptr, 0, nullptr};
         hipLaunchKernelGGL(fc1_bwd2_kernel, dim3(ndx1 + (FC / 32) * 7 + (L.gate.flag ? 1 : 0)), dim3(512), 0, c.st, L);
         return;
     }
@@ -3870,13 +3931,13 @@
     const int B = p.B, FC = h->FC, rbt = h->nsplit_train == 1;
     int z3 = min((B * 25 + 255) / 256, h->zmax);
     const size_t ss = CONV_PARAMS;
-    const AdamSpan span{master(h, 0), h->adam_m, h->adam_v, p.G, h->adam, span0, span1};
-    const FbGate gate_fc1 = p.split && c.only < 0 ? FbGate{&p.split->f->fc1_done, p.split->seq, &p.split->f->timeouts[3]} : FbGate{nullptr, 0, nullptr};
+    const bool emit = span1 > span0 && emits_planes(h, p);
+    const AdamSpan span{master(h, 0), h->adam_m, h->adam_v, p.G, h->adam, span0, span1, emit ? h->wsp[0] + WSP_WF1 : nullptr, FC, emit ? planes_mask(h) : 0};
     const FbSampleRider srider = p.sample_rider ? *p.sample_rider : FbSampleRider{};
     const bool fold1 = 2 * B > h->zmax;
     const int fold = (2 * B + h->zmax - 1) / h->zmax;
     const int z1 = fold1 ? (2 * B + fold - 1) / fold : 2 * B;
-    const int n_adam5 = (span1 - span0 + 511) / 512;
+    const int n_adam5 = adam_span_wgs(span);
     const BxArgs bx{h->dh3, h->h2, h->p1, h->dh2, h->dp1, h->wsp[0] + wsp_w3t(FC), h->wsp[0] + wsp_w2t(FC)};
     const Dw1Ring dr{p.ring ? p.ring->c.bits : nullptr, h->ring_fo};
     float *s1 = fold1 ? h->slabs1 : h->slabs;
@@ -3886,13 +3947,13 @@
     const bool bw = !c.big && B <= h->zmax;
     if (bw) {
         z3 = B;
-        const dim3 g(BW_WGS * B + n_adam5 + (srider.k ? 1 : 0) + (gate_fc1.flag ? 1 : 0));
+        const dim3 g(BW_WGS * B + n_adam5 + (srider.k ? 1 : 0));
         if (runs(c, K_CONV3_BWD)) with_nsp(h->nsplit_train, [&](auto ns) { with_bool(p.ring != nullptr, [&](auto r) {
             hipLaunchKernelGGL((conv_bw_kernel<decltype(ns)::value, decltype(r)::value>), g, dim3(512), 0, c.st,
-                               bx, B, h->slabs, ss, s1, st1, p.s, (const uint8_t *)h->amax, dr, n_adam5, span, srider, rbt, gate_fc1);
+                               bx, B, h->slabs, ss, s1, st1, p.s, (const uint8_t *)h->amax, dr, n_adam5, span, srider, rbt);
         }); });
     } else {
-        const dim3 g3(B + 38 * zt3 + n_adam5 + (srider.k ? 1 : 0)), g2(34 * zt2 + 2 * B + (gate_fc1.flag ? 1 : 0));
+        const dim3 g3(B + 38 * zt3 + n_adam5 + (srider.k ? 1 : 0)), g2(34 * zt2 + 2 * B);
         if (runs(c, K_CONV3_BWD)) with_nsp(h->nsplit_train, [&](auto ns) {
             hipLaunchKernelGGL(conv_bx_kernel<decltype(ns)::value>, g3, dim3(512), 0, c.st, bx, B, zt3, h->slabs, ss, n_adam5, span, srider, rbt);
         });
@@ -3905,7 +3966,7 @@
         }
         if (runs(c, K_CONV2_BWD)) with_bool(p.ring != nullptr, [&](auto r) {
             hipLaunchKernelGGL((conv_dw21_kernel<2, decltype(r)::value>), g2, dim3(512), 0, c.st,
-                               zt2, B, h->p1, h->dh2, p.s, h->dp1, h->amax, h->slabs, ss, s1, st1, rbt, dr, gate_fc1);
+                               zt2, B, h->p1, h->dh2, p.s, h->dp1, h->amax, h->slabs, ss, s1, st1, rbt, dr);
         });
     }
     if (fold1 && runs(c, K_CONV2_BWD)) hipLaunchKernelGGL(slab_fold_kernel, dim3((CONV1_PARAMS + 255) / 256, z1), dim3(256), 0, c.st, h->slabs1, 2 * B, fold, h->slabs, ss);
@@ -3921,6 +3982,7 @@
         af.p = master(h, 0); af.m = h->adam_m; af.v = h->adam_v; af.g = p.G; af.n = h->ntot; af.ad = h->adam;
         af.slabs = h->slabs; af.slab_stride = CONV_PARAMS; af.z1 = z.z1; af.z2 = af.z3 = z.z3;
         af.w1s = h->w1s[0]; af.wsp = h->wsp[0]; af.FC = h->FC; af.tail0 = span1;
+        af.planes = emits_planes(h, p);
         const long long nrest4 = OFF_W2 / 4 + (OFF_W3 - OFF_B2) / 4 + (OFF_WF1 - OFF_B3) / 4 + (h->ntot / 4 - span1);
         af.lanes = 4;
         af.split = p.split && c.only < 0 ? p.split->f : nullptr; af.split_val = p.split ? p.split->seq : 0;
@@ -3933,6 +3995,7 @@
 
 static int run_plan(fb_qnet *h, const Plan &p, int only, hipStream_t st) {
     const PlanCtx c = plan_ctx(h, p, only, st);
+    if (h->wf1_recheck) { hipLaunchKernelGGL(mark_stale_kernel, dim3(1), dim3(1), 0, st, h->adam, 0); h->wf1_recheck = false; }
     if (c.trunk && runs(c, K_CONV2)) ring_trunk(h, p, c);
     if (c.big) {
         for (int z = 0; z < p.ns;) {
@@ -3943,6 +4006,7 @@
     head_stage(h, p, c);
     if (p.train) {
         if (p.tick) h->adam_ticked = !p.apply_adam;
+        if (only < 0) h->planes_pending = !p.apply_adam && emits_planes(h, p);
         if ((c.c51 || c.big) && runs(c, K_LOSS)) loss_stage(h, p, c);
         if (runs(c, K_FC1_BWD)) fc1_backward(h, p, c);
         if (!p.apply_adam && only < 0) {
@@ -4069,7 +4133,7 @@
     EnvScale es{sp ? h->a3s : nullptr, sp ? nullptr : h->h3, pl2, h->a3n, n, h->nnet.nz, 0, 0, 0, 0, h->adam, h->sig_seen, &h->adam->ovf};
     put_seed_words(es, seed, step);
     hipLaunchKernelGGL(env_noise_scale_kernel, dim3((unsigned)(((long long)n * 800 + 255) / 256)), dim3(256), 0, st, es);
-    const Fc1Args af{h->a3n, pl2, h->zeros, h->wsig + WSP_WF1, h->ht, stot, n, FC, nullptr, nullptr, nullptr, 0, nullptr, nullptr, 0, nullptr, 0};
+    const Fc1Args af{h->a3n, pl2, h->zeros, h->wsig + WSP_WF1, h->ht, stot, n, FC, nullptr, nullptr, nullptr, 0, nullptr, nullptr, 0};
     hipLaunchKernelGGL(fc1_sp_kernel<3>, dim3(((n + 127) / 128) * (FC / 64) * FC1_SP_KS), dim3(256), 0, st, af);
     EnvNoiseHead H;
     H.hf = sp ? h->hf_act : h->hf; H.ht = h->ht; H.stot = stot; H.nks = sp ? FC1_SP_KS : 1;
@@ -4195,6 +4259,13 @@
     af.slabs = nullptr; af.slab_stride = 0; af.z1 = af.z2 = af.z3 = 0;
     af.w1s = h->w1s[0]; af.wsp = h->wsp[0]; af.FC = h->FC; af.tail0 = OFF_WF1 / 4;
     af.n_rest = ADAM_GRID; af.lanes = 1;
+    af.planes = h->planes_pending && cap == hipStreamCaptureStatusNone;
+    h->planes_pending = false;
+    if (af.planes) {
+        const AdamSpan span{af.p, af.m, af.v, flat_grad, h->adam, OFF_WF1 / 4, (OFF_WF1 + 1600 * h->FC) / 4, h->wsp[0] + WSP_WF1, h->FC, planes_mask(h)};
+        af.tail0 = span.q1;
+        hipLaunchKernelGGL(adam_span_kernel, dim3(adam_span_wgs(span)), dim3(SPAN_ACTIVE), 0, st, span);
+    }
     af.split = h->split_adam_pending && h->split && h->split->tstream ? h->split->f : nullptr; af.split_val = af.split ? h->split->seq : 0;
     h->split_adam_pending = false;
     hipLaunchKernelGGL(adam_fused_kernel, dim3(ADAMF_T2 + ADAMF_T3 + af.n_rest), dim3(256), 0, st, af);
@@ -4268,13 +4339,14 @@
 }
 
 int fb_qnet_train_step_ring(fb_qnet_t h, int algo, int B, const FbRingSrc *ring, const float *isw, double gamma, float *loss, float *abs_err,
-                            float *flat_grad, void *stream, const FbSampleRider *rider, const FbSplitCtx *split) {
+                            float *flat_grad, void *stream, const FbSampleRider *rider, const FbSplitCtx *split, bool planes) {
     FB_REQUIRE(h && ring && ring->idx && ring->a && ring->r && ring->t, "fb_qnet_train_step_ring: NULL argument");
     Plan p;
     int rc = train_plan(h, algo, B, nullptr, ring->a, ring->r, nullptr, ring->t, isw, gamma, loss, abs_err, nullptr, flat_grad, &p, ring);
     if (rc != FB_OK) return rc;
     p.sample_rider = rider;
     p.split = split;
+    p.planes = planes;
     return run_plan(h, p, -1, fb_stream(stream));
 }
 
```

After: 10.78 million. 0.95x the previous value.
